# Gabriel-Ducrocq/GibbsSampler

Hardware: NVIDIA B200
Metric: gibbs_iters_per_s (higher is better)
Workload: dtype f64

## Files before the change

### gibbssampler_b200/_lib.py

```python
import ctypes as C
import os

_HERE = os.path.dirname(os.path.abspath(__file__))
LIB_PATH = os.environ.get("GIBBS_B200_LIB") or os.path.join(_HERE, "csrc", "_build", "libgibbs_b200.so")

GS_ALM_COMPLEX = 0
GS_ALM_REAL = 1

_lib = None

_vp = C.c_void_p
_i = C.c_int
_d = C.c_double
_i64 = C.c_int64

SIGNATURES = {
    "gs_last_error_string": (C.c_char_p, []),
    "gs_version": (_i, []),
    "gs_plan_create": (_i, [C.POINTER(_vp), _i, _i, _i]),
    "gs_plan_destroy": (_i, [_vp]),
    "gs_plan_reserve_chains": (_i, [_vp, _i]),
    "gs_plan_nside": (_i, [_vp]),
    "gs_plan_lmax": (_i, [_vp]),
    "gs_plan_npix": (_i64, [_vp]),
    "gs_plan_nalm": (_i64, [_vp]),
    "gs_plan_nreal": (_i64, [_vp]),
    "gs_alm2map_spin0": (_i, [_vp, _vp, _i, _vp, _vp, _vp]),
    "gs_alm2map_spin2": (_i, [_vp, _vp, _vp, _i, _vp, _vp, _vp, _vp]),
    "gs_map2alm_spin0": (_i, [_vp, _vp, _vp, _i, _i, _vp, _vp, _i, _vp]),
    "gs_map2alm_spin2": (_i, [_vp, _vp, _vp, _vp, _i, _i, _vp, _vp, _vp, _i, _vp]),
    "gs_alm2map_batch": (_i, [_vp, _i, _i, _vp, _vp, _i64, _i, _vp, _vp, _vp, _i64, _vp]),
    "gs_map2alm_batch": (_i, [_vp, _i, _i, _vp, _vp, _i64, _vp, _i, _vp, _vp, _vp, _i64, _i, _vp]),
    "gs_real_to_complex": (_i, [_vp, _vp, _i, _vp]),
    "gs_complex_to_real": (_i, [_vp, _vp, _i, _vp]),
    "gs_expand_per_l": (_i, [_vp, _i, _i, _vp, _vp]),
    "gs_unfold_bins": (_i, [_vp, _vp, _i, _vp, _i, _vp]),
    "gs_almxfl": (_i, [_vp, _i, _i, _vp, _vp, _vp]),
    "gs_alm2cl": (_i, [_vp, _i, _i, _vp, _vp]),
    "gs_alm2map_spin2_fl2": (_i, [_vp, _vp, _vp, _i, _vp, _vp, _vp, _vp, _vp]),
    "gs_cr_rhs_pol": (_i, [_vp] * 14 + [_i, _vp, _vp, _vp]),
    "gs_cr_pcg_pol": (_i, [_vp, _vp, _vp, _vp, _vp, _d, _vp, _vp, _vp, _vp, _i, _d, _i, _i,
                           C.POINTER(_i), C.POINTER(_d), _vp]),
    "gs_cr_pcg_pol_batch": (_i, [_vp, _i, _vp, _vp, _vp, _vp, _d, _vp, _vp, _vp, _vp, _i64, _d, _i, _i,
                                 C.POINTER(_i), C.POINTER(_d), _vp]),
    "gs_set_pcg_graph": (_i, [_i]),
    "gs_cr_apply_q_pol": (_i, [_vp] * 10),
    "gs_cr_rhs_tt": (_i, [_vp] * 9 + [_i, _vp, _vp]),
    "gs_cr_pcg_tt": (_i, [_vp, _vp, _vp, _vp, _d, _vp, _vp, _i, _d, _i, _i, C.POINTER(_i), C.POINTER(_d), _vp]),
    "gs_cr_apply_q_tt": (_i, [_vp] * 7),
    "gs_cr_rhs_teb": (_i, [_vp] * 22 + [_i, _vp, _vp, _vp, _vp]),
    "gs_cr_pcg_teb": (_i, [_vp] * 8 + [_d, _d] + [_vp] * 6 + [_i, _d, _i, _i, C.POINTER(_i), C.POINTER(_d), _vp]),
    "gs_cr_apply_q_teb": (_i, [_vp] * 15),
    "gs_gibbs_run_centered_fullsky": (_i, [_i, _i64, _d, _vp, _vp, _vp, _vp, _i, _vp, _i, _vp, _vp, _i, C.c_uint64, _vp, _vp, _vp, _vp,
                                           _i, _vp]),
    "gs_cr_direct": (_i, [_vp, _vp, _vp, _vp, _d, _i, _i, _vp, _vp]),
    "gs_cr_direct_pix": (_i, [_vp, _vp, _vp, _vp, _d, _i, _i, _i, _vp, _vp]),
    "gs_cls_invgamma": (_i, [_vp, _vp, _i, _vp, C.c_uint64, C.c_uint64, _vp, _vp, _vp, _vp]),
    "gs_truncnorm_propose": (_i, [_vp, _vp, _i, _vp, _vp, _vp]),
    "gs_truncnorm_logpdf": (_i, [_vp, _vp, _vp, _i, _vp, _vp]),
    "gs_loglik_pix": (_i, [_vp, _vp, _vp, _vp, _vp, _i64, _vp, _vp, _vp]),
    "gs_loglik_alm": (_i, [_vp, _vp, _vp, _vp, _vp, _vp, _i, _d, _vp, _vp, _vp]),
    "gs_randn": (_i, [_vp, _i64, C.c_uint64, C.c_uint64, _vp]),
    "gs_randu": (_i, [_vp, _i64, C.c_uint64, C.c_uint64, _vp]),
    "gs_sum": (_i, [_vp, _i64, _vp, _vp, _vp]),
    "gs_mwg_filters": (_i, [_vp, _vp, _vp, _vp, _vp, _i, _vp, _i, _i, _i, _i, _vp, _i, _i, _vp, _vp, _vp]),
    "gs_mwg_accept": (_i, [_vp, _vp, _vp, _i, _i, _vp, _vp, _vp, _vp, _vp]),
    "gs_mwg_sweep_blocks": (_i, [_vp] * 9 + [_vp, _i, _vp, _i, _vp, _i, _vp, _i, _i, _vp, _i, _vp, _vp, _vp, _vp, _vp, _vp, _i64, _vp]),
    "gs_mul": (_i, [_vp, _vp, _vp, _i64, _vp]),
    "gs_aux_v_update": (_i, [_vp, _vp, _vp, _vp, _d, _d, _vp, _vp, _i64, _vp]),
    "gs_aux_s_update": (_i, [_vp, _vp, _vp, _vp, _d, _d, _i, _vp, _vp]),
    "gs_pncp_factor": (_i, [_vp, _i, _i, _i, _vp, _vp]),
    "gs_mala_sigma": (_i, [_vp, _vp, _d, _i, _vp, _vp]),
    "gs_mala_grad": (_i, [_vp, _vp, _vp, _vp, _vp, _i64, _vp]),
    "gs_mala_propose": (_i, [_vp, _vp, _vp, _vp, _d, _vp, _i64, _vp]),
    "gs_mala_logq": (_i, [_vp, _vp, _vp, _vp, _d, _i64, _vp, _vp, _vp]),
    "gs_dot3": (_i, [_vp, _vp, _vp, _i64, _vp, _vp, _vp]),
    "gs_ula_nomask": (_i, [_vp, _vp, _vp, _vp, _vp, _d, _d, _i, _vp, _vp, _vp, _vp]),
    "gs_remove_monopole_dipole": (_i, [_vp, _i, _vp]),
    "gs_expand_var_cl_3x3": (_i, [_vp, _i, _vp, _vp]),
    "gs_inv_chol_3x3": (_i, [_vp, _vp, _i, _vp, _vp, _vp]),
    "gs_matvec_3x3": (_i, [_vp, _vp, _vp, _i, _vp, _vp]),
    "gs_alm2cl_cross": (_i, [_vp, _vp, _i, _vp, _vp]),
    "gs_cls_invwishart": (_i, [_vp, _vp, _vp, _i, _vp, C.c_uint64, C.c_uint64, _vp, _vp, _vp, _vp]),
    "gs_cls_invwishart_binned": (_i, [_vp, _vp, _vp, _i, _vp, _i, _vp, C.c_uint64, C.c_uint64, _vp, _vp, _vp, _vp]),
    "gs_nccl_unique_id": (_i, [C.c_char_p]),
    "gs_plan_create_sharded": (_i, [C.POINTER(_vp), _i, _i, _i, _i, _i, C.c_char_p]),
    "gs_local_group_create": (_i, [C.POINTER(_vp), _i]),
    "gs_local_group_destroy": (_i, [_vp]),
    "gs_plan_create_sharded_local": (_i, [C.POINTER(_vp), _i, _i, _i, _i, _i, _vp]),
    "gs_plan_world": (_i, [_vp]),
    "gs_plan_rank": (_i, [_vp]),
    "gs_plan_nreal_local": (_i64, [_vp]),
    "gs_plan_npix_local": (_i64, [_vp]),
    "gs_shard_partition_m": (_i, [_i, _i, _i, _vp]),
    "gs_shard_partition_rings": (_i, [_i, _i, _i, _vp]),
    "gs_shard_real_index": (_i64, [_i, _i, _i, _vp]),
    "gs_shard_pixel_index": (_i64, [_i, _i, _i, _vp]),
    "gs_shard_expand_per_l": (_i, [_vp, _vp, _i, _vp, _vp]),
# ... 42 lines not shown
```

### gibbssampler_b200/csrc/gs_internal.h

```cpp
#pragma once
#include <cuda_runtime.h>
#include <stdint.h>
#include <string>
#include <vector>

#include "../../include/gibbs_b200.h"

void gs_set_error(const char* fmt, ...);
#define GS_CHECK_CUDA(expr)                                                                  \
    do {                                                                                     \
        cudaError_t _e = (expr);                                                             \
        if (_e != cudaSuccess) {                                                             \
            gs_set_error("%s:%d: %s -> %s", __FILE__, __LINE__, #expr, cudaGetErrorString(_e)); \
            return GS_E_CUDA;                                                                \
        }                                                                                    \
    } while (0)
#define GS_CHECK_LAUNCH() GS_CHECK_CUDA(cudaGetLastError())
#define GS_REQUIRE(cond, msg)                                \
    do {                                                     \
        if (!(cond)) {                                       \
            gs_set_error("%s: %s", __func__, msg);           \
            return GS_E_BADARG;                              \
        }                                                    \
    } while (0)
// ... 31 lines not shown
    const int64_t* rbase;
    const int* m_owner;
    const int* m_loc;
    const int* ring_owner;
    const int* ring_loc;
    const int64_t* ring_start_loc;
    const int* l_of_loc;
};

struct SplitJob {
    int ringA, compA, ringB, compB;
    int bs2;
    int pad;
    int64_t off;
};

struct PlanDev {
    int nside, lmax, nring, npair;
    int64_t npix, nalm;
    const double* cth;
    const double* sth;
    const double* c2;
    const double* s2;
    const int* mlim0;
    const int* mlim2;
    const int* pmin0;
    const int* pmin2;
    const ScaledSeed* seed0;
    const ScaledSeed* seed2;
    const ScaledSeed* sinpow;
    const double* rec0;
    const double* alpha0;
    const double2* rec2;
    const double* alpha2;
    const int* ring_nphi;
    const int64_t* ring_start;
    const int* ring_phq;
    const int* ring_phden;
    const int* ring_bs;
    const BluesteinDesc* bs;
    const double2* bs_tab;
    const double2* tw;
    int tw_n;
    int max_M;
    ShardDev sh;
};

struct RingFlags {
    unsigned char* act_ring;
    int* act_pairs;
    int* act_count;
    int* act_slot0;
    double* ring_wconst;
    int2* groups0_dyn;
    int2* groups2_dyn;
};

struct gs_plan {
    int device;
    PlanDev d;
    int world, rank;
    int64_t nreal_loc, npix_loc;
    void* comm;
    void* lgroup;
    double2* Fx;
    double* red_loc;
    std::vector<int> h_mlist, h_rings;
    std::vector<void*> owned;
    RingJob* jobs2;
    int njobs2;
    RingJob* jobs0;
    int njobs0;
    int2* groups2;
    int ngroups2;
    int2* groups0;
    int ngroups0;
    int2* groups2_dyn;
    int2* groups0_dyn;
    SplitJob* sjobs2;
    int nsjobs2;
    SplitJob* sjobs0;
    int nsjobs0;
    double2* ring_scratch;
    size_t split_smem;
    double2* mwg_F;
    double* mwg_maps;
    int mwg_group;
    double* mwg_small;
    double* mwg_data;
    int* mwg_meta;
    std::vector<int> mwg_meta_host;
    unsigned char* act_ring;
    int* act_pairs;
    int* act_count;
    double* act_red;
    int* act_slot0;
    double* ring_wconst;
    bool use_act;
    double2* Fm;
    double* partial;
    int anal_chunks;
    int chain_cap;
    size_t ring_smem;
    double* mapQ_tmp;
    double* mapU_tmp;
    double* almE_tmp;
    double* almB_tmp;
    double* almE_tmp2;
    double* almB_tmp2;
    void* pcg_ws;
    void* pcg_ws_batch;
    int* pcg_alldone;
    void* pcg_ws_teb;
    RingFlags flags_T;
    void* comm_stream;
    std::vector<void*> comm_events;
    void* work_stream;
    void* work_event;
};

extern int g_gs_ring_const;
extern int g_gs_ring_skip;
extern int g_gs_ring_fused;
extern long long g_gs_launches;
static inline int64_t gs_nalm(int lmax) { return (int64_t)(lmax + 1) * (lmax + 2) / 2; }

int gs_leg_synth(gs_plan* p, int spin, const double* almE, const double* almB, int layout, const double* fl,
                 cudaStream_t st, const int* skip = nullptr, const double* flB = nullptr, int nc = 1, int64_t alm_stride = 0);
int gs_leg_anal(gs_plan* p, int spin, double* almE, double* almB, int layout, const double* fl, double scale,
                int accumulate, cudaStream_t st, const int* skip = nullptr, int nc = 1, int64_t alm_stride = 0);
int64_t gs_fm_stride(const gs_plan* p);
int64_t gs_part_stride(const gs_plan* p, int nc);
int gs_active_rings_build(gs_plan* p, const double* pixw, cudaStream_t st);
int gs_leg_build_sinpow(gs_plan* p);
int gs_leg_prepare(gs_plan* p);
int gs_ring_setup(gs_plan* p);
int gs_ring_synth(gs_plan* p, int spin, double* mapQ, double* mapU, cudaStream_t st, const int* skip = nullptr, int nc = 1,
                  int64_t map_stride = 0, const double* wconst = nullptr);
int gs_ring_anal(gs_plan* p, int spin, const double* mapQ, const double* mapU, const double* pixw, cudaStream_t st,
                 const int* skip = nullptr, int nc = 1, int64_t map_stride = 0);
int gs_ring_apply(gs_plan* p, int spin, const double* pixw, cudaStream_t st, const int* skip = nullptr, int nc = 1);
int gs_ring_synth_batch(gs_plan* p, const double2* F, int64_t f_stride, const int* mmax, double* mapQ, double* mapU,
                        int64_t map_stride, int nb, cudaStream_t st, const unsigned char* ract = nullptr, const double* wconst = nullptr);
int gs_ring_order_build(gs_plan* p, cudaStream_t st);
int gs_ring_mwg_data(gs_plan* p, const double* mapQ, const double* mapU, double* outQ, double* outU, const double* wconst, cudaStream_t st);
int gs_leg_synth_blocks(gs_plan* p, const double* almE, const double* almB, const double* dflE, const double* dflB,
                        const int* lbE, int e0, int e1, const int* lbB, int b0, int b1, int lend, double2* Fblk, cudaStream_t st);
int gs_launch_expand_per_l(const double* x, int lmax, int mode, double* out, cudaStream_t st);
int gs_plan_expand_per_l(gs_plan* p, const double* x, int mode, double* out, cudaStream_t st);
void gs_pcg_ws_free(gs_plan* p);
int gs_shard_build(gs_plan* p, int rank, int world, const char* nccl_id);
void gs_shard_free(gs_plan* p);
int gs_shard_exchange(gs_plan* p, const double2* send, double2* recv, cudaStream_t st);
int gs_shard_exchange_block(gs_plan* p, const double2* send, double2* recv, int blk, cudaStream_t st);
int gs_shard_pipeline(gs_plan* p, cudaStream_t* comm, cudaEvent_t** events);
int gs_shard_allreduce(gs_plan* p, double* buf, int n, cudaStream_t st);
```

### gibbssampler_b200/csrc/legendre.cu

```cuda
#include <algorithm>
#include <type_traits>

#include "gs_internal.h"

#ifndef LEG_NT
#define LEG_NT 128
#endif
#define LEG_NW (LEG_NT / 32)
#define LEG_TL LEG_NT
#ifndef LEG_SU
#define LEG_SU 1
#endif
#define LEG_TLS (LEG_SU * LEG_NT)
#ifndef LEG_R
#define LEG_R 2
#endif
#ifndef LEG_R2
#define LEG_R2 2
#endif
#ifndef LEG_RA
#define LEG_RA 4
#endif
#ifndef LEG_UA
#define LEG_UA 2
// ... 189 lines not shown
#pragma unroll
    for (int c = 1; c < NC; ++c) {
        double2 dummy;
        fetch_alm<SPIN, false>(P, m, l, base, roff, almE + c * alm_stride, SPIN ? almB + c * alm_stride : almB, layout, fl, flB, e[c], b[c], dummy);
    }
}

template <bool SH>
__device__ __forceinline__ int64_t fm_index(const PlanDev& P, int comp, int ring, int m, int mk)
{
    if (SH) {
        const int blk = mk / P.sh.MLb, w = mk - blk * P.sh.MLb;
        return ((((int64_t)blk * P.sh.world + P.sh.ring_owner[ring]) * 2 + comp) * P.sh.RL + P.sh.ring_loc[ring]) * P.sh.MLb + w;
    }
    return ((int64_t)comp * P.nring + ring) * (P.lmax + 1) + m;
}
template <bool SH>
__device__ __forceinline__ int64_t real_off(const PlanDev& P, int m, int mk, int64_t base)
{
    if (SH) return P.sh.rbase[mk] - (m ? 2 : 1) * (int64_t)m;
    return m ? 2 * base - (P.lmax + 1) : 0;
}

template <int SPIN>
struct SynthAcc {
    double sqr, sqi, aqr, aqi;
    double sur, sui, aur, aui;
};

template <int SPIN, bool FIRST>
__device__ __forceinline__ void synth_acc(SynthAcc<SPIN>& A, double pc, double mc, double2 e, double2 b)
{
    if (SPIN == 0) {
        if (FIRST) { A.sqr = fma(e.x, pc, A.sqr); A.sqi = fma(e.y, pc, A.sqi); }
        else       { A.aqr = fma(e.x, pc, A.aqr); A.aqi = fma(e.y, pc, A.aqi); }
    } else {
        A.sqr = fma(pc, e.x, A.sqr); A.sqi = fma(mc, e.y, A.sqi);
        A.sur = fma(pc, b.x, A.sur); A.sui = fma(mc, b.y, A.sui);
        if (FIRST) {
            A.aqr = fma(mc, e.x, A.aqr); A.aqi = fma(pc, e.y, A.aqi);
            A.aur = fma(mc, b.x, A.aur); A.aui = fma(pc, b.y, A.aui);
        } else {
            A.aqr = fma(-mc, e.x, A.aqr); A.aqi = fma(-pc, e.y, A.aqi);
            A.aur = fma(-mc, b.x, A.aur); A.aui = fma(-pc, b.y, A.aui);
        }
    }
}

template <int SPIN, int R, bool SH, int NC>
__global__ void LEG_SYNTH_BOUNDS
leg_synth_kernel(PlanDev P, const double* __restrict__ almE, const double* __restrict__ almB, int layout,
                 const double* __restrict__ fl, const double* __restrict__ flB, double2* __restrict__ Fm,
                 const int* __restrict__ skip, const int* __restrict__ plist, const int* __restrict__ pcount,
                 const int* __restrict__ slot0, int64_t alm_stride, int64_t fm_stride, int mk0)
{
    if (skip && *skip) return;
    const int L = P.lmax, mk = blockIdx.y + mk0, m = SH ? P.sh.mlist[mk] : mk, tid = threadIdx.x;
    const int s0 = slot0[m], nact = (plist ? *pcount : P.npair) - s0;
    if ((int)blockIdx.x * (LEG_NT * R) >= nact) return;
    __shared__ double2 sEb[2][NC][LEG_TLS], sBb[2][SPIN ? NC : 1][SPIN ? LEG_TLS : 1], sRb[2][LEG_TLS];
    const int l0 = m > SPIN ? m : SPIN;
    const int64_t base = (int64_t)m * (2 * L + 1 - m) / 2;
    const int64_t roff = real_off<SH>(P, m, mk, base);
    const int chunk = blockIdx.x * (LEG_NT * R);

    RingState<SPIN> st[R];
    SynthAcc<SPIN> acc[R][NC];
    int pj[R];
    bool any_act = false;
    unsigned myact = 0;
#pragma unroll
    for (int j = 0; j < R; ++j) {
        const int k = chunk + ((tid >> 5) * R + j) * 32 + (tid & 31);
        const int p = k < nact ? (plist ? plist[s0 + k] : s0 + k) : -1;
        pj[j] = p;
        st[j].x = 0.0; st[j].pc = st[j].pp = st[j].mc = st[j].mp = 0.0; st[j].sc = 0;
#pragma unroll
        for (int c = 0; c < NC; ++c) {
            acc[j][c].sqr = acc[j][c].sqi = acc[j][c].aqr = acc[j][c].aqi = 0.0;
            acc[j][c].sur = acc[j][c].sui = acc[j][c].aur = acc[j][c].aui = 0.0;
        }
        if (p >= 0 && m <= (SPIN ? P.mlim2[p] : P.mlim0[p])) {
            st[j].x = P.cth[p];
            seed_ring<SPIN>(P, p, m, st[j].pc, st[j].mc, st[j].sc);
            any_act = true;
            myact |= 1u << j;
        }
    }
    const bool warp_act = __any_sync(FULL, any_act);
    unsigned gact = 0;
#pragma unroll
    for (int j = 0; j < R; ++j) if (__any_sync(FULL, (myact >> j) & 1u)) gact |= 1u << j;
    bool all_live = false;

#pragma unroll
    for (int u = 0; u < LEG_SU; ++u) {
        double2 e[NC], b[NC], r;
        fetch_alm_nc<SPIN, NC>(P, m, l0 + u * LEG_NT + tid, base, roff, almE, almB, alm_stride, layout, fl, flB, e, b, r);
#pragma unroll
        for (int c = 0; c < NC; ++c) { sEb[0][c][u * LEG_NT + tid] = e[c]; if (SPIN) sBb[0][c][u * LEG_NT + tid] = b[c]; }
        sRb[0][u * LEG_NT + tid] = r;
    }
    __syncthreads();
    int cur = 0;
    for (int lt = l0; lt <= L; lt += LEG_TLS, cur ^= 1) {
        const bool has_next = lt + LEG_TLS <= L;
        double2 ne[LEG_SU][NC], nb[LEG_SU][NC], nr[LEG_SU];
// ... 62 lines not shown
                        }
                        rec_step<SPIN>(st[j], r0.x, r0.y);
                        if (j >= J0) {
#pragma unroll
                            for (int c = 0; c < NC; ++c) synth_acc<SPIN, false>(acc[j][c], st[j].pc, st[j].mc, e1[c], b1[c]);
                        }
                        rec_step<SPIN>(st[j], r1.x, r1.y);
                    }
                }
            };
            if (R >= 4 && jlo == 3) run(std::integral_constant<int, (R >= 4 ? 3 : R)>());
            else if (R >= 3 && jlo == 2) run(std::integral_constant<int, (R >= 3 ? 2 : R)>());
            else if (R >= 2 && jlo == 1) run(std::integral_constant<int, (R >= 2 ? 1 : R)>());
            else run(std::integral_constant<int, R>());
        }
#pragma unroll 2
        for (; ip < npr; ++ip) {
            const int i = 2 * ip;
            const double2 r0 = sR[i], r1 = sR[i + 1];
            double2 e0[NC], b0[NC], e1[NC], b1[NC];
#pragma unroll
            for (int c = 0; c < NC; ++c) {
                e0[c] = sE[c][i]; e1[c] = sE[c][i + 1];
                b0[c] = SPIN ? sB[c][i] : e0[c]; b1[c] = SPIN ? sB[c][i + 1] : e1[c];
            }
#pragma unroll
            for (int j = 0; j < R; ++j) {
#pragma unroll
                for (int c = 0; c < NC; ++c) synth_acc<SPIN, true>(acc[j][c], st[j].pc, st[j].mc, e0[c], b0[c]);
                rec_step<SPIN>(st[j], r0.x, r0.y);
#pragma unroll
                for (int c = 0; c < NC; ++c) synth_acc<SPIN, false>(acc[j][c], st[j].pc, st[j].mc, e1[c], b1[c]);
                rec_step<SPIN>(st[j], r1.x, r1.y);
            }
        }
        if (has_next) {
#pragma unroll
            for (int u = 0; u < LEG_SU; ++u) {
#pragma unroll
                for (int c = 0; c < NC; ++c) { sEb[cur ^ 1][c][u * LEG_NT + tid] = ne[u][c]; if (SPIN) sBb[cur ^ 1][c][u * LEG_NT + tid] = nb[u][c]; }
                sRb[cur ^ 1][u * LEG_NT + tid] = nr[u];
            }
        }
        __syncthreads();
    }

    const double sg = ((l0 + m) & 1) ? -1.0 : 1.0;
#pragma unroll
    for (int j = 0; j < R; ++j) {
        const int p = pj[j];
        if (p < 0) continue;
        const int rn = p, rs = P.nring - 1 - p;
        const int64_t in = fm_index<SH>(P, 0, rn, m, mk), is = fm_index<SH>(P, 0, rs, m, mk);
#pragma unroll
        for (int c = 0; c < NC; ++c) {
            const SynthAcc<SPIN>& a = acc[j][c];
            double2* F = Fm + c * fm_stride;
            if (SPIN == 0) {
                F[in] = make_double2(a.sqr + a.aqr, a.sqi + a.aqi);
                if (rs != rn) F[is] = make_double2(sg * (a.sqr - a.aqr), sg * (a.sqi - a.aqi));
            } else {
                const int64_t cs = SH ? (int64_t)P.sh.RL * P.sh.MLb : (int64_t)P.nring * (L + 1);
                F[in] = make_double2(a.sqr + a.sqi, a.sur + a.sui);
                F[in + cs] = make_double2(a.sur - a.sui, a.sqi - a.sqr);
                if (rs != rn) {
                    F[is] = make_double2(sg * (a.aqr + a.aqi), sg * (a.aur + a.aui));
                    F[is + cs] = make_double2(sg * (a.aur - a.aui), sg * (a.aqi - a.aqr));
                }
            }
        }
    }
}

template <int R, bool DO_E, bool DO_B>
__global__ void __launch_bounds__(LEG_NT)
leg_synth_blocks_kernel(PlanDev P, const double* __restrict__ almE, const double* __restrict__ almB, const double* __restrict__ dflE,
                        const double* __restrict__ dflB, const int* __restrict__ lbE, int e0, int e1, const int* __restrict__ lbB,
                        int b0, int b1, int lend, double2* __restrict__ Fblk)
{
    __shared__ double2 sE[LEG_TL], sB[LEG_TL], sSE[LEG_TL], sSB[LEG_TL], sR[LEG_TL];
    extern __shared__ unsigned char sflag[];
    const int L = P.lmax, m = blockIdx.y, tid = threadIdx.x;
    const int l0 = m > 2 ? m : 2;
    if (l0 >= lend) return;
    const int s0 = P.pmin2[m], nact = P.npair - s0;
    const int chunk = blockIdx.x * (LEG_NT * R);
    if (chunk >= nact) return;
    unsigned char* sfE = sflag;
    unsigned char* sfB = sflag + (L + 2);
    for (int i = tid; i < 2 * (L + 2); i += LEG_NT) sflag[i] = 0;
    __syncthreads();
    if (DO_E) for (int i = e0 + tid; i < e1; i += LEG_NT) { const int end = lbE[i + 1]; if (end >= 1 && end <= L + 1) sfE[end - 1] = 1; }
    if (DO_B) for (int i = b0 + tid; i < b1; i += LEG_NT) { const int end = lbB[i + 1]; if (end >= 1 && end <= L + 1) sfB[end - 1] = 1; }
    const int64_t base = (int64_t)m * (2 * L + 1 - m) / 2;
    const int64_t roff = real_off<false>(P, m, m, base);
    const int64_t nm = L + 1, cs = (int64_t)P.nring * nm, slot = 2 * cs;

    RingState<2> st[R];
    double aE[R][DO_E ? 8 : 1], aB[R][DO_B ? 8 : 1];
    int pj[R];
    bool any_act = false, all_plain = true;
#pragma unroll
    for (int j = 0; j < R; ++j) {
        const int k = chunk + ((tid >> 5) * R + j) * 32 + (tid & 31);
        const int p = k < nact ? s0 + k : -1;
        pj[j] = p;
        st[j].x = 0.0; st[j].pc = st[j].pp = st[j].mc = st[j].mp = 0.0; st[j].sc = 0;
#pragma unroll
        for (int q = 0; q < (DO_E ? 8 : 1); ++q) aE[j][q] = 0.0;
#pragma unroll
        for (int q = 0; q < (DO_B ? 8 : 1); ++q) aB[j][q] = 0.0;
        if (p >= 0 && m <= P.mlim2[p]) {
            st[j].x = P.cth[p];
            seed_ring<2>(P, p, m, st[j].pc, st[j].mc, st[j].sc);
            any_act = true;
            all_plain = all_plain && st[j].sc == 0;
        }
    }
    const bool warp_act = __any_sync(FULL, any_act);
    bool fast = __all_sync(FULL, all_plain);
// ... 435 lines not shown
        } else {
#pragma unroll kUnrollA
            for (; ip < npr; ++ip) {
                double v[NC][NVAL];
                const double2 r0 = sR[2 * ip], r1 = sR[2 * ip + 1];
#pragma unroll
                for (int j = 0; j < R; ++j) {
#pragma unroll
                    for (int c = 0; c < NC; ++c) {
                        if (j == 0) anal_acc<SPIN, true, true>(v[c], G[j][c], st[j].pc, st[j].mc);
                        else anal_acc<SPIN, true, false>(v[c], G[j][c], st[j].pc, st[j].mc);
                    }
                    rec_step<SPIN>(st[j], r0.x, r0.y);
#pragma unroll
                    for (int c = 0; c < NC; ++c) {
                        if (j == 0) anal_acc<SPIN, false, true>(v[c] + NV, G[j][c], st[j].pc, st[j].mc);
                        else anal_acc<SPIN, false, false>(v[c] + NV, G[j][c], st[j].pc, st[j].mc);
                    }
                    rec_step<SPIN>(st[j], r1.x, r1.y);
                }
#pragma unroll
                for (int c = 0; c < NC; ++c) {
                    const double s = warp_fold<SPIN>(v[c], lane);
                    if (writer) sPart(w, c)[ip * NVAL + vidx] = __hiloint2double(__double2hiint(s) ^ flipmask, __double2loint(s));
                }
            }
        }
        __syncthreads();
#pragma unroll
        for (int c = 0; c < NC; ++c) {
            double* out = partial + c * part_stride + (pbase + lt) * NV;
            for (int i = tid; i < ni * NV; i += LEG_NT) {
                double s = 0.0;
#pragma unroll
                for (int ww = 0; ww < LEG_NW; ++ww) s += sPart(ww, c)[i];
                out[i] = s;
            }
        }
    }
}

template <int SPIN, bool SH>
__global__ void leg_finish_kernel(PlanDev P, const double* __restrict__ partial, int nchunk, double* __restrict__ almE,
                                  double* __restrict__ almB, int layout, const double* __restrict__ fl, double scale,
                                  int accumulate, const int* __restrict__ skip, const int* __restrict__ pcount,
                                  const int* __restrict__ slot0, int chunk_pairs, int64_t part_stride, int64_t alm_stride)
{
    if (skip && *skip) return;
    constexpr int NV = SPIN ? 4 : 2;
    const int L = P.lmax, mk = blockIdx.y, m = SH ? P.sh.mlist[mk] : mk;
    partial += blockIdx.z * part_stride;
    almE += blockIdx.z * alm_stride;
    if (SPIN) almB += blockIdx.z * alm_stride;
    {
        const int nact = (pcount ? *pcount : P.npair) - slot0[m];
        nchunk = nact > 0 ? (nact + chunk_pairs - 1) / chunk_pairs : 0;
    }
    const int l = m + blockIdx.x * blockDim.x + threadIdx.x;
    if (l > L) return;
    const int64_t base = (int64_t)m * (2 * L + 1 - m) / 2, id = base + l;
    const int64_t pid = SH ? P.sh.cbase[mk] + (l - m) : id, pn = SH ? P.sh.nalm_loc : P.nalm;
    const int64_t roff = real_off<SH>(P, m, mk, base);
    double v[NV];
#pragma unroll
    for (int c = 0; c < NV; ++c) v[c] = 0.0;
    if (l >= SPIN) {
        for (int k = 0; k < nchunk; ++k) {
            const double* q = partial + ((int64_t)k * pn + pid) * NV;
#pragma unroll
            for (int c = 0; c < NV; ++c) v[c] += q[c];
        }
        if (SPIN) {
            const double y1 = v[0], y2 = v[1], y3 = v[2], y4 = v[3];
            v[0] = y1 + y2; v[1] = y3 + y4; v[2] = y3 - y4; v[3] = y2 - y1;
        }
        double post = scale * (SPIN ? -0.5 * P.alpha2[id] : P.alpha0[id]);
        if (fl) post *= fl[l];
        if (layout == GS_ALM_REAL && m > 0) post *= 1.41421356237309504880;
#pragma unroll
        for (int c = 0; c < NV; ++c) v[c] *= post;
    }
    if (layout == GS_ALM_COMPLEX) {
        double2* E = reinterpret_cast<double2*>(almE);
        double2 e = make_double2(v[0], v[1]);
        if (accumulate) { double2 o = E[id]; e.x += o.x; e.y += o.y; }
        E[id] = e;
        if (SPIN) {
            double2* B = reinterpret_cast<double2*>(almB);
            double2 b = make_double2(v[2], v[3]);
            if (accumulate) { double2 o = B[id]; b.x += o.x; b.y += o.y; }
            B[id] = b;
        }
    } else if (m == 0) {
        almE[roff + l] = accumulate ? almE[roff + l] + v[0] : v[0];
        if (SPIN) almB[roff + l] = accumulate ? almB[roff + l] + v[2] : v[2];
    } else {
        const int64_t off = roff + 2 * l;
        almE[off] = accumulate ? almE[off] + v[0] : v[0];
        almE[off + 1] = accumulate ? almE[off + 1] + v[1] : v[1];
        if (SPIN) {
            almB[off] = accumulate ? almB[off] + v[2] : v[2];
            almB[off + 1] = accumulate ? almB[off + 1] + v[3] : v[3];
        }
    }
}

template <bool SH>
__global__ void __launch_bounds__(256) ring_active_kernel(PlanDev P, const double* __restrict__ pixw, unsigned char* __restrict__ act,
                                                          double* __restrict__ actd, double* __restrict__ wconst)
{
    const int ring = blockIdx.x, n = P.ring_nphi[ring];
    if (SH && P.sh.ring_owner[ring] != P.sh.rank) { if (threadIdx.x == 0) actd[ring] = 0.0; return; }
    const double* w = pixw + (SH ? P.sh.ring_start_loc[ring] : P.ring_start[ring]);
    const double w0 = w[0];
    int any = 0, differ = 0;
    for (int j = threadIdx.x; j < n; j += blockDim.x) { const double v = w[j]; any |= (v != 0.0); differ |= !(v == w0); }
    any = __syncthreads_or(any);
    if (!SH && wconst) differ = __syncthreads_or(differ);
    if (threadIdx.x == 0) {
        if (SH) actd[ring] = any ? 1.0 : 0.0; else act[ring] = any ? 1 : 0;
        if (!SH && wconst) wconst[ring] = differ ? __longlong_as_double(0x7ff8000000000000LL) : w0;
    }
}

__global__ void ring_flags_kernel(const double* __restrict__ actd, unsigned char* __restrict__ act, int n)
{
    const int i = blockIdx.x * blockDim.x + threadIdx.x;
    if (i < n) act[i] = actd[i] > 0.0 ? 1 : 0;
}

__global__ void __launch_bounds__(1024) pair_compact_kernel(PlanDev P, unsigned char* act, int* __restrict__ list,
                                                            int* __restrict__ count)
{
    __shared__ int wsum[32];
// ... 17 lines not shown
    }
    if (tid == 0) *count = base;
}

__global__ void __launch_bounds__(256) list_slot0_kernel(PlanDev P, const int* __restrict__ list, const int* __restrict__ count,
                                                         int* __restrict__ slot0)
{
    const int L = P.lmax, wid = (blockIdx.x * blockDim.x + threadIdx.x) >> 5, lane = threadIdx.x & 31;
    if (wid >= 2 * (L + 1)) return;
    const int spin2 = wid > L, m = spin2 ? wid - (L + 1) : wid, n = *count;
    const int* mlim = spin2 ? P.mlim2 : P.mlim0;
    int first = n;
    for (int k0 = 0; k0 < n && first == n; k0 += 32) {
        const int k = k0 + lane;
        const unsigned b = __ballot_sync(FULL, k < n && mlim[list[k]] >= m);
        if (b) first = k0 + __ffs(b) - 1;
    }
    if (lane == 0) slot0[wid] = first;
}

int gs_active_rings_build(gs_plan* p, const double* pixw, cudaStream_t st)
{
    if (p->world > 1) {
        ring_active_kernel<true><<<p->d.nring, 256, 0, st>>>(p->d, pixw, p->act_ring, p->act_red, nullptr);
        GS_CHECK_LAUNCH();
        int rc = gs_shard_allreduce(p, p->act_red, p->d.nring, st);
        if (rc) return rc;
        ring_flags_kernel<<<(p->d.nring + 255) / 256, 256, 0, st>>>(p->act_red, p->act_ring, p->d.nring);
    } else {
        ring_active_kernel<false><<<p->d.nring, 256, 0, st>>>(p->d, pixw, p->act_ring, nullptr, p->ring_wconst);
    }
    pair_compact_kernel<<<1, 1024, 0, st>>>(p->d, p->act_ring, p->act_pairs, p->act_count);
    list_slot0_kernel<<<(2 * (p->d.lmax + 1) * 32 + 255) / 256, 256, 0, st>>>(p->d, p->act_pairs, p->act_count, p->act_slot0);
    GS_CHECK_LAUNCH();
    g_gs_launches += 3;
    return gs_ring_order_build(p, st);
}

int64_t gs_fm_stride(const gs_plan* p) { return (int64_t)2 * p->d.nring * (p->d.lmax + 1); }
static int anal_chunks_of(const gs_plan* p, int nc) { const int per = LEG_NT * (nc > 1 ? LEG_RA2 : LEG_RA); return (p->d.npair + per - 1) / per; }
int64_t gs_part_stride(const gs_plan* p, int nc) { return (int64_t)anal_chunks_of(p, nc) * p->d.nalm * 4; }

static int check_batch(const gs_plan* p, int nc, int layout, const char* who)
{
    if (nc == 1) return GS_OK;
    if (nc != 2) { gs_set_error("%s: chain batches run 2 right-hand sides per launch (got %d)", who, nc); return GS_E_BADARG; }
    if (p->world > 1) { gs_set_error("%s: chain batches need an unsharded plan", who); return GS_E_BADARG; }
    if (p->chain_cap < nc) { gs_set_error("%s: call gs_plan_reserve_chains(plan, %d) first", who, nc); return GS_E_BADARG; }
    (void)layout;
    return GS_OK;
}

int gs_leg_synth(gs_plan* p, int spin, const double* almE, const double* almB, int layout, const double* fl,
                 cudaStream_t st, const int* skip, const double* flB, int nc, int64_t alm_stride)
{
    const bool sh = p->world > 1;
    if (sh && layout != GS_ALM_REAL) { gs_set_error("sharded plans take the (local) real alm layout only"); return GS_E_BADARG; }
    int rc = check_batch(p, nc, layout, "gs_leg_synth");
    if (rc) return rc;
    const int rr = nc == 2 ? LEG_R2 : LEG_R;
    dim3 grid((p->d.npair + LEG_NT * rr - 1) / (LEG_NT * rr), sh ? p->d.sh.nm_loc : p->d.lmax + 1);
    const int* plist = p->use_act ? p->act_pairs : nullptr;
    const int* pcount = plist ? p->act_count : nullptr;
    const int* slot0 = plist ? p->act_slot0 + (spin ? p->d.lmax + 1 : 0) : (spin ? p->d.pmin2 : p->d.pmin0);
    const int64_t fs = gs_fm_stride(p);
    if (nc == 2) {
        if (spin == 0) leg_synth_kernel<0, LEG_R2, false, 2><<<grid, LEG_NT, 0, st>>>(p->d, almE, almB, layout, fl, flB, p->Fm, skip, plist, pcount, slot0, alm_stride, fs, 0);
        else leg_synth_kernel<2, LEG_R2, false, 2><<<grid, LEG_NT, 0, st>>>(p->d, almE, almB, layout, fl, flB, p->Fm, skip, plist, pcount, slot0, alm_stride, fs, 0);
    } else if (!sh) {
        if (spin == 0) leg_synth_kernel<0, LEG_R, false, 1><<<grid, LEG_NT, 0, st>>>(p->d, almE, almB, layout, fl, flB, p->Fm, skip, plist, pcount, slot0, 0, 0, 0);
        else leg_synth_kernel<2, LEG_R, false, 1><<<grid, LEG_NT, 0, st>>>(p->d, almE, almB, layout, fl, flB, p->Fm, skip, plist, pcount, slot0, 0, 0, 0);
    } else {
        const ShardDev& S = p->d.sh;
        cudaStream_t comm = st;
        cudaEvent_t* ev = nullptr;
        const bool pipelined = !p->lgroup && S.NB > 1;
        if (pipelined && (rc = gs_shard_pipeline(p, &comm, &ev))) return rc;
        for (int b = 0; b < S.NB; ++b) {
            const int mk0 = b * S.MLb, cnt = std::min(S.MLb, S.nm_loc - mk0);
            if (cnt > 0) {
                dim3 g(grid.x, cnt);
                if (spin == 0) leg_synth_kernel<0, LEG_R, true, 1><<<g, LEG_NT, 0, st>>>(p->d, almE, almB, layout, fl, flB, p->Fm, skip, plist, pcount, slot0, 0, 0, mk0);
                else leg_synth_kernel<2, LEG_R, true, 1><<<g, LEG_NT, 0, st>>>(p->d, almE, almB, layout, fl, flB, p->Fm, skip, plist, pcount, slot0, 0, 0, mk0);
                GS_CHECK_LAUNCH();
                g_gs_launches += 1;
            }
            if (pipelined) {
                GS_CHECK_CUDA(cudaEventRecord(ev[b], st));
                GS_CHECK_CUDA(cudaStreamWaitEvent(comm, ev[b], 0));
            }
            if ((rc = gs_shard_exchange_block(p, p->Fm, p->Fx, b, comm))) return rc;
        }
        if (pipelined) {
            GS_CHECK_CUDA(cudaEventRecord(ev[S.NB], comm));
            GS_CHECK_CUDA(cudaStreamWaitEvent(st, ev[S.NB], 0));
        }
        return GS_OK;
    }
    GS_CHECK_LAUNCH();
    g_gs_launches += 1;
    return GS_OK;
}

template <int SPIN, int R, bool SH, int NC>
static int launch_anal(gs_plan* p, dim3 grid, cudaStream_t st, const int* skip, const int* plist, const int* pcount, const int* slot0,
                       int64_t fs, int64_t ps, int mk0 = 0)
{
    constexpr size_t sm = leg_anal_smem<SPIN, NC>();
    leg_anal_kernel<SPIN, R, SH, NC><<<grid, LEG_NT, sm, st>>>(p->d, p->Fm, p->partial, skip, plist, pcount, slot0, fs, ps, mk0);
    GS_CHECK_LAUNCH();
    return GS_OK;
}

int gs_leg_prepare(gs_plan* p)
{
    (void)p;
#define GS_ANAL_ATTR(SPIN, R, SH, NC) \
    GS_CHECK_CUDA(cudaFuncSetAttribute(leg_anal_kernel<SPIN, R, SH, NC>, cudaFuncAttributeMaxDynamicSharedMemorySize, (int)leg_anal_smem<SPIN, NC>()))
    GS_ANAL_ATTR(0, LEG_RA, false, 1); GS_ANAL_ATTR(2, LEG_RA, false, 1);
    GS_ANAL_ATTR(0, LEG_RA, true, 1);  GS_ANAL_ATTR(2, LEG_RA, true, 1);
    GS_ANAL_ATTR(0, LEG_RA2, false, 2); GS_ANAL_ATTR(2, LEG_RA2, false, 2);
#undef GS_ANAL_ATTR
    return GS_OK;
}

int gs_leg_anal(gs_plan* p, int spin, double* almE, double* almB, int layout, const double* fl, double scale,
                int accumulate, cudaStream_t st, const int* skip, int nc, int64_t alm_stride)
{
    const bool sh = p->world > 1;
    if (sh && layout != GS_ALM_REAL) { gs_set_error("sharded plans take the (local) real alm layout only"); return GS_E_BADARG; }
    int rc = check_batch(p, nc, layout, "gs_leg_anal");
    if (rc) return rc;
    const int nchunk = anal_chunks_of(p, nc);
    if (nchunk * nc > p->anal_chunks) { gs_set_error("gs_leg_anal: workspace too small"); return GS_E_BADARG; }
    const int nmy = sh ? p->d.sh.nm_loc : p->d.lmax + 1;
    dim3 grid(nchunk, nmy);
    dim3 fgrid((p->d.lmax + 256) / 256, nmy, nc);
    const int* plist = p->use_act ? p->act_pairs : nullptr;
    const int* pcount = plist ? p->act_count : nullptr;
    const int* slot0 = plist ? p->act_slot0 + (spin ? p->d.lmax + 1 : 0) : (spin ? p->d.pmin2 : p->d.pmin0);
    const int64_t fs = gs_fm_stride(p), ps = gs_part_stride(p, nc);
    const int cp = LEG_NT * (nc > 1 ? LEG_RA2 : LEG_RA);

    if (nc == 2) {
        if (spin == 0) {
            if ((rc = launch_anal<0, LEG_RA2, false, 2>(p, grid, st, skip, plist, pcount, slot0, fs, ps))) return rc;
            leg_finish_kernel<0, false><<<fgrid, 256, 0, st>>>(p->d, p->partial, nchunk, almE, almB, layout, fl, scale, accumulate, skip, pcount, slot0, cp, ps, alm_stride);
        } else {
            if ((rc = launch_anal<2, LEG_RA2, false, 2>(p, grid, st, skip, plist, pcount, slot0, fs, ps))) return rc;
            leg_finish_kernel<2, false><<<fgrid, 256, 0, st>>>(p->d, p->partial, nchunk, almE, almB, layout, fl, scale, accumulate, skip, pcount, slot0, cp, ps, alm_stride);
        }
    } else if (!sh) {
        if (spin == 0) {
            if ((rc = launch_anal<0, LEG_RA, false, 1>(p, grid, st, skip, plist, pcount, slot0, 0, 0))) return rc;
            leg_finish_kernel<0, false><<<fgrid, 256, 0, st>>>(p->d, p->partial, nchunk, almE, almB, layout, fl, scale, accumulate, skip, pcount, slot0, cp, 0, 0);
        } else {
            if ((rc = launch_anal<2, LEG_RA, false, 1>(p, grid, st, skip, plist, pcount, slot0, 0, 0))) return rc;
            leg_finish_kernel<2, false><<<fgrid, 256, 0, st>>>(p->d, p->partial, nchunk, almE, almB, layout, fl, scale, accumulate, skip, pcount, slot0, cp, 0, 0);
        }
    } else {
        const ShardDev& S = p->d.sh;
        cudaStream_t comm = st;
        cudaEvent_t* ev = nullptr;
        const bool pipelined = !p->lgroup && S.NB > 1;
        if (pipelined) {
            if ((rc = gs_shard_pipeline(p, &comm, &ev))) return rc;
            GS_CHECK_CUDA(cudaEventRecord(ev[S.NB], st));
            GS_CHECK_CUDA(cudaStreamWaitEvent(comm, ev[S.NB], 0));
        }
        for (int b = 0; b < S.NB; ++b) {
            if ((rc = gs_shard_exchange_block(p, p->Fx, p->Fm, b, comm))) return rc;
            if (pipelined) {
                GS_CHECK_CUDA(cudaEventRecord(ev[b], comm));
                GS_CHECK_CUDA(cudaStreamWaitEvent(st, ev[b], 0));
            }
            const int mk0 = b * S.MLb, cnt = std::min(S.MLb, S.nm_loc - mk0);
            if (cnt <= 0) continue;
            dim3 g(grid.x, cnt);
            if (spin == 0) rc = launch_anal<0, LEG_RA, true, 1>(p, g, st, skip, plist, pcount, slot0, 0, 0, mk0);
            else rc = launch_anal<2, LEG_RA, true, 1>(p, g, st, skip, plist, pcount, slot0, 0, 0, mk0);
            if (rc) return rc;
        }
        if (spin == 0) leg_finish_kernel<0, true><<<fgrid, 256, 0, st>>>(p->d, p->partial, nchunk, almE, almB, layout, fl, scale, accumulate, skip, pcount, slot0, cp, 0, 0);
        else leg_finish_kernel<2, true><<<fgrid, 256, 0, st>>>(p->d, p->partial, nchunk, almE, almB, layout, fl, scale, accumulate, skip, pcount, slot0, cp, 0, 0);
    }
    GS_CHECK_LAUNCH();
    g_gs_launches += 2;
    return GS_OK;
}

int gs_leg_synth_blocks(gs_plan* p, const double* almE, const double* almB, const double* dflE, const double* dflB,
                        const int* lbE, int e0, int e1, const int* lbB, int b0, int b1, int lend, double2* Fblk, cudaStream_t st)
{
    if (p->world > 1) { gs_set_error("block-batched synthesis needs an unsharded plan"); return GS_E_BADARG; }
    constexpr int RB = 2;
    dim3 grid((p->d.npair + LEG_NT * RB - 1) / (LEG_NT * RB), std::min(lend, p->d.lmax + 1));
    const size_t sm = 2 * (size_t)(p->d.lmax + 2);
    const bool doE = e1 > e0, doB = b1 > b0;
    if (!doE && !doB) return GS_OK;
    if (doE && doB) leg_synth_blocks_kernel<RB, true, true><<<grid, LEG_NT, sm, st>>>(p->d, almE, almB, dflE, dflB, lbE, e0, e1, lbB, b0, b1, lend, Fblk);
    else if (doE) leg_synth_blocks_kernel<RB, true, false><<<grid, LEG_NT, sm, st>>>(p->d, almE, almB, dflE, dflB, lbE, e0, e1, lbB, b0, b1, lend, Fblk);
    else leg_synth_blocks_kernel<RB, false, true><<<grid, LEG_NT, sm, st>>>(p->d, almE, almB, dflE, dflB, lbE, e0, e1, lbB, b0, b1, lend, Fblk);
    GS_CHECK_LAUNCH();
    g_gs_launches += 1;
    return GS_OK;
}
```

### gibbssampler_b200/csrc/plan.cu

```cuda
#include <math.h>
#include <stdarg.h>
#include <stdio.h>
#include <string.h>

#include <algorithm>

#include "gs_internal.h"

static thread_local char g_err[512] = "";

void gs_set_error(const char* fmt, ...)
{
    va_list ap;
    va_start(ap, fmt);
    vsnprintf(g_err, sizeof(g_err), fmt, ap);
    va_end(ap);
}

extern "C" const char* gs_last_error_string(void) { return g_err; }
extern "C" int gs_version(void) { return 100; }

static const long double PI_L = 3.14159265358979323846264338327950288L;

template <typename T>
// ... 152 lines not shown
                long double ll = l, L1 = l + 1.0L, mm = m;
                long double den = sqrtl((L1 * L1 - mm * mm) * (L1 * L1 - mp * mp));
                long double f = L1 * (2.0L * ll + 1.0L) / den;
                long double A = sqrtl((2.0L * ll + 3.0L) / (2.0L * ll + 1.0L)) * f;
                long double B = (l == 0) ? 0.0L : mm * mp / (ll * L1);
                long double a_next;
                if (l == l0) a_next = 1.0L;
                else {
                    long double Cc = sqrtl((2.0L * ll + 3.0L) / (2.0L * ll - 1.0L)) * f *
                                     sqrtl((ll * ll - mm * mm) * (ll * ll - mp * mp)) / (ll * (2.0L * ll + 1.0L));
                    a_next = Cc * a_prev;
                }
                long double a = A * a_cur / a_next;
                if (spin == 0) rec0[base + l] = (double)a;
                else rec2[base + l] = make_double2((double)a, (double)(a * B));
                a_prev = a_cur;
                a_cur = a_next;
            }
        }
    }
    if ((rc = upload(p, rec0, &p->d.rec0))) return rc;
    if ((rc = upload(p, alpha0, &p->d.alpha0))) return rc;
    if ((rc = upload(p, rec2, &p->d.rec2))) return rc;
    if ((rc = upload(p, alpha2, &p->d.alpha2))) return rc;
    return GS_OK;
}

static int plan_create_impl(gs_plan** out, int nside, int lmax, int device, int rank, int world, const char* nccl_id,
                            void* lgroup = nullptr)
{
    if (!out) { gs_set_error("gs_plan_create: null output"); return GS_E_BADARG; }
    *out = nullptr;
    GS_REQUIRE(nside >= 1 && nside <= 8192, "nside out of range [1, 8192]");
    GS_REQUIRE(lmax >= 2 && lmax <= 4 * nside, "lmax must satisfy 2 <= lmax <= 4 nside");
    GS_REQUIRE(world >= 1 && rank >= 0 && rank < world, "need 0 <= rank < world");
    GS_REQUIRE(world <= 2 * nside && world <= (lmax + 2) / 2, "more ranks than ring pairs or m pairs");
    if (device >= 0) GS_CHECK_CUDA(cudaSetDevice(device));
    int dev = 0;
    GS_CHECK_CUDA(cudaGetDevice(&dev));
    gs_plan* p = new gs_plan();
    memset(&p->d, 0, sizeof(p->d));
    p->device = dev;
    p->d.nside = nside;
    p->d.lmax = lmax;
    p->jobs0 = p->jobs2 = nullptr;
    p->groups0 = p->groups2 = nullptr;
    p->groups0_dyn = p->groups2_dyn = nullptr;
    p->ngroups0 = p->ngroups2 = 0;
    p->sjobs0 = p->sjobs2 = nullptr;
    p->nsjobs0 = p->nsjobs2 = 0;
    p->ring_scratch = nullptr;
    p->act_ring = nullptr;
    p->ring_wconst = nullptr;
    p->act_pairs = nullptr;
    p->act_count = nullptr;
    p->act_slot0 = nullptr;
    p->act_red = nullptr;
    p->use_act = false;
    p->mwg_F = nullptr;
    p->mwg_maps = nullptr;
    p->mwg_group = 0;
    p->mwg_small = nullptr;
    p->mwg_data = nullptr;
    p->mwg_meta = nullptr;
    p->world = world;
    p->rank = rank;
    p->comm = nullptr;
    p->lgroup = lgroup;
    p->pcg_ws = nullptr;
    p->pcg_ws_batch = nullptr;
    p->pcg_alldone = nullptr;
    p->pcg_ws_teb = nullptr;
    memset(&p->flags_T, 0, sizeof(p->flags_T));
    p->work_stream = nullptr;
    p->work_event = nullptr;
    p->comm_stream = nullptr;
    p->chain_cap = 1;
    p->Fx = nullptr;
    p->red_loc = nullptr;
    p->d.sh.world = 1;
    int rc = build_tables(p);
    if (rc == GS_OK) rc = gs_leg_build_sinpow(p);
    if (rc == GS_OK) rc = gs_leg_prepare(p);
    const int64_t nm = lmax + 1;
    p->nreal_loc = nm * nm;
    p->npix_loc = p->d.npix;
    if (rc == GS_OK && world > 1) rc = gs_shard_build(p, rank, world, nccl_id);
    if (rc == GS_OK) rc = gs_ring_setup(p);
    if (rc == GS_OK) {
        const size_t nfm = world > 1 ? (size_t)world * 2 * p->d.sh.RL * p->d.sh.ML : (size_t)2 * p->d.nring * nm;
        rc = dev_alloc(p, nfm, &p->Fm);
        if (rc == GS_OK && world > 1) rc = dev_alloc(p, nfm, &p->Fx);
        if (rc == GS_OK) cudaMemset(p->Fm, 0, nfm * sizeof(double2));
        if (rc == GS_OK && world > 1) cudaMemset(p->Fx, 0, nfm * sizeof(double2));
        p->anal_chunks = (p->d.npair + 127) / 128;
        const size_t nalm_part = world > 1 ? (size_t)p->d.sh.nalm_loc : (size_t)p->d.nalm;
        if (rc == GS_OK) rc = dev_alloc(p, (size_t)p->anal_chunks * nalm_part * 4, &p->partial);
        if (rc == GS_OK) rc = dev_alloc(p, (size_t)p->d.nring, &p->act_ring);
        if (rc == GS_OK) rc = dev_alloc(p, (size_t)p->d.npair, &p->act_pairs);
        if (rc == GS_OK) rc = dev_alloc(p, (size_t)1, &p->act_count);
        if (rc == GS_OK) rc = dev_alloc(p, (size_t)2 * (lmax + 1), &p->act_slot0);
        if (rc == GS_OK) rc = dev_alloc(p, (size_t)p->d.nring, &p->act_red);
        if (rc == GS_OK && world <= 1) rc = dev_alloc(p, (size_t)p->d.nring, &p->ring_wconst);
        if (rc == GS_OK) rc = dev_alloc(p, (size_t)p->npix_loc, &p->mapQ_tmp);
        if (rc == GS_OK) rc = dev_alloc(p, (size_t)p->npix_loc, &p->mapU_tmp);
        const size_t nre = (size_t)p->nreal_loc;
        if (rc == GS_OK) rc = dev_alloc(p, nre, &p->almE_tmp);
        if (rc == GS_OK) rc = dev_alloc(p, nre, &p->almB_tmp);
        if (rc == GS_OK) rc = dev_alloc(p, nre, &p->almE_tmp2);
        if (rc == GS_OK) rc = dev_alloc(p, nre, &p->almB_tmp2);
    }
    if (rc == GS_OK) {
        cudaError_t e = cudaDeviceSynchronize();
        if (e != cudaSuccess) { gs_set_error("plan setup: %s", cudaGetErrorString(e)); rc = GS_E_CUDA; }
    }
    if (rc != GS_OK) { gs_plan_destroy(p); return rc; }
    *out = p;
    return GS_OK;
}

extern "C" int gs_plan_create(gs_plan** out, int nside, int lmax, int device)
{
    return plan_create_impl(out, nside, lmax, device, 0, 1, nullptr);
}

extern "C" int gs_plan_create_sharded(gs_plan** out, int nside, int lmax, int device, int rank, int world,
                                      const char* nccl_id128_host)
{
    return plan_create_impl(out, nside, lmax, device, rank, world, nccl_id128_host);
}

extern "C" int gs_plan_create_sharded_local(gs_plan** out, int nside, int lmax, int device, int rank, int world,
                                            void* local_group)
{
    if (!local_group) { gs_set_error("null local group"); return GS_E_BADARG; }
    return plan_create_impl(out, nside, lmax, device, rank, world, nullptr, local_group);
}

extern "C" int gs_plan_reserve_chains(gs_plan* p, int n_chain)
{
    if (!p) { gs_set_error("null plan"); return GS_E_BADARG; }
    GS_REQUIRE(n_chain >= 1 && n_chain <= 2, "n_chain must be 1 or 2");
    GS_REQUIRE(p->world == 1, "chain batches need an unsharded plan");
    if (n_chain <= p->chain_cap) return GS_OK;
    GS_CHECK_CUDA(cudaSetDevice(p->device));
    const int64_t nm = p->d.lmax + 1;
    const size_t nfm = (size_t)n_chain * 2 * p->d.nring * nm;
    double2* F = nullptr;
    int rc = dev_alloc(p, nfm, &F);
    if (rc) return rc;
    GS_CHECK_CUDA(cudaMemset(F, 0, nfm * sizeof(double2)));
    const int chunks = std::max(p->anal_chunks, n_chain * ((p->d.npair + 255) / 256));
    double* part = nullptr;
    if (chunks > p->anal_chunks) {
        rc = dev_alloc(p, (size_t)chunks * p->d.nalm * 4, &part);
        if (rc) return rc;
// ... 34 lines not shown
```

### gibbssampler_b200/csrc/ringfft.cu

```cuda
#include <math.h>
#include <stdlib.h>

#include <algorithm>
#include <map>

#include "gs_internal.h"

#define RF_NT 256

__device__ __forceinline__ double2 cmul(double2 a, double2 b) { return make_double2(a.x * b.x - a.y * b.y, a.x * b.y + a.y * b.x); }
__device__ __forceinline__ double2 cmulc(double2 a, double2 b) { return make_double2(a.x * b.x + a.y * b.y, a.y * b.x - a.x * b.y); }
__device__ __forceinline__ double2 cadd(double2 a, double2 b) { return make_double2(a.x + b.x, a.y + b.y); }
__device__ __forceinline__ double2 csub(double2 a, double2 b) { return make_double2(a.x - b.x, a.y - b.y); }

#define PADI(i) ((i) + ((i) >> 4) + ((i) >> 8))
#define PADLEN(M) ((M) + ((M) >> 4) + ((M) >> 8) + 2)

__device__ __forceinline__ double2 tw_get(const double2* twq, int idx, int quarter)
{
    if (idx < quarter) return twq[idx];
    const double2 w = twq[idx - quarter];
    return make_double2(w.y, -w.x);
}

// ... 167 lines not shown
    if (r == 3) { N <<= 3; pass8<true>(buf, M, N, twq, twn, tid, nt); return; }
    if (r & 2) { N <<= 2; pass4<true>(buf, M, N, twq, twn, tid, nt); }
    if (r & 1) { N <<= 1; pass2<true>(buf, M, N, twq, twn, tid, nt); }
}

__device__ __forceinline__ void load_twq(const PlanDev& P, double2* twq)
{
    const int nq = (P.tw_n >> 2) + 1;
    for (int k = threadIdx.x; k < nq; k += RF_NT) twq[k] = __ldg(&P.tw[k]);
}

__device__ __forceinline__ double2 chirp_val(int t, int n)
{
    const int r = (int)(((long long)t * t) % (2 * n));
    double s, c;
    sincospi((double)r / (double)n, &s, &c);
    return make_double2(c, s);
}

__device__ void ring_idft(const PlanDev& P, double2* buf, const double2* twq, int n, int bsi, int tid = threadIdx.x, int nt = RF_NT)
{
    __syncthreads();
    if (bsi < 0) { fft_dit_inv(buf, n, twq, P.tw_n, tid, nt); return; }
    const BluesteinDesc d = P.bs[bsi];
    fft_dif<true>(buf, d.M, twq, P.tw_n, P.bs_tab + d.bhat_off, tid, nt);
    fft_dit_inv(buf, d.M, twq, P.tw_n, tid, nt);
}

__global__ void __launch_bounds__(RF_NT) bluestein_setup_kernel(PlanDev P, double2* tab, int nbs)
{
    extern __shared__ double2 smem_all[];
    double2* twq = smem_all;
    double2* buf = smem_all + (P.tw_n >> 2) + 1;
    load_twq(P, twq);
    const BluesteinDesc d = P.bs[blockIdx.x];
    double2* chirp = tab + d.chirp_off;
    double2* bhat = tab + d.bhat_off;
    for (int k = threadIdx.x; k < d.M; k += blockDim.x) buf[PADI(k)] = make_double2(0.0, 0.0);
    __syncthreads();
    for (int t = threadIdx.x; t < d.n; t += blockDim.x) {
        const double2 c = chirp_val(t, d.n);
        chirp[t] = c;
        const double2 cc = make_double2(c.x, -c.y);
        buf[PADI(t)] = cc;
        if (t > 0) buf[PADI(d.M - t)] = cc;
    }
    __syncthreads();
    fft_dif<false>(buf, d.M, twq, P.tw_n, nullptr);
    const double inv = 1.0 / (double)d.M;
    for (int k = threadIdx.x; k < d.M; k += blockDim.x) { const double2 v = buf[PADI(k)]; bhat[k] = make_double2(v.x * inv, v.y * inv); }
    (void)nbs;
}

__device__ __forceinline__ double2 ring_phase(const PlanDev& P, int ring, int m)
{
    const int q = P.ring_phq[ring], den = P.ring_phden[ring];
    const unsigned r = ((unsigned)m * (unsigned)q) % (2u * (unsigned)den);
    double s, c;
    sincospi((double)r / (double)den, &s, &c);
    return make_double2(c, s);
}

template <bool SH>
__device__ __forceinline__ int64_t fm_ring_index(const PlanDev& P, int comp, int ring, int m)
{
    if (SH) return P.sh.m_base[m] + ((int64_t)comp * P.sh.RL + P.sh.ring_loc[ring]) * P.sh.MLb;
    return ((int64_t)comp * P.nring + ring) * (P.lmax + 1) + m;
}
template <bool SH>
__device__ __forceinline__ int64_t ring_first_pixel(const PlanDev& P, int ring)
{
    return SH ? P.sh.ring_start_loc[ring] : P.ring_start[ring];
}

__device__ __forceinline__ int ring_mtop(const PlanDev& P, int ring, int spin2)
{
    const int p = ring < P.npair ? ring : P.nring - 1 - ring;
    return spin2 ? P.mlim2[p] : P.mlim0[p];
}

__device__ __forceinline__ bool group_idle(const unsigned char* __restrict__ ract, const RingJob* __restrict__ jobs, const int2* __restrict__ groups)
{
    if (!ract) return false;
    const int2 g = groups[blockIdx.x];
    bool any = false;
    for (int s = 0; s < g.y; ++s) {
        const RingJob jb = jobs[g.x + s];
        any = any || ract[jb.ringA] || (jb.ringB >= 0 && ract[jb.ringB]);
    }
    return !any;
}
__device__ __forceinline__ bool group_const(const double* __restrict__ wconst, const RingJob* __restrict__ jobs, const int2* __restrict__ groups)
{
    if (!wconst) return false;
    const int2 g = groups[blockIdx.x];
    bool all = true;
    for (int s = 0; s < g.y; ++s) {
        const RingJob jb = jobs[g.x + s];
        const double a = wconst[jb.ringA], b = jb.ringB >= 0 ? wconst[jb.ringB] : 0.0;
        all = all && a == a && b == b;
    }
    return all;
}
__global__ void __launch_bounds__(1024) ring_order_kernel(const RingJob* __restrict__ jobs, const int2* __restrict__ groups, int ngroups,
                                                          const unsigned char* __restrict__ ract, const double* __restrict__ wconst,
                                                          int2* __restrict__ groups_out)
{
    __shared__ int wcount[32][3];
    __shared__ int base[3], total[3];
    const int tid = threadIdx.x, lane = tid & 31, w = tid >> 5;
    auto cls_of = [&](int gi) {
        if (gi >= ngroups) return 3;
        const int2 g = groups[gi];
        bool any = false, allc = true;
        for (int s = 0; s < g.y; ++s) {
            const RingJob jb = jobs[g.x + s];
            any = any || ract[jb.ringA] || (jb.ringB >= 0 && ract[jb.ringB]);
            const double a = wconst[jb.ringA], b = jb.ringB >= 0 ? wconst[jb.ringB] : 0.0;
            allc = allc && a == a && b == b;
        }
        return !any ? 2 : allc ? 1 : 0;
    };
    for (int pass = 0; pass < 2; ++pass) {
        if (tid < 3) { if (pass == 0) total[tid] = 0; else base[tid] = tid == 0 ? 0 : tid == 1 ? total[0] : total[0] + total[1]; }
        __syncthreads();
        for (int g0 = 0; g0 < ngroups; g0 += 1024) {
            const int gi = g0 + tid, c = cls_of(gi);
            unsigned bal[3];
#pragma unroll
            for (int k = 0; k < 3; ++k) { bal[k] = __ballot_sync(0xffffffffu, c == k); if (lane == 0) wcount[w][k] = __popc(bal[k]); }
            __syncthreads();
            if (pass == 1 && c < 3) {
                int off = base[c];
                for (int i = 0; i < w; ++i) off += wcount[i][c];
                groups_out[off + __popc(bal[c] & ((1u << lane) - 1u))] = groups[gi];
            }
            __syncthreads();
            if (tid < 3) {
                int t = 0;
                for (int i = 0; i < 32; ++i) t += wcount[i][tid];
                if (pass == 0) total[tid] += t; else base[tid] += t;
            }
            __syncthreads();
        }
    }
}

__device__ __forceinline__ bool split_idle(const unsigned char* __restrict__ ract, const SplitJob& jb)
{
    return ract && !(ract[jb.ringA] || (jb.ringB >= 0 && ract[jb.ringB]));
}

struct RingSub {
    RingJob job;
    int n, bsi, M, tid, nt;
    double2* buf;
    double2* scratch;
    const double2* chirp;
};

// ... 270 lines not shown
    const int lg = 31 - __clz(n);
    for (int j = S.tid; j < S.M; j += S.nt) {
        const int pos = PADI(S.bsi < 0 ? (int)(__brev((unsigned)j) >> (32 - lg)) : j);
        if (j >= n) { S.buf[pos] = make_double2(0.0, 0.0); continue; }
        double a = ia[j], b = ib ? ib[j] : 0.0;
        if (pixw) { a *= pixw[sa + j]; if (ib) b *= pixw[sb + j]; }
        double2 z = make_double2(a, -b);
        if (S.bsi >= 0) z = cmul(z, __ldg(&S.chirp[j]));
        S.buf[pos] = z;
    }
    ring_idft(P, S.buf, twq, n, S.bsi, S.tid, S.nt);
    ring_unpack_F<SH>(P, S, UNPACK_CONJ, Fm, ring_mtop(P, job.ringA, spin2), S.bsi >= 0 ? S.chirp : nullptr);
}

__global__ void __launch_bounds__(RF_NT, 2)
ring_mwg_data_kernel(PlanDev P, const RingJob* __restrict__ jobs, const int2* __restrict__ groups, const double* __restrict__ mapQ,
                     const double* __restrict__ mapU, double* __restrict__ outQ, double* __restrict__ outU, const double* __restrict__ wconst)
{
    extern __shared__ double2 smem[];
    double2* twq = smem;
    const bool spectral = group_const(wconst, jobs, groups);
    if (spectral) load_twq(P, twq);
    const RingSub S = ring_sub(P, jobs, groups, twq + (P.tw_n >> 2) + 1);
    const int n = S.n;
    const int64_t s0 = P.ring_start[S.job.ringA];
    const double* ia = mapQ + s0;
    const double* ib = mapU + s0;
    if (!spectral) {
        for (int j = S.tid; j < n; j += S.nt) { outQ[s0 + j] = ia[j]; outU[s0 + j] = ib[j]; }
        return;
    }
    const int lg = 31 - __clz(n);
    for (int j = S.tid; j < S.M; j += S.nt) {
        const int pos = PADI(S.bsi < 0 ? (int)(__brev((unsigned)j) >> (32 - lg)) : j);
        if (j >= n) { S.buf[pos] = make_double2(0.0, 0.0); continue; }
        double2 z = make_double2(ia[j], -ib[j]);
        if (S.bsi >= 0) z = cmul(z, __ldg(&S.chirp[j]));
        S.buf[pos] = z;
    }
    ring_idft(P, S.buf, twq, n, S.bsi, S.tid, S.nt);
    const double s = rsqrt((double)n);
    for (int k = S.tid; k < n; k += S.nt) {
        double2 c = S.buf[PADI(k)];
        if (S.bsi >= 0) c = cmul(c, __ldg(&S.chirp[k]));
        outQ[s0 + k] = s * c.x;
        outU[s0 + k] = -s * c.y;
    }
}

template <bool SH>
__global__ void __launch_bounds__(RF_NT, 2)
ring_apply_kernel(PlanDev P, const RingJob* __restrict__ jobs, const int2* __restrict__ groups, double2* __restrict__ Fm,
                  const double* __restrict__ pixw, const int* __restrict__ skip, const unsigned char* __restrict__ ract, int spin2,
                  int64_t f_stride, const double* __restrict__ wconst)
{
    if (skip && *skip) return;
    if (group_idle(ract, jobs, groups)) return;
    extern __shared__ double2 smem[];
    Fm += blockIdx.y * f_stride;
    double2* twq = smem;
    if (group_const(wconst, jobs, groups)) {
        const RingSub S = ring_sub(P, jobs, groups, twq + (P.tw_n >> 2) + 1);
        const int mtop = ring_mtop(P, S.job.ringA, spin2);
        const double wA = wconst[S.job.ringA], wB = wconst[S.job.ringB >= 0 ? S.job.ringB : S.job.ringA];
        bool direct = true;
        {
            const int2 g = groups[blockIdx.x];
            for (int s = 0; s < g.y; ++s) {
                const int ra = jobs[g.x + s].ringA;
                direct = direct && 2 * ring_mtop(P, ra, spin2) <= P.ring_nphi[ra];
            }
        }
        if (direct) {
            const RingJob& job = S.job;
            const double sa = (double)S.n * wA, sb = (double)S.n * wB;
            for (int m = S.tid; m <= mtop; m += S.nt) {
                const int64_t ia = fm_ring_index<SH>(P, job.compA, job.ringA, m);
                const int64_t ib = job.ringB >= 0 ? fm_ring_index<SH>(P, job.compB, job.ringB, m) : ia;
                double2 a = Fm[ia], b = job.ringB >= 0 ? Fm[ib] : make_double2(0.0, 0.0);
                if (m == 0) { a.y = 0.0; b.y = 0.0; }
                else if (2 * m == S.n) {
                    const double2 e2 = ring_phase(P, job.ringA, 2 * m);
                    const double2 ta = cmul(a, e2), tb = cmul(b, e2);
                    a = make_double2(a.x + ta.x, a.y - ta.y);
                    b = make_double2(b.x + tb.x, b.y - tb.y);
                }
                Fm[ia] = make_double2(sa * a.x, sa * a.y);
                if (job.ringB >= 0) Fm[ib] = make_double2(sb * b.x, sb * b.y);
            }
            return;
        }
        ring_build_Z<SH>(P, S, Fm, mtop, S.scratch, false, true);
        __syncthreads();
        const double half_n = 0.5 * (double)S.n;
        ring_unpack_F<SH>(P, S, UNPACK_PLAIN, Fm, mtop, nullptr, half_n * wA, half_n * wB);
        return;
    }
    load_twq(P, twq);
    const RingSub S = ring_sub(P, jobs, groups, twq + (P.tw_n >> 2) + 1);
    const int n = S.n;
    const double* wa = pixw + ring_first_pixel<SH>(P, S.job.ringA);
    const double* wb = S.job.ringB >= 0 ? pixw + ring_first_pixel<SH>(P, S.job.ringB) : wa;
    const int mtop = ring_mtop(P, S.job.ringA, spin2);
    ring_build_Z<SH>(P, S, Fm, mtop, S.scratch);
    __syncthreads();
    ring_idft(P, S.buf, twq, n, S.bsi, S.tid, S.nt);
    if (S.bsi < 0) {
        auto weigh = [wa, wb](int j, double2 z) { return make_double2(z.x * wa[j], z.y * wb[j]); };
        fft_dif<false>(S.buf, n, twq, P.tw_n, nullptr, S.tid, S.nt, weigh);
        ring_unpack_F<SH>(P, S, UNPACK_BREV, Fm, mtop);
    } else {
        const double2* chirp = S.chirp;
        for (int j = S.tid; j < S.M; j += S.nt) {
            if (j >= n) { S.buf[PADI(j)] = make_double2(0.0, 0.0); continue; }
            const double2 c = __ldg(&chirp[j]);
            const double2 z = cmul(S.buf[PADI(j)], c);
            S.buf[PADI(j)] = cmul(make_double2(z.x * wa[j], -z.y * wb[j]), c);
        }
        ring_idft(P, S.buf, twq, n, S.bsi, S.tid, S.nt);
        ring_unpack_F<SH>(P, S, UNPACK_CONJ, Fm, mtop, chirp);
    }
    __syncthreads();
}

template <bool SH>
__device__ __forceinline__ double2 fold_spectrum(const PlanDev& P, const double2* __restrict__ Fm, int comp, int ring, int k, int n, int L)
{
    const int kk = (n - k) % n;
    double2 g = make_double2(0.0, 0.0), h = g;
    for (int m = k; m <= L; m += n) {
        const double w = m ? 1.0 : 0.5;
        const double2 ph = ring_phase(P, ring, m);
        g = cadd(g, cmul(Fm[fm_ring_index<SH>(P, comp, ring, m)], make_double2(ph.x * w, ph.y * w)));
    }
    for (int m = kk; m <= L; m += n) {
        const double w = m ? 1.0 : 0.5;
        const double2 ph = ring_phase(P, ring, m);
        h = cadd(h, cmul(Fm[fm_ring_index<SH>(P, comp, ring, m)], make_double2(ph.x * w, ph.y * w)));
    }
    return make_double2(g.x + h.x, g.y - h.y);
}

__device__ __forceinline__ double2 mul_ipow(double2 v, int p)
{
// ... 354 lines not shown
        return rc;
    }
    const RingJob* jobs = spin == 0 ? p->jobs0 : p->jobs2;
    const int2* grp = spin == 0 ? p->groups0 : p->groups2;
    const SplitJob* sj = spin == 0 ? p->sjobs0 : p->sjobs2;
    const unsigned char* ract = p->use_act ? p->act_ring : nullptr;
    const double* mu = spin == 0 ? mapQ : mapU;
    const bool sh = p->world > 1;
    double2* F = sh ? p->Fx : p->Fm;
    if (ns > 0) {
        if (sh) {
            ring_anal_split_kernel<true><<<4 * ns, RF_NT, p->split_smem, st>>>(p->d, sj, mapQ, mu, pixw, p->ring_scratch, skip, ract);
            ring_anal_finish_kernel<true><<<ns, RF_NT, 0, st>>>(p->d, sj, p->ring_scratch, F, skip, ract);
        } else {
            ring_anal_split_kernel<false><<<4 * ns, RF_NT, p->split_smem, st>>>(p->d, sj, mapQ, mu, pixw, p->ring_scratch, skip, ract);
            ring_anal_finish_kernel<false><<<ns, RF_NT, 0, st>>>(p->d, sj, p->ring_scratch, F, skip, ract);
        }
        GS_CHECK_LAUNCH();
        g_gs_launches += 2;
    }
    if (nj > 0) {
        if (sh) ring_anal_kernel<true><<<nj, RF_NT, p->ring_smem, st>>>(p->d, jobs, grp, mapQ, mu, pixw, F, skip, spin ? 1 : 0, ract, 0, 0);
        else ring_anal_kernel<false><<<dim3(nj, nc), RF_NT, p->ring_smem, st>>>(p->d, jobs, grp, mapQ, mu, pixw, F, skip, spin ? 1 : 0, ract, nc > 1 ? gs_fm_stride(p) : 0, nc > 1 ? map_stride : 0);
        GS_CHECK_LAUNCH();
    }
    g_gs_launches += 1;
    return GS_OK;
}

int gs_ring_apply(gs_plan* p, int spin, const double* pixw, cudaStream_t st, const int* skip, int nc)
{
    const int nj = spin == 0 ? p->ngroups0 : p->ngroups2, ns = spin == 0 ? p->nsjobs0 : p->nsjobs2;
    if (nc > 1 && (p->world > 1 || !pixw)) { gs_set_error("chain batches need an unsharded plan and pixel weights"); return GS_E_BADARG; }
    if (nc > 1 && ns > 0) {
        double2* F0 = p->Fm;
        int rc = GS_OK;
        for (int c = 0; c < nc && rc == GS_OK; ++c) {
            p->Fm = F0 + c * gs_fm_stride(p);
            rc = gs_ring_apply(p, spin, pixw, st, skip, 1);
        }
        p->Fm = F0;
        return rc;
    }
    if (ns > 0 || !pixw) {
        int rc = gs_ring_synth(p, spin, p->mapQ_tmp, p->mapU_tmp, st, skip);
        if (rc) return rc;
        return gs_ring_anal(p, spin, p->mapQ_tmp, p->mapU_tmp, pixw, st, skip);
    }
    if (nj <= 0) return GS_OK;
    const RingJob* jobs = spin == 0 ? p->jobs0 : p->jobs2;
    const int2* grp = spin == 0 ? p->groups0 : p->groups2;
    const double* wconst = (p->use_act && g_gs_ring_const) ? p->ring_wconst : nullptr;
    if (wconst) grp = spin == 0 ? p->groups0_dyn : p->groups2_dyn;
    if (p->world > 1) ring_apply_kernel<true><<<nj, RF_NT, p->ring_smem, st>>>(p->d, jobs, grp, p->Fx, pixw, skip, p->use_act ? p->act_ring : nullptr, spin ? 1 : 0, 0, nullptr);
    else ring_apply_kernel<false><<<dim3(nj, nc), RF_NT, p->ring_smem, st>>>(p->d, jobs, grp, p->Fm, pixw, skip, p->use_act ? p->act_ring : nullptr, spin ? 1 : 0, nc > 1 ? gs_fm_stride(p) : 0, wconst);
    GS_CHECK_LAUNCH();
    g_gs_launches += 1;
    return GS_OK;
}

int gs_ring_order_build(gs_plan* p, cudaStream_t st)
{
    if (p->world > 1 || !p->ring_wconst) return GS_OK;
    if (p->ngroups2 > 0) ring_order_kernel<<<1, 1024, 0, st>>>(p->jobs2, p->groups2, p->ngroups2, p->act_ring, p->ring_wconst, p->groups2_dyn);
    if (p->ngroups0 > 0) ring_order_kernel<<<1, 1024, 0, st>>>(p->jobs0, p->groups0, p->ngroups0, p->act_ring, p->ring_wconst, p->groups0_dyn);
    GS_CHECK_LAUNCH();
    g_gs_launches += 2;
    return GS_OK;
}

int gs_ring_mwg_data(gs_plan* p, const double* mapQ, const double* mapU, double* outQ, double* outU, const double* wconst, cudaStream_t st)
{
    if (p->world > 1 || p->nsjobs2 > 0) { gs_set_error("spectral ring storage needs an unsharded plan without split rings"); return GS_E_BADARG; }
    if (p->ngroups2 <= 0) return GS_OK;
    ring_mwg_data_kernel<<<p->ngroups2, RF_NT, p->ring_smem, st>>>(p->d, p->jobs2, p->groups2, mapQ, mapU, outQ, outU, wconst);
    GS_CHECK_LAUNCH();
    g_gs_launches += 1;
    return GS_OK;
}

int gs_ring_synth_batch(gs_plan* p, const double2* F, int64_t f_stride, const int* mmax, double* mapQ, double* mapU,
                        int64_t map_stride, int nb, cudaStream_t st, const unsigned char* ract, const double* wconst)
{
    if (p->world > 1 || p->nsjobs2 > 0) { gs_set_error("batched ring synthesis needs an unsharded plan without split rings"); return GS_E_BADARG; }
    if (nb <= 0 || p->ngroups2 <= 0) return GS_OK;
    ring_synth_kernel<false><<<dim3(p->ngroups2, nb), RF_NT, p->ring_smem, st>>>(p->d, p->jobs2, wconst ? p->groups2_dyn : p->groups2, F, mapQ, mapU,
                                                                                 nullptr, f_stride, map_stride, mmax, 1, ract, wconst);
    GS_CHECK_LAUNCH();
    g_gs_launches += 1;
    return GS_OK;
}
```

### gibbssampler_b200/csrc/rng.cuh

```cuda
#pragma once
#include <math.h>
#include <stdint.h>

struct Philox {
    uint32_t k0, k1;
    __device__ Philox(uint64_t seed) : k0((uint32_t)seed), k1((uint32_t)(seed >> 32)) {}
    __device__ uint4 operator()(uint64_t ctr, uint64_t stream) const
    {
        uint32_t c0 = (uint32_t)ctr, c1 = (uint32_t)(ctr >> 32), c2 = (uint32_t)stream, c3 = (uint32_t)(stream >> 32);
        uint32_t a = k0, b = k1;
#pragma unroll
        for (int r = 0; r < 10; ++r) {
            const uint32_t hi0 = __umulhi(0xD2511F53u, c0), lo0 = 0xD2511F53u * c0;
            const uint32_t hi1 = __umulhi(0xCD9E8D57u, c2), lo1 = 0xCD9E8D57u * c2;
            const uint32_t n0 = hi1 ^ c1 ^ a, n2 = hi0 ^ c3 ^ b;
            c0 = n0; c1 = lo1; c2 = n2; c3 = lo0;
            a += 0x9E3779B9u; b += 0xBB67AE85u;
        }
        return make_uint4(c0, c1, c2, c3);
    }
};

__device__ __forceinline__ double u01(uint32_t hi, uint32_t lo)
{
    const uint64_t x = (((uint64_t)hi << 32) | lo) >> 11;
    return ((double)x + 0.5) * 0x1p-53;
}

__device__ __forceinline__ void box_muller(uint4 r, double& n0, double& n1)
{
    const double u1 = u01(r.x, r.y), u2 = u01(r.z, r.w);
    const double rad = sqrt(-2.0 * log(u1));
    double s, c;
    sincospi(2.0 * u2, &s, &c);
    n0 = rad * c;
    n1 = rad * s;
}

__device__ inline double gamma_mt(double a, const Philox& ph, uint64_t stream)
{
    uint64_t ctr = 0;
    double boost = 1.0;
    if (a < 1.0) {
        const uint4 r = ph(ctr++, stream);
        boost = pow(u01(r.x, r.y), 1.0 / a);
        a += 1.0;
    }
    const double d = a - 1.0 / 3.0, c = 1.0 / sqrt(9.0 * d);
    for (int it = 0; it < 1000; ++it) {
        double x, x2;
        box_muller(ph(ctr++, stream), x, x2);
        const uint4 r = ph(ctr++, stream);
        const double u = u01(r.x, r.y);
        double v = 1.0 + c * x;
        if (v <= 0.0) { x = x2; v = 1.0 + c * x; if (v <= 0.0) continue; }
        v = v * v * v;
        if (log(u) < 0.5 * x * x + d * (1.0 - v + log(v))) return boost * d * v;
    }
    return boost * d;
}

__device__ __forceinline__ int l_of_real(int64_t i, int L)
{
    if (i <= L) return (int)i;
    const int64_t id = (i + L + 1) >> 1;
    const double b = 2.0 * L + 3.0;
    int mm = (int)floor((b - sqrt(b * b - 8.0 * (double)id)) * 0.5);
    if (mm < 0) mm = 0;
    if (mm > L) mm = L;
    while (mm > 0 && (int64_t)mm * (2 * L + 1 - mm) / 2 + mm > id) --mm;
    while (mm < L && (int64_t)(mm + 1) * (2 * L + 1 - (mm + 1)) / 2 + (mm + 1) <= id) ++mm;
    return (int)(id - (int64_t)mm * (2 * L + 1 - mm) / 2);
}
```

### gibbssampler_b200/csrc/solver.cu

```cuda
#include <math.h>
#include <string.h>

#include <algorithm>

#include "gs_internal.h"
#include "rng.cuh"

#define SV_NT 256
#define SV_GRID (148 * 4)

struct PcgState {
    double delta, pq, rr, rz, d0, alpha, beta, eps2;
    int iter, itermax, done;
    unsigned counter;
};

struct gs_pcg_ws {
    double *r[2], *p[2], *q[2];
    const unsigned short* lof;
    double* ic_l[2];
    double* pre_l[2];
    double* partials;
    double* red;
    PcgState* state;
    PcgState* host_state;
};

template <int NR>
__device__ bool grid_reduce(double (&v)[NR], double* partials, unsigned* counter, double (&tot)[NR])
{
    __shared__ double sm[NR][SV_NT / 32];
    __shared__ bool last;
    const int lane = threadIdx.x & 31, w = threadIdx.x >> 5;
#pragma unroll
    for (int k = 0; k < NR; ++k) {
        double s = v[k];
        for (int o = 16; o; o >>= 1) s += __shfl_xor_sync(0xffffffffu, s, o);
        if (lane == 0) sm[k][w] = s;
    }
    __syncthreads();
    if (threadIdx.x == 0) {
#pragma unroll
        for (int k = 0; k < NR; ++k) {
            double s = 0.0;
            for (int i = 0; i < SV_NT / 32; ++i) s += sm[k][i];
            partials[blockIdx.x * NR + k] = s;
        }
        __threadfence();
        const unsigned t = atomicInc(counter, gridDim.x - 1);
        last = (t == gridDim.x - 1);
    }
    __syncthreads();
    if (!last) return false;
    __threadfence();
#pragma unroll
    for (int k = 0; k < NR; ++k) {
        double s = 0.0;
        for (int i = threadIdx.x; i < (int)gridDim.x; i += blockDim.x) s += partials[i * NR + k];
        for (int o = 16; o; o >>= 1) s += __shfl_xor_sync(0xffffffffu, s, o);
        __syncthreads();
        if (lane == 0) sm[k][w] = s;
        __syncthreads();
        double t = 0.0;
        for (int i = 0; i < SV_NT / 32; ++i) t += sm[k][i];
        tot[k] = t;
    }
    return true;
}

__global__ void precond_kernel(const double* __restrict__ dl, const double* __restrict__ bl, double ninv, int L,
                               double* __restrict__ invc_l, double* __restrict__ pre_l)
{
    const int l = blockIdx.x * blockDim.x + threadIdx.x;
    if (l > L) return;
    double c = dl[l];
    if (l) c = c * 2.0 * 3.14159265358979323846 / ((double)l * (double)(l + 1));
    const double ic = c != 0.0 ? 1.0 / c : 0.0;
    const double d = ic + bl[l] * bl[l] * ninv;
    invc_l[l] = ic;
    pre_l[l] = d != 0.0 ? 1.0 / d : 0.0;
}

__device__ __forceinline__ void pick(int64_t i, int64_t n, int& c, int64_t& j)
{
    c = i >= n;
    j = c ? i - n : i;
}

__device__ __forceinline__ void fin_init(PcgState* s, double rr, double rz)
{
    s->rr = rr; s->d0 = rr; s->delta = rz; s->iter = 0;
    s->done = (rr <= 0.0 || s->itermax <= 0) ? 1 : 0;
}
__device__ __forceinline__ void fin_apq(PcgState* s, double pq)
{
    s->pq = pq;
    s->alpha = pq != 0.0 ? s->delta / pq : 0.0;
}
__device__ __forceinline__ void fin_update(PcgState* s, double rr, double rz)
{
    s->rr = rr; s->rz = rz;
    s->beta = s->delta != 0.0 ? rz / s->delta : 0.0;
    s->delta = rz;
    s->iter += 1;
    if (rr <= s->eps2 * s->d0 || s->iter >= s->itermax) s->done = 1;
}
__global__ void pcg_scalar_kernel(gs_pcg_ws W, int stage)
{
    PcgState* s = W.state;
    if (stage == 0) fin_init(s, W.red[0], W.red[1]);
    else if (s->done) return;
    else if (stage == 1) fin_apq(s, W.red[0]);
    else fin_update(s, W.red[0], W.red[1]);
}

__global__ void __launch_bounds__(SV_NT)
pcg_init_kernel(gs_pcg_ws W, const double* bE, const double* bB, int have_q, int64_t n, int nc)
{
    double v[2] = {0.0, 0.0};
    for (int64_t i = blockIdx.x * (int64_t)blockDim.x + threadIdx.x; i < nc * n; i += (int64_t)gridDim.x * blockDim.x) {
        int c; int64_t j;
        pick(i, n, c, j);
        double r = (c ? bB : bE)[j];
        if (have_q) r -= (c ? W.q[1] : W.q[0])[j];
        const double z = (c ? W.pre_l[1] : W.pre_l[0])[W.lof[j]] * r;
        (c ? W.r[1] : W.r[0])[j] = r;
        (c ? W.p[1] : W.p[0])[j] = z;
        v[0] += r * r;
        v[1] += r * z;
    }
    double tot[2];
    if (grid_reduce<2>(v, W.partials, &W.state->counter, tot) && threadIdx.x == 0) {
        if (W.red) { W.red[0] = tot[0]; W.red[1] = tot[1]; }
        else fin_init(W.state, tot[0], tot[1]);
    }
}

#define SV_U 4

__global__ void __launch_bounds__(SV_NT) pcg_apq_kernel(gs_pcg_ws W, int64_t n, int nc)
{
    if (W.state->done) return;
    double v[1] = {0.0};
    const int64_t stride = (int64_t)gridDim.x * blockDim.x, total = nc * n;
    for (int64_t i0 = blockIdx.x * (int64_t)blockDim.x + threadIdx.x; i0 < total; i0 += SV_U * stride) {
        double p[SV_U], q[SV_U], ic[SV_U];
#pragma unroll
        for (int k = 0; k < SV_U; ++k) {
            const int64_t i = i0 + k * stride;
            int c; int64_t j;
            pick(i, n, c, j);
            const bool ok = i < total;
            p[k] = ok ? (c ? W.p[1] : W.p[0])[j] : 0.0; q[k] = ok ? (c ? W.q[1] : W.q[0])[j] : 0.0;
            ic[k] = ok ? __ldg((c ? W.ic_l[1] : W.ic_l[0]) + W.lof[j]) : 0.0;
        }
#pragma unroll
        for (int k = 0; k < SV_U; ++k) {
            const int64_t i = i0 + k * stride;
            if (i >= total) break;
            int c; int64_t j;
            pick(i, n, c, j);
            const double qq = fma(ic[k], p[k], q[k]);
            (c ? W.q[1] : W.q[0])[j] = qq;
            v[0] += p[k] * qq;
        }
    }
    double tot[1];
    if (grid_reduce<1>(v, W.partials, &W.state->counter, tot) && threadIdx.x == 0) {
        if (W.red) W.red[0] = tot[0];
        else fin_apq(W.state, tot[0]);
    }
}

__global__ void __launch_bounds__(SV_NT) pcg_update_kernel(gs_pcg_ws W, double* xE, double* xB, int64_t n, int nc)
{
    if (W.state->done) return;
    const double alpha = W.state->alpha;
    double v[2] = {0.0, 0.0};
    const int64_t stride = (int64_t)gridDim.x * blockDim.x, total = nc * n;
    for (int64_t i0 = blockIdx.x * (int64_t)blockDim.x + threadIdx.x; i0 < total; i0 += SV_U * stride) {
        double x[SV_U], p[SV_U], q[SV_U], r[SV_U], pre[SV_U];
#pragma unroll
        for (int k = 0; k < SV_U; ++k) {
            const int64_t i = i0 + k * stride;
            int c; int64_t j;
            pick(i, n, c, j);
            const bool ok = i < total;
            x[k] = ok ? (c ? xB : xE)[j] : 0.0; p[k] = ok ? (c ? W.p[1] : W.p[0])[j] : 0.0; q[k] = ok ? (c ? W.q[1] : W.q[0])[j] : 0.0;
            r[k] = ok ? (c ? W.r[1] : W.r[0])[j] : 0.0; pre[k] = ok ? __ldg((c ? W.pre_l[1] : W.pre_l[0]) + W.lof[j]) : 0.0;
        }
#pragma unroll
        for (int k = 0; k < SV_U; ++k) {
            const int64_t i = i0 + k * stride;
            if (i >= total) break;
            int c; int64_t j;
            pick(i, n, c, j);
            (c ? xB : xE)[j] = fma(alpha, p[k], x[k]);
            const double rr = fma(-alpha, q[k], r[k]);
            (c ? W.r[1] : W.r[0])[j] = rr;
            v[0] += rr * rr;
            v[1] += rr * rr * pre[k];
        }
    }
    double tot[2];
    if (grid_reduce<2>(v, W.partials, &W.state->counter, tot) && threadIdx.x == 0) {
        if (W.red) { W.red[0] = tot[0]; W.red[1] = tot[1]; }
        else fin_update(W.state, tot[0], tot[1]);
    }
}

__global__ void __launch_bounds__(SV_NT) pcg_dir_kernel(gs_pcg_ws W, int64_t n, int nc)
{
    if (W.state->done) return;
    const double beta = W.state->beta;
    const int64_t stride = (int64_t)gridDim.x * blockDim.x, total = nc * n;
    for (int64_t i0 = blockIdx.x * (int64_t)blockDim.x + threadIdx.x; i0 < total; i0 += SV_U * stride) {
        double p[SV_U], r[SV_U], pre[SV_U];
#pragma unroll
        for (int k = 0; k < SV_U; ++k) {
            const int64_t i = i0 + k * stride;
            int c; int64_t j;
            pick(i, n, c, j);
            const bool ok = i < total;
            p[k] = ok ? (c ? W.p[1] : W.p[0])[j] : 0.0; r[k] = ok ? (c ? W.r[1] : W.r[0])[j] : 0.0;
            pre[k] = ok ? __ldg((c ? W.pre_l[1] : W.pre_l[0]) + W.lof[j]) : 0.0;
        }
#pragma unroll
        for (int k = 0; k < SV_U; ++k) {
            const int64_t i = i0 + k * stride;
            if (i >= total) break;
            int c; int64_t j;
            pick(i, n, c, j);
            (c ? W.p[1] : W.p[0])[j] = fma(beta, p[k], pre[k] * r[k]);
        }
    }
}

__global__ void zero2_kernel(double* a, double* b, int64_t n)
{
    for (int64_t i = blockIdx.x * (int64_t)blockDim.x + threadIdx.x; i < n; i += (int64_t)gridDim.x * blockDim.x) {
        a[i] = 0.0;
        b[i] = 0.0;
    }
}

__global__ void add_cinv_kernel(const double* q, const double* __restrict__ ic_l, const unsigned short* __restrict__ lof,
                                const double* __restrict__ x, double* y, int64_t n)
{
    for (int64_t i = blockIdx.x * (int64_t)blockDim.x + threadIdx.x; i < n; i += (int64_t)gridDim.x * blockDim.x)
        y[i] = fma(ic_l[lof[i]], x[i], q[i]);
}

__global__ void scale_map_kernel(const double* __restrict__ a, const double* __restrict__ w, double* __restrict__ out, int64_t n)
{
    for (int64_t i = blockIdx.x * (int64_t)blockDim.x + threadIdx.x; i < n; i += (int64_t)gridDim.x * blockDim.x) out[i] = a[i] * w[i];
}

__global__ void rhs_combine_kernel(double* rhs, const double* sic, const double* xi, const double* bdata, double resc, int64_t n)
{
    for (int64_t i = blockIdx.x * (int64_t)blockDim.x + threadIdx.x; i < n; i += (int64_t)gridDim.x * blockDim.x)
        rhs[i] = fma(resc, rhs[i], fma(sic[i], xi[i], bdata[i]));
}

__global__ void lof_build_kernel(unsigned short* __restrict__ lof, const int* __restrict__ l_of_loc, int L, int64_t n)
{
    for (int64_t i = blockIdx.x * (int64_t)blockDim.x + threadIdx.x; i < n; i += (int64_t)gridDim.x * blockDim.x)
        lof[i] = (unsigned short)(l_of_loc ? l_of_loc[i] : l_of_real(i, L));
}
static bool build_lof(gs_plan* p, const unsigned short** out)
{
    void* d = nullptr;
    const int64_t n = p->nreal_loc;
    if (cudaMalloc(&d, (size_t)n * sizeof(unsigned short)) != cudaSuccess) return false;
    p->owned.push_back(d);
    lof_build_kernel<<<SV_GRID, SV_NT>>>((unsigned short*)d, p->world > 1 ? p->d.sh.l_of_loc : nullptr, p->d.lmax, n);
    if (cudaDeviceSynchronize() != cudaSuccess) return false;
    *out = (const unsigned short*)d;
    return true;
}

static bool alloc_owned(gs_plan* p, double** q, size_t cnt)
{
    void* d = nullptr;
    if (cudaMalloc(&d, cnt * sizeof(double)) != cudaSuccess) return false;
    p->owned.push_back(d);
    *q = (double*)d;
    return true;
}

static bool alloc_state(gs_plan* p, PcgState** state, PcgState** host_state)
{
    void* d = nullptr;
    if (cudaMalloc(&d, sizeof(PcgState)) != cudaSuccess) return false;
    p->owned.push_back(d);
    *state = (PcgState*)d;
    return cudaMallocHost((void**)host_state, 2 * sizeof(PcgState)) == cudaSuccess;
}

static gs_pcg_ws* get_ws(gs_plan* p)
{
    if (p->pcg_ws) return (gs_pcg_ws*)p->pcg_ws;
    gs_pcg_ws* w = new gs_pcg_ws();
    const size_t n = (size_t)p->nreal_loc;
    w->red = p->world > 1 ? p->red_loc : nullptr;
    bool ok = true;
    const size_t L1 = (size_t)p->d.lmax + 1;
    for (int c = 0; c < 2 && ok; ++c)
        ok = alloc_owned(p, &w->r[c], n) && alloc_owned(p, &w->p[c], n) && alloc_owned(p, &w->q[c], n) && alloc_owned(p, &w->ic_l[c], L1) &&
             alloc_owned(p, &w->pre_l[c], L1);
    ok = ok && alloc_owned(p, &w->partials, SV_GRID * 2) && build_lof(p, &w->lof);
    ok = ok && alloc_state(p, &w->state, &w->host_state);
    if (!ok) { gs_set_error("PCG workspace allocation failed: %s", cudaGetErrorString(cudaGetLastError())); delete w; return nullptr; }
    p->pcg_ws = w;
    return w;
}

static gs_pcg_ws* get_ws_batch(gs_plan* p)
{
    if (p->pcg_ws_batch) return (gs_pcg_ws*)p->pcg_ws_batch;
    gs_pcg_ws* w = new gs_pcg_ws[2]();
    const size_t n = (size_t)p->nreal_loc, L1 = (size_t)p->d.lmax + 1;
    double *P = nullptr, *Q = nullptr;
    bool ok = alloc_owned(p, &P, 4 * n) && alloc_owned(p, &Q, 4 * n);
    for (int k = 0; k < 2 && ok; ++k) {
        w[k].red = nullptr;
        for (int c = 0; c < 2 && ok; ++c) {
            w[k].p[c] = P + (2 * k + c) * n;
            w[k].q[c] = Q + (2 * k + c) * n;
            ok = alloc_owned(p, &w[k].r[c], n) && alloc_owned(p, &w[k].ic_l[c], L1) && alloc_owned(p, &w[k].pre_l[c], L1);
        }
        ok = ok && alloc_owned(p, &w[k].partials, SV_GRID * 2);
        if (ok) { if (k == 0) ok = build_lof(p, &w[0].lof); else w[1].lof = w[0].lof; }
        ok = ok && alloc_state(p, &w[k].state, &w[k].host_state);
    }
    void* d = nullptr;
    ok = ok && cudaMalloc(&d, sizeof(int)) == cudaSuccess;
    if (ok) { p->owned.push_back(d); p->pcg_alldone = (int*)d; }
    if (!ok) { gs_set_error("batched PCG workspace allocation failed: %s", cudaGetErrorString(cudaGetLastError())); delete[] w; return nullptr; }
    p->pcg_ws_batch = w;
    return w;
}

static void teb_ws_free(gs_plan* p);
void gs_pcg_ws_free(gs_plan* p)
{
    teb_ws_free(p);
    gs_pcg_ws* w = (gs_pcg_ws*)p->pcg_ws;
    if (w) {
        if (w->host_state) cudaFreeHost(w->host_state);
        delete w;
        p->pcg_ws = nullptr;
    }
    gs_pcg_ws* b = (gs_pcg_ws*)p->pcg_ws_batch;
    if (b) {
        for (int k = 0; k < 2; ++k) if (b[k].host_state) cudaFreeHost(b[k].host_state);
        delete[] b;
        p->pcg_ws_batch = nullptr;
    }
}

int g_gs_pcg_graph = 1;
extern "C" int gs_set_pcg_graph(int on) { const int old = g_gs_pcg_graph; g_gs_pcg_graph = on ? 1 : 0; return old; }
int g_gs_ring_fused = 1;
extern "C" int gs_set_ring_fused(int fused) { const int old = g_gs_ring_fused; g_gs_ring_fused = fused ? 1 : 0; return old; }

int g_gs_ring_skip = 1;
int g_gs_ring_const = 1;
extern "C" int gs_set_ring_const(int on) { const int old = g_gs_ring_const; g_gs_ring_const = on ? 1 : 0; return old; }
extern "C" int gs_set_ring_skip(int on) { const int old = g_gs_ring_skip; g_gs_ring_skip = on ? 1 : 0; return old; }

struct ActiveRings {
    gs_plan* p;
    bool on;
    ActiveRings(gs_plan* p_) : p(p_), on(false) {}
    int begin(const double* pixw, cudaStream_t st)
    {
        if (!g_gs_ring_skip || !pixw) return GS_OK;
        int rc = gs_active_rings_build(p, pixw, st);
        if (rc == GS_OK) { p->use_act = true; on = true; }
        return rc;
    }
    ~ActiveRings() { if (on) p->use_act = false; }
};

static int apply_noise_op(gs_plan* p, const double* vE, const double* vB, const double* bl, const double* inv_noise,
                          double* qE, double* qB, cudaStream_t st, const int* skip, int spin = 2, int nc = 1, int64_t stride = 0)
{
    int rc;
    if ((rc = gs_leg_synth(p, spin, vE, vB, GS_ALM_REAL, bl, st, skip, nullptr, nc, stride))) return rc;
    if (g_gs_ring_fused || nc > 1) {
        if ((rc = gs_ring_apply(p, spin, inv_noise, st, skip, nc))) return rc;
    } else {
        if ((rc = gs_ring_synth(p, spin, p->mapQ_tmp, p->mapU_tmp, st, skip))) return rc;
        if ((rc = gs_ring_anal(p, spin, p->mapQ_tmp, p->mapU_tmp, inv_noise, st, skip))) return rc;
    }
    return gs_leg_anal(p, spin, qE, qB, GS_ALM_REAL, bl, 1.0, 0, st, skip, nc, stride);
}

template <class Iteration>
static int pcg_poll_loop(gs_plan* p, cudaStream_t st, PcgState* state, PcgState* host_state, bool dist, double eps, int itermax,
                         int check_every, Iteration& iteration, int* n_iter_out, double* resid_out)
{
    int rc = GS_OK;
    int launched = 0;
    bool finished = false;
    cudaGraphExec_t gexec = nullptr;
    long long launches_per_graph = 0;
    if (g_gs_pcg_graph && !dist && itermax >= check_every) {
        if (!p->work_stream) {
            cudaStream_t ws = nullptr;
            GS_CHECK_CUDA(cudaStreamCreateWithFlags(&ws, cudaStreamNonBlocking));
            p->work_stream = ws;
            cudaEvent_t ev = nullptr;
            GS_CHECK_CUDA(cudaEventCreateWithFlags(&ev, cudaEventDisableTiming));
            p->work_event = ev;
        }
        cudaStream_t ws = (cudaStream_t)p->work_stream;
        GS_CHECK_CUDA(cudaEventRecord((cudaEvent_t)p->work_event, st));
        GS_CHECK_CUDA(cudaStreamWaitEvent(ws, (cudaEvent_t)p->work_event, 0));
        st = ws;
        cudaGraph_t graph = nullptr;
        const long long l0 = g_gs_launches;
        GS_CHECK_CUDA(cudaStreamBeginCapture(st, cudaStreamCaptureModeThreadLocal));
        rc = GS_OK;
        for (int k = 0; k < check_every && rc == GS_OK; ++k) rc = iteration(st);
        cudaError_t ce = cudaStreamEndCapture(st, &graph);
        launches_per_graph = g_gs_launches - l0;
        g_gs_launches = l0;
        if (rc != GS_OK) { if (graph) cudaGraphDestroy(graph); return rc; }
        if (ce != cudaSuccess) { gs_set_error("PCG graph capture: %s", cudaGetErrorString(ce)); return GS_E_CUDA; }
        ce = cudaGraphInstantiate(&gexec, graph, 0);
        cudaGraphDestroy(graph);
        if (ce != cudaSuccess) { gs_set_error("PCG graph instantiate: %s", cudaGetErrorString(ce)); return GS_E_CUDA; }
    }
    if (gexec) {
        PcgState* hs = host_state;
        cudaEvent_t ev[2] = {nullptr, nullptr};
        cudaError_t ce = cudaEventCreateWithFlags(&ev[0], cudaEventDisableTiming);
        if (ce == cudaSuccess) ce = cudaEventCreateWithFlags(&ev[1], cudaEventDisableTiming);
        int cur = 0, inflight = 0;
        while (ce == cudaSuccess && !finished) {
            while (ce == cudaSuccess && inflight < 2 && launched + check_every <= itermax) {
                const int sl = (cur + inflight) & 1;
                ce = cudaGraphLaunch(gexec, st);
                if (ce == cudaSuccess) ce = cudaMemcpyAsync(hs + sl, state, sizeof(PcgState), cudaMemcpyDeviceToHost, st);
                if (ce == cudaSuccess) ce = cudaEventRecord(ev[sl], st);
                launched += check_every;
                g_gs_launches += launches_per_graph;
                ++inflight;
// ... 31 lines not shown
    if (resid_out) *resid_out = s.d0 > 0.0 ? sqrt(s.rr / s.d0) : 0.0;
    if (s.d0 > 0.0 && s.rr > s.eps2 * s.d0) {
        gs_set_error("PCG stopped at iter_max = %d with |r|/|r0| = %.3e > eps = %.1e", itermax, sqrt(s.rr / s.d0), eps);
        return GS_E_NOTCONVERGED;
    }
    return GS_OK;
}

static int cr_pcg_impl(gs_plan* p, int spin, const double* dl_EE, const double* dl_BB, const double* bl,
                       const double* inv_noise, double ninv_sum_over_4pi, const double* rhs_E,
                       const double* rhs_B, double* x_E, double* x_B, int warm_start, double eps, int itermax,
                       int check_every, int* n_iter_out, double* resid_out, void* stream)
{
    const int nc = spin ? 2 : 1;
    GS_REQUIRE(eps > 0.0 && itermax >= 0, "eps must be > 0 and itermax >= 0");
    GS_CHECK_CUDA(cudaSetDevice(p->device));
    cudaStream_t st = (cudaStream_t)stream;
    gs_pcg_ws* w = get_ws(p);
    if (!w) return GS_E_NOMEM;
    const int L = p->d.lmax;
    const int64_t n = p->nreal_loc;
    if (check_every < 1) check_every = 8;

    const int lb = (L + 256) / 256;
    precond_kernel<<<lb, 256, 0, st>>>(dl_EE, bl, ninv_sum_over_4pi, L, w->ic_l[0], w->pre_l[0]);
    if (nc == 2) precond_kernel<<<lb, 256, 0, st>>>(dl_BB, bl, ninv_sum_over_4pi, L, w->ic_l[1], w->pre_l[1]);
    GS_CHECK_LAUNCH();
    int rc;
    const bool dist = p->world > 1;
    ActiveRings act(p);
    if ((rc = act.begin(inv_noise, st))) return rc;

    PcgState h;
    memset(&h, 0, sizeof(h));
    h.eps2 = eps * eps;
    h.itermax = itermax;
    *w->host_state = h;
    GS_CHECK_CUDA(cudaMemcpyAsync(w->state, w->host_state, sizeof(PcgState), cudaMemcpyHostToDevice, st));
    if (warm_start) {
        if ((rc = apply_noise_op(p, x_E, x_B, bl, inv_noise, w->q[0], w->q[1], st, nullptr, spin))) return rc;
        add_cinv_kernel<<<SV_GRID, SV_NT, 0, st>>>(w->q[0], w->ic_l[0], w->lof, x_E, w->q[0], n);
        if (nc == 2) add_cinv_kernel<<<SV_GRID, SV_NT, 0, st>>>(w->q[1], w->ic_l[1], w->lof, x_B, w->q[1], n);
    } else {
        zero2_kernel<<<SV_GRID, SV_NT, 0, st>>>(x_E, nc == 2 ? x_B : x_E, n);
    }
    pcg_init_kernel<<<SV_GRID, SV_NT, 0, st>>>(*w, rhs_E, rhs_B, warm_start ? 1 : 0, n, nc);
    GS_CHECK_LAUNCH();
    if (dist) {
        if ((rc = gs_shard_allreduce(p, w->red, 2, st))) return rc;
        pcg_scalar_kernel<<<1, 1, 0, st>>>(*w, 0);
    }

    const int* done = &w->state->done;
    auto iteration = [&](cudaStream_t s) -> int {
        int r;
        if ((r = apply_noise_op(p, w->p[0], w->p[1], bl, inv_noise, w->q[0], w->q[1], s, done, spin))) return r;
        pcg_apq_kernel<<<SV_GRID, SV_NT, 0, s>>>(*w, n, nc);
        if (dist) {
            if ((r = gs_shard_allreduce(p, w->red, 1, s))) return r;
            pcg_scalar_kernel<<<1, 1, 0, s>>>(*w, 1);
        }
        pcg_update_kernel<<<SV_GRID, SV_NT, 0, s>>>(*w, x_E, x_B, n, nc);
        if (dist) {
            if ((r = gs_shard_allreduce(p, w->red, 2, s))) return r;
            pcg_scalar_kernel<<<1, 1, 0, s>>>(*w, 2);
        }
        pcg_dir_kernel<<<SV_GRID, SV_NT, 0, s>>>(*w, n, nc);
        GS_CHECK_LAUNCH();
        g_gs_launches += 3;
        return GS_OK;
    };
    return pcg_poll_loop(p, st, w->state, w->host_state, dist, eps, itermax, check_every, iteration, n_iter_out, resid_out);
}

extern "C" int gs_cr_pcg_pol(gs_plan* p, const double* dl_EE, const double* dl_BB, const double* bl,
                             const double* inv_noise, double ninv_sum_over_4pi, const double* rhs_E,
                             const double* rhs_B, double* x_E, double* x_B, int warm_start, double eps, int itermax,
                             int check_every, int* n_iter_out, double* resid_out, void* stream)
{
    if (!p) { gs_set_error("null plan"); return GS_E_BADARG; }
    GS_REQUIRE(dl_EE && dl_BB && bl && inv_noise && rhs_E && rhs_B && x_E && x_B, "null pointer argument");
    return cr_pcg_impl(p, 2, dl_EE, dl_BB, bl, inv_noise, ninv_sum_over_4pi, rhs_E, rhs_B, x_E, x_B, warm_start, eps, itermax,
                       check_every, n_iter_out, resid_out, stream);
}

__global__ void pcg_alldone_kernel(const PcgState* a, const PcgState* b, int* out) { *out = (a->done && b->done) ? 1 : 0; }

extern "C" int gs_cr_pcg_pol_batch(gs_plan* p, int n_chain, const double* dl_EE, const double* dl_BB, const double* bl,
                                   const double* inv_noise, double ninv_sum_over_4pi, const double* rhs_E,
                                   const double* rhs_B, double* x_E, double* x_B, int64_t stride, double eps, int itermax,
                                   int check_every, int* n_iter_out, double* resid_out, void* stream)
{
    if (!p) { gs_set_error("null plan"); return GS_E_BADARG; }
    GS_REQUIRE(dl_EE && dl_BB && bl && inv_noise && rhs_E && rhs_B && x_E && x_B, "null pointer argument");
    GS_REQUIRE(n_chain == 1 || n_chain == 2, "n_chain must be 1 or 2");
    const int L = p->d.lmax;
    if (n_chain == 1)
        return cr_pcg_impl(p, 2, dl_EE, dl_BB, bl, inv_noise, ninv_sum_over_4pi, rhs_E, rhs_B, x_E, x_B, 0, eps, itermax, check_every,
                           n_iter_out, resid_out, stream);
    GS_REQUIRE(p->world == 1, "chain batches need an unsharded plan");
    GS_REQUIRE(eps > 0.0 && itermax >= 0, "eps must be > 0 and itermax >= 0");
    GS_CHECK_CUDA(cudaSetDevice(p->device));
    int rc;
    if ((rc = gs_plan_reserve_chains(p, 2))) return rc;
    cudaStream_t st = (cudaStream_t)stream;
    gs_pcg_ws* W = get_ws_batch(p);
    if (!W) return GS_E_NOMEM;
    const int64_t n = p->nreal_loc;
    if (check_every < 1) check_every = 8;
    const int lb = (L + 256) / 256;
    ActiveRings act(p);
    if ((rc = act.begin(inv_noise, st))) return rc;
    for (int k = 0; k < 2; ++k) {
        gs_pcg_ws* w = &W[k];
        precond_kernel<<<lb, 256, 0, st>>>(dl_EE + k * (L + 1), bl, ninv_sum_over_4pi, L, w->ic_l[0], w->pre_l[0]);
        precond_kernel<<<lb, 256, 0, st>>>(dl_BB + k * (L + 1), bl, ninv_sum_over_4pi, L, w->ic_l[1], w->pre_l[1]);
        GS_CHECK_LAUNCH();
        PcgState h;
        memset(&h, 0, sizeof(h));
        h.eps2 = eps * eps;
        h.itermax = itermax;
        *w->host_state = h;
        GS_CHECK_CUDA(cudaMemcpyAsync(w->state, w->host_state, sizeof(PcgState), cudaMemcpyHostToDevice, st));
        zero2_kernel<<<SV_GRID, SV_NT, 0, st>>>(x_E + k * stride, x_B + k * stride, n);
        pcg_init_kernel<<<SV_GRID, SV_NT, 0, st>>>(*w, rhs_E + k * stride, rhs_B + k * stride, 0, n, 2);
        GS_CHECK_LAUNCH();
    }
    pcg_alldone_kernel<<<1, 1, 0, st>>>(W[0].state, W[1].state, p->pcg_alldone);
    const int64_t bstride = 2 * n;
    bool done[2] = {false, false};
    int launched = 0;
    while (!(done[0] && done[1]) && launched < itermax) {
        for (int it = 0; it < check_every && launched < itermax; ++it, ++launched) {
            if (!done[0] && !done[1]) {
                if ((rc = apply_noise_op(p, W[0].p[0], W[0].p[1], bl, inv_noise, W[0].q[0], W[0].q[1], st, p->pcg_alldone, 2, 2, bstride))) return rc;
            } else {
                gs_pcg_ws* w = &W[done[0] ? 1 : 0];
                if ((rc = apply_noise_op(p, w->p[0], w->p[1], bl, inv_noise, w->q[0], w->q[1], st, &w->state->done, 2))) return rc;
            }
            for (int k = 0; k < 2; ++k) {
                if (done[k]) continue;
                pcg_apq_kernel<<<SV_GRID, SV_NT, 0, st>>>(W[k], n, 2);
                pcg_update_kernel<<<SV_GRID, SV_NT, 0, st>>>(W[k], x_E + k * stride, x_B + k * stride, n, 2);
                pcg_dir_kernel<<<SV_GRID, SV_NT, 0, st>>>(W[k], n, 2);
                g_gs_launches += 3;
            }
            if (!done[0] && !done[1]) { pcg_alldone_kernel<<<1, 1, 0, st>>>(W[0].state, W[1].state, p->pcg_alldone); g_gs_launches += 1; }
            GS_CHECK_LAUNCH();
        }
        for (int k = 0; k < 2; ++k) GS_CHECK_CUDA(cudaMemcpyAsync(W[k].host_state, W[k].state, sizeof(PcgState), cudaMemcpyDeviceToHost, st));
        GS_CHECK_CUDA(cudaStreamSynchronize(st));
        for (int k = 0; k < 2; ++k) done[k] = W[k].host_state->done != 0;
    }
    int ret = GS_OK;
    for (int k = 0; k < 2; ++k) {
        const PcgState& sdone = *W[k].host_state;
        if (n_iter_out) n_iter_out[k] = sdone.iter;
        if (resid_out) resid_out[k] = sdone.d0 > 0.0 ? sqrt(sdone.rr / sdone.d0) : 0.0;
        if (sdone.d0 > 0.0 && sdone.rr > sdone.eps2 * sdone.d0) {
            gs_set_error("PCG (chain %d of the batch) stopped at iter_max = %d with |r|/|r0| = %.3e > eps = %.1e", k, itermax, sqrt(sdone.rr / sdone.d0), eps);
            ret = GS_E_NOTCONVERGED;
        }
    }
    return ret;
}

extern "C" int gs_cr_pcg_tt(gs_plan* p, const double* dl_TT, const double* bl, const double* inv_noise,
                            double ninv_sum_over_4pi, const double* rhs, double* x, int warm_start, double eps, int itermax,
                            int check_every, int* n_iter_out, double* resid_out, void* stream)
{
    if (!p) { gs_set_error("null plan"); return GS_E_BADARG; }
    GS_REQUIRE(dl_TT && bl && inv_noise && rhs && x, "null pointer argument");
    return cr_pcg_impl(p, 0, dl_TT, nullptr, bl, inv_noise, ninv_sum_over_4pi, rhs, nullptr, x, nullptr, warm_start, eps, itermax,
                       check_every, n_iter_out, resid_out, stream);
}

extern "C" int gs_cr_apply_q_tt(gs_plan* p, const double* dl_TT, const double* bl, const double* inv_noise, const double* x,
                                double* y, void* stream)
{
    if (!p) { gs_set_error("null plan"); return GS_E_BADARG; }
    GS_REQUIRE(dl_TT && bl && inv_noise && x && y, "null pointer argument");
    GS_CHECK_CUDA(cudaSetDevice(p->device));
    cudaStream_t st = (cudaStream_t)stream;
    gs_pcg_ws* w = get_ws(p);
    if (!w) return GS_E_NOMEM;
    int rc;
    ActiveRings act(p);
    if ((rc = act.begin(inv_noise, st))) return rc;
    const int L = p->d.lmax;
    precond_kernel<<<(L + 256) / 256, 256, 0, st>>>(dl_TT, bl, 0.0, L, w->ic_l[0], w->pre_l[0]);
    if ((rc = apply_noise_op(p, x, nullptr, bl, inv_noise, w->q[0], nullptr, st, nullptr, 0))) return rc;
    add_cinv_kernel<<<SV_GRID, SV_NT, 0, st>>>(w->q[0], w->ic_l[0], w->lof, x, y, p->nreal_loc);
    GS_CHECK_LAUNCH();
    return GS_OK;
// ... 294 lines not shown
        double fTT, fTE, fEE;
        if (b == 0.0) {
            fTT = a != 0.0 ? sqrt(1.0 / a) : 0.0;
            fTE = 0.0;
            fEE = d != 0.0 ? sqrt(1.0 / d) : 0.0;
        } else {
            const double l11 = sqrt(a), l21 = b / l11, l22 = sqrt(d - l21 * l21);
            fTT = 1.0 / l11;
            fTE = -l21 / (l11 * l22);
            fEE = 1.0 / l22;
        }
        const double fBB = e != 0.0 ? sqrt(1.0 / e) : 0.0;
        const double xt = xiT[j], xe = xiE[j], xb = xiB[j];
        rT[j] = fma(resc, rT[j], fma(fTT, xt, fma(fTE, xe, bdT[j])));
        rE[j] = fma(resc, rE[j], fma(fEE, xe, bdE[j]));
        rB[j] = fma(resc, rB[j], fma(fBB, xb, bdB[j]));
    }
}

static TebWs* get_ws_teb(gs_plan* p)
{
    if (p->pcg_ws_teb) return (TebWs*)p->pcg_ws_teb;
    gs_pcg_ws* base = get_ws(p);
    if (!base) return nullptr;
    TebWs* w = new TebWs();
    const size_t n = (size_t)p->nreal_loc;
    bool ok = true;
    for (int c = 0; c < 3 && ok; ++c) ok = alloc_owned(p, &w->r[c], n) && alloc_owned(p, &w->p[c], n) && alloc_owned(p, &w->q[c], n);
    ok = ok && alloc_owned(p, &w->tab, (size_t)TEB_TAB * (p->d.lmax + 1)) && alloc_owned(p, &w->partials, SV_GRID * 2);
    w->lof = base->lof;
    ok = ok && alloc_state(p, &w->state, &w->host_state);
    if (!ok) { gs_set_error("joint T/E/B workspace allocation failed: %s", cudaGetErrorString(cudaGetLastError())); delete w; return nullptr; }
    p->pcg_ws_teb = w;
    return w;
}

static void teb_ws_free(gs_plan* p)
{
    TebWs* w = (TebWs*)p->pcg_ws_teb;
    if (!w) return;
    if (w->host_state) cudaFreeHost(w->host_state);
    delete w;
    p->pcg_ws_teb = nullptr;
}

static void swap_flags(gs_plan* p)
{
    RingFlags& f = p->flags_T;
    std::swap(p->act_ring, f.act_ring);
    std::swap(p->act_pairs, f.act_pairs);
    std::swap(p->act_count, f.act_count);
    std::swap(p->act_slot0, f.act_slot0);
    std::swap(p->ring_wconst, f.ring_wconst);
    std::swap(p->groups0_dyn, f.groups0_dyn);
    std::swap(p->groups2_dyn, f.groups2_dyn);
}

static int alloc_flags_T(gs_plan* p)
{
    RingFlags& f = p->flags_T;
    if (f.act_ring) return GS_OK;
    const int L1 = p->d.lmax + 1;
    auto alloc = [&](void** q, size_t bytes) { void* d = nullptr; if (cudaMalloc(&d, std::max<size_t>(16, bytes)) != cudaSuccess) return false; p->owned.push_back(d); *q = d; return true; };
    bool ok = alloc((void**)&f.act_ring, (size_t)p->d.nring) && alloc((void**)&f.act_pairs, (size_t)p->d.npair * sizeof(int)) &&
              alloc((void**)&f.act_count, sizeof(int)) && alloc((void**)&f.act_slot0, (size_t)2 * L1 * sizeof(int)) &&
              alloc((void**)&f.ring_wconst, (size_t)p->d.nring * sizeof(double)) &&
              alloc((void**)&f.groups0_dyn, (size_t)p->ngroups0 * sizeof(int2)) && alloc((void**)&f.groups2_dyn, (size_t)p->ngroups2 * sizeof(int2));
    if (!ok) { memset(&f, 0, sizeof(f)); gs_set_error("ring flag allocation failed: %s", cudaGetErrorString(cudaGetLastError())); return GS_E_NOMEM; }
    return GS_OK;
}

struct TebRings {
    gs_plan* p;
    ActiveRings act;
    bool two;
    TebRings(gs_plan* p_) : p(p_), act(p_), two(false) {}
    int begin(const double* invT, const double* invP, cudaStream_t st)
    {
        int rc = act.begin(invP, st);
        if (rc || !act.on || invT == invP) return rc;
        if ((rc = alloc_flags_T(p))) return rc;
        swap_flags(p);
        rc = gs_active_rings_build(p, invT, st);
        swap_flags(p);
        two = rc == GS_OK;
        return rc;
    }
};

static int teb_noise_op(gs_plan* p, TebRings& tr, const double* vT, const double* vE, const double* vB, const double* bl,
                        const double* invT, const double* invP, double* qT, double* qE, double* qB, cudaStream_t st, const int* skip)
{
    if (tr.two) swap_flags(p);
    int rc = apply_noise_op(p, vT, nullptr, bl, invT, qT, nullptr, st, skip, 0);
    if (tr.two) swap_flags(p);
    if (rc) return rc;
    return apply_noise_op(p, vE, vB, bl, invP, qE, qB, st, skip, 2);
}

static int teb_unsharded(gs_plan* p, const char* who)
{
    if (p->world > 1) {
        gs_set_error("%s: the joint T/E/B solve needs an unsharded plan (this plan is sharded over %d ranks)", who, p->world);
        return GS_E_BADARG;
    }
    return GS_OK;
}

extern "C" int gs_cr_pcg_teb(gs_plan* p, const double* dl_TT, const double* dl_TE, const double* dl_EE, const double* dl_BB,
                             const double* bl, const double* inv_noise_T, const double* inv_noise_P, double ninvT_sum_over_4pi,
                             double ninvP_sum_over_4pi, const double* rhs_T, const double* rhs_E, const double* rhs_B, double* x_T,
                             double* x_E, double* x_B, int warm_start, double eps, int itermax, int check_every, int* n_iter_out,
                             double* resid_out, void* stream)
{
    if (!p) { gs_set_error("null plan"); return GS_E_BADARG; }
    GS_REQUIRE(dl_TT && dl_TE && dl_EE && dl_BB && bl && inv_noise_T && inv_noise_P && rhs_T && rhs_E && rhs_B && x_T && x_E && x_B,
               "null pointer argument");
    GS_REQUIRE(eps > 0.0 && itermax >= 0, "eps must be > 0 and itermax >= 0");
    int rc;
// ... 130 lines not shown
        for (int k = 0; k < 5 && rc == GS_OK; ++k) {
            for (int rep = -1; rep < nrep && rc == GS_OK; ++rep) {
                if (k >= 2 && (cudaMemsetAsync(p->partial, 0, flush_bytes, st) != cudaSuccess ||
                               cudaMemsetAsync(scratch, 0, sizeof(PcgState), st) != cudaSuccess)) { rc = GS_E_CUDA; break; }
                cudaEventRecord(e0, st);
                if (k == 0) {
                    if (tr.two) swap_flags(p);
                    rc = apply_noise_op(p, w->p[0], nullptr, bl, inv_noise_T, w->q[0], nullptr, st, nullptr, 0);
                    if (tr.two) swap_flags(p);
                } else if (k == 1) {
                    rc = apply_noise_op(p, w->p[1], w->p[2], bl, inv_noise_P, w->q[1], w->q[2], st, nullptr, 2);
                } else if (k == 2) {
                    teb_apq_kernel<<<SV_GRID, SV_NT, 0, st>>>(v, n);
                } else if (k == 3) {
                    teb_update_kernel<<<SV_GRID, SV_NT, 0, st>>>(v, x[0], x[1], x[2], n);
                } else {
                    teb_dir_kernel<<<SV_GRID, SV_NT, 0, st>>>(v, n);
                }
                cudaEventRecord(e1, st);
                if (cudaEventSynchronize(e1) != cudaSuccess) { rc = GS_E_CUDA; break; }
                float ms = 0;
                cudaEventElapsedTime(&ms, e0, e1);
                if (rep >= 0) acc[k] += ms;
            }
        }
    }
    if (rc == GS_E_CUDA) gs_set_error("gs_profile_matvec_teb: %s", cudaGetErrorString(cudaGetLastError()));
    for (int k = 0; k < 5; ++k) ms_out[k] = (float)(acc[k] / nrep);
    if (e0) cudaEventDestroy(e0);
    if (e1) cudaEventDestroy(e1);
    cudaFree(scratch);
    return rc;
}

long long g_gs_launches = 0;
extern "C" long long gs_launch_count(void) { return g_gs_launches; }

extern "C" int gs_profile_matvec(gs_plan* p, const double* x_E, const double* x_B, const double* bl,
                                 const double* inv_noise, double* y_E, double* y_B, int nrep, float* ms_out,
                                 void* stream)
{
    if (!p) { gs_set_error("null plan"); return GS_E_BADARG; }
    GS_REQUIRE(x_E && x_B && bl && inv_noise && y_E && y_B && ms_out && nrep >= 1, "bad arguments");
    GS_CHECK_CUDA(cudaSetDevice(p->device));
    cudaStream_t st = (cudaStream_t)stream;
    cudaEvent_t ev[5];
    for (int i = 0; i < 5; ++i) GS_CHECK_CUDA(cudaEventCreate(&ev[i]));
    double acc[4] = {0, 0, 0, 0};
    int rc = GS_OK;
    ActiveRings act(p);
    if ((rc = act.begin(inv_noise, st))) { for (int i = 0; i < 5; ++i) cudaEventDestroy(ev[i]); return rc; }
    for (int r = 0; r < nrep && rc == GS_OK; ++r) {
        cudaEventRecord(ev[0], st);
        rc = gs_leg_synth(p, 2, x_E, x_B, GS_ALM_REAL, bl, st);
        cudaEventRecord(ev[1], st);
        if (!rc) rc = g_gs_ring_fused ? gs_ring_apply(p, 2, inv_noise, st) : gs_ring_synth(p, 2, p->mapQ_tmp, p->mapU_tmp, st);
        cudaEventRecord(ev[2], st);
        if (!rc && !g_gs_ring_fused) rc = gs_ring_anal(p, 2, p->mapQ_tmp, p->mapU_tmp, inv_noise, st);
        cudaEventRecord(ev[3], st);
        if (!rc) rc = gs_leg_anal(p, 2, y_E, y_B, GS_ALM_REAL, bl, 1.0, 0, st);
        cudaEventRecord(ev[4], st);
        if (cudaEventSynchronize(ev[4]) != cudaSuccess) { gs_set_error("gs_profile_matvec: %s", cudaGetErrorString(cudaGetLastError())); rc = GS_E_CUDA; break; }
        for (int i = 0; i < 4; ++i) { float ms = 0; cudaEventElapsedTime(&ms, ev[i], ev[i + 1]); acc[i] += ms; }
    }
    for (int i = 0; i < 4; ++i) ms_out[i] = (float)(acc[i] / nrep);
    if (g_gs_ring_fused) ms_out[2] = 0.0f;
    for (int i = 0; i < 5; ++i) cudaEventDestroy(ev[i]);
    return rc;
}

extern "C" int gs_profile_matvec_batch(gs_plan* p, int n_chain, const double* x_E, const double* x_B, int64_t stride,
                                       const double* bl, const double* inv_noise, double* y_E, double* y_B, int nrep,
                                       float* ms_out, void* stream)
{
    if (!p) { gs_set_error("null plan"); return GS_E_BADARG; }
    GS_REQUIRE(x_E && x_B && bl && inv_noise && y_E && y_B && ms_out && nrep >= 1 && (n_chain == 1 || n_chain == 2), "bad arguments");
    GS_CHECK_CUDA(cudaSetDevice(p->device));
    int rc;
    if (n_chain > 1 && (rc = gs_plan_reserve_chains(p, n_chain))) return rc;
    cudaStream_t st = (cudaStream_t)stream;
    cudaEvent_t ev[4];
    for (int i = 0; i < 4; ++i) GS_CHECK_CUDA(cudaEventCreate(&ev[i]));
    double acc[3] = {0, 0, 0};
    rc = GS_OK;
    {
        ActiveRings act(p);
        rc = act.begin(inv_noise, st);
        for (int r = 0; r < nrep && rc == GS_OK; ++r) {
            cudaEventRecord(ev[0], st);
            rc = gs_leg_synth(p, 2, x_E, x_B, GS_ALM_REAL, bl, st, nullptr, nullptr, n_chain, stride);
            cudaEventRecord(ev[1], st);
            if (!rc) rc = gs_ring_apply(p, 2, inv_noise, st, nullptr, n_chain);
            cudaEventRecord(ev[2], st);
            if (!rc) rc = gs_leg_anal(p, 2, y_E, y_B, GS_ALM_REAL, bl, 1.0, 0, st, nullptr, n_chain, stride);
            cudaEventRecord(ev[3], st);
            if (cudaEventSynchronize(ev[3]) != cudaSuccess) { gs_set_error("gs_profile_matvec_batch: %s", cudaGetErrorString(cudaGetLastError())); rc = GS_E_CUDA; break; }
            for (int i = 0; i < 3; ++i) { float ms = 0; cudaEventElapsedTime(&ms, ev[i], ev[i + 1]); acc[i] += ms; }
        }
    }
    for (int i = 0; i < 3; ++i) ms_out[i] = (float)(acc[i] / nrep);
    for (int i = 0; i < 4; ++i) cudaEventDestroy(ev[i]);
    return rc;
}

extern "C" int gs_profile_pcg_vectors(gs_plan* p, int spin, int nrep, float* ms_out, void* stream)
{
    if (!p) { gs_set_error("null plan"); return GS_E_BADARG; }
    GS_REQUIRE(ms_out && nrep >= 1 && (spin == 0 || spin == 2), "bad arguments");
    GS_CHECK_CUDA(cudaSetDevice(p->device));
    cudaStream_t st = (cudaStream_t)stream;
    gs_pcg_ws* w = get_ws(p);
    if (!w) return GS_E_NOMEM;
    const int nc = spin ? 2 : 1;
    const int64_t n = p->nreal_loc;
    for (int c = 0; c < 2; ++c) {
        double* arrs[3] = {w->r[c], w->p[c], w->q[c]};
        for (double* a : arrs) GS_CHECK_CUDA(cudaMemsetAsync(a, 0, (size_t)n * sizeof(double), st));
        double* tabs[2] = {w->ic_l[c], w->pre_l[c]};
        for (double* a : tabs) GS_CHECK_CUDA(cudaMemsetAsync(a, 0, (size_t)(p->d.lmax + 1) * sizeof(double), st));
    }
    GS_CHECK_CUDA(cudaMemsetAsync(p->almE_tmp, 0, (size_t)n * sizeof(double), st));
    GS_CHECK_CUDA(cudaMemsetAsync(p->almB_tmp, 0, (size_t)n * sizeof(double), st));
    GS_CHECK_CUDA(cudaMemsetAsync(w->state, 0, sizeof(PcgState), st));
    double* red = nullptr;
    GS_CHECK_CUDA(cudaMalloc(&red, 2 * sizeof(double)));
    gs_pcg_ws v = *w;
    v.red = red;
    cudaEvent_t e0 = nullptr, e1 = nullptr;
    int rc = GS_OK;
    if (cudaEventCreate(&e0) != cudaSuccess || cudaEventCreate(&e1) != cudaSuccess) rc = GS_E_CUDA;
    const size_t flush_bytes = (size_t)p->anal_chunks * (size_t)(p->world > 1 ? p->d.sh.nalm_loc : p->d.nalm) * 4 * sizeof(double);
    for (int k = 0; k < 3 && rc == GS_OK; ++k) {
        double acc = 0.0;
        for (int rep = -2; rep < nrep; ++rep) {
            if (cudaMemsetAsync(p->partial, 0, flush_bytes, st) != cudaSuccess) { rc = GS_E_CUDA; break; }
            cudaEventRecord(e0, st);
            if (k == 0) pcg_apq_kernel<<<SV_GRID, SV_NT, 0, st>>>(v, n, nc);
            else if (k == 1) pcg_update_kernel<<<SV_GRID, SV_NT, 0, st>>>(v, p->almE_tmp, p->almB_tmp, n, nc);
            else pcg_dir_kernel<<<SV_GRID, SV_NT, 0, st>>>(v, n, nc);
            cudaEventRecord(e1, st);
            if (cudaEventSynchronize(e1) != cudaSuccess) { rc = GS_E_CUDA; break; }
            float ms = 0;
            cudaEventElapsedTime(&ms, e0, e1);
// ... 80 lines not shown
```

### include/gibbs_b200.h

```cpp
#ifndef GIBBS_B200_H
#define GIBBS_B200_H

#include <stddef.h>
#include <stdint.h>

#ifdef __cplusplus
extern "C" {
#endif

#define GS_OK 0
#define GS_E_BADARG (-1)
#define GS_E_CUDA (-2)
#define GS_E_NOTCONVERGED (-3)
#define GS_E_NCCL (-4)
#define GS_E_NOMEM (-5)

#define GS_ALM_COMPLEX 0
#define GS_ALM_REAL 1

typedef struct gs_plan gs_plan;

const char* gs_last_error_string(void);
int gs_version(void);

// ... 5 lines not shown
int64_t gs_plan_npix(const gs_plan* plan);
int64_t gs_plan_nalm(const gs_plan* plan);
int64_t gs_plan_nreal(const gs_plan* plan);

int gs_alm2map_spin0(gs_plan* plan, const double* alm, int layout, const double* fl, double* map,
                     void* stream);

int gs_alm2map_spin2(gs_plan* plan, const double* almE, const double* almB, int layout,
                     const double* fl, double* mapQ, double* mapU, void* stream);

int gs_map2alm_spin0(gs_plan* plan, const double* map, const double* pixw, int iter, int adjoint,
                     const double* fl, double* alm, int layout, void* stream);

int gs_map2alm_spin2(gs_plan* plan, const double* mapQ, const double* mapU, const double* pixw,
                     int iter, int adjoint, const double* fl, double* almE, double* almB,
                     int layout, void* stream);

int gs_alm2map_batch(gs_plan* plan, int spin, int n_chain, const double* almE, const double* almB,
                     int64_t alm_stride, int layout, const double* fl, double* mapQ, double* mapU,
                     int64_t map_stride, void* stream);
int gs_map2alm_batch(gs_plan* plan, int spin, int n_chain, const double* mapQ, const double* mapU,
                     int64_t map_stride, const double* pixw, int adjoint, const double* fl, double* almE,
                     double* almB, int64_t alm_stride, int layout, void* stream);

int gs_real_to_complex(const double* real_alm, double* complex_alm, int lmax, void* stream);
int gs_complex_to_real(const double* complex_alm, double* real_alm, int lmax, void* stream);
int gs_expand_per_l(const double* x, int lmax, int mode, double* out, void* stream);
int gs_unfold_bins(const double* binned, const int* bins, int nbins, double* out, int nout,
                   void* stream);
int gs_almxfl(const double* alm, int layout, int lmax, const double* fl, double* out, void* stream);
int gs_alm2cl(const double* alm, int layout, int lmax, double* cl, void* stream);

int gs_alm2map_spin2_fl2(gs_plan* plan, const double* almE, const double* almB, int layout,
                         const double* flE, const double* flB, double* mapQ, double* mapU,
                         void* stream);

int gs_cr_rhs_pol(gs_plan* plan, const double* dl_EE, const double* dl_BB, const double* bl,
                  const double* inv_noise, const double* sqrt_inv_noise, const double* bdata_E,
                  const double* bdata_B, const double* d_Q, const double* d_U, const double* xi_Q,
                  const double* xi_U, const double* xi_E, const double* xi_B, int fluct_iter,
                  double* rhs_E, double* rhs_B, void* stream);

int gs_cr_pcg_pol(gs_plan* plan, const double* dl_EE, const double* dl_BB, const double* bl,
                  const double* inv_noise, double ninv_sum_over_4pi, const double* rhs_E,
                  const double* rhs_B, double* x_E, double* x_B, int warm_start, double eps,
                  int itermax, int check_every, int* n_iter_out, double* resid_out, void* stream);

int gs_cr_pcg_pol_batch(gs_plan* plan, int n_chain, const double* dl_EE, const double* dl_BB, const double* bl,
                        const double* inv_noise, double ninv_sum_over_4pi, const double* rhs_E,
                        const double* rhs_B, double* x_E, double* x_B, int64_t stride, double eps, int itermax,
                        int check_every, int* n_iter_out, double* resid_out, void* stream);

int gs_set_pcg_graph(int on);

int gs_cr_apply_q_pol(gs_plan* plan, const double* dl_EE, const double* dl_BB, const double* bl,
                      const double* inv_noise, const double* x_E, const double* x_B, double* y_E,
                      double* y_B, void* stream);

int gs_cr_rhs_tt(gs_plan* plan, const double* dl_TT, const double* bl, const double* inv_noise,
                 const double* sqrt_inv_noise, const double* bdata, const double* d, const double* xi_alm,
                 const double* xi_pix, int fluct_iter, double* rhs, void* stream);
int gs_cr_pcg_tt(gs_plan* plan, const double* dl_TT, const double* bl, const double* inv_noise,
                 double ninv_sum_over_4pi, const double* rhs, double* x, int warm_start, double eps, int itermax,
                 int check_every, int* n_iter_out, double* resid_out, void* stream);
int gs_cr_apply_q_tt(gs_plan* plan, const double* dl_TT, const double* bl, const double* inv_noise,
                     const double* x, double* y, void* stream);

int gs_cr_rhs_teb(gs_plan* plan, const double* dl_TT, const double* dl_TE, const double* dl_EE, const double* dl_BB,
                  const double* bl, const double* inv_noise_T, const double* sqrt_inv_noise_T, const double* inv_noise_P,
                  const double* sqrt_inv_noise_P, const double* bdata_T, const double* bdata_E, const double* bdata_B,
                  const double* d_I, const double* d_Q, const double* d_U, const double* xi_I, const double* xi_Q,
                  const double* xi_U, const double* xi_T, const double* xi_E, const double* xi_B, int fluct_iter,
                  double* rhs_T, double* rhs_E, double* rhs_B, void* stream);
int gs_cr_pcg_teb(gs_plan* plan, const double* dl_TT, const double* dl_TE, const double* dl_EE, const double* dl_BB,
                  const double* bl, const double* inv_noise_T, const double* inv_noise_P, double ninvT_sum_over_4pi,
                  double ninvP_sum_over_4pi, const double* rhs_T, const double* rhs_E, const double* rhs_B, double* x_T,
                  double* x_E, double* x_B, int warm_start, double eps, int itermax, int check_every, int* n_iter_out,
                  double* resid_out, void* stream);
int gs_cr_apply_q_teb(gs_plan* plan, const double* dl_TT, const double* dl_TE, const double* dl_EE, const double* dl_BB,
                      const double* bl, const double* inv_noise_T, const double* inv_noise_P, const double* x_T,
                      const double* x_E, const double* x_B, double* y_T, double* y_E, double* y_B, void* stream);

int gs_cr_direct(const double* dl, const double* bl, const double* d_alm, const double* xi,
                 double npix_over_noise_4pi, int lmax, int mode, double* out, void* stream);

int gs_cr_direct_pix(const double* dl, const double* bl, const double* bsum, const double* xi,
                     double npix_over_noise_4pi, int lmax, int l_cut, int zero_low, double* out, void* stream);

int gs_cls_invgamma(const double* cl_hat, const int* bins, int nbins, const double* gamma_inject,
                    uint64_t seed, uint64_t call, double* dl_binned, double* alpha_out,
                    double* beta_out, void* stream);

int gs_truncnorm_propose(const double* dl_old, const double* prop_var, int nbins, const double* u,
                         double* dl_new, void* stream);
int gs_truncnorm_logpdf(const double* x, const double* from, const double* prop_var, int nbins,
                        double* out, void* stream);
int gs_loglik_pix(const double* d_Q, const double* d_U, const double* m_Q, const double* m_U,
                  const double* inv_noise, int64_t npix, double* scratch, double* out, void* stream);
int gs_loglik_alm(const double* d_E, const double* d_B, const double* s_E, const double* s_B, const double* fl_E,
                  const double* fl_B, int lmax, double weight, double* scratch, double* out, void* stream);

int gs_mwg_filters(const double* cur_E, const double* cur_B, const double* prop_E, const double* prop_B,
                   const int* bins_E, int nbins_E, const int* bins_B, int nbins_B, int pol, int b_start,
                   int b_end, const double* bl, int lmax, int l_cut, double* flE, double* flB,
                   void* stream);
int gs_mwg_accept(double* cur, const double* prop, const double* logr, int b_start, int b_end,
// ... 95 lines not shown
```

Baseline: 2.786.

## Fuse Legendre finish into PCG tail and apply ring scaling directly in synthesis

Result: no change. 2.768, median of 6 (-0.7%).

```diff
diff --git a/gibbssampler_b200/_lib.py b/gibbssampler_b200/_lib.py
--- a/gibbssampler_b200/_lib.py
+++ b/gibbssampler_b200/_lib.py
@@ -44,6 +44,7 @@
     "gs_cr_pcg_pol_batch": (_i, [_vp, _i, _vp, _vp, _vp, _vp, _d, _vp, _vp, _vp, _vp, _i64, _d, _i, _i,
                                  C.POINTER(_i), C.POINTER(_d), _vp]),
     "gs_set_pcg_graph": (_i, [_i]),
+    "gs_set_pcg_tail": (_i, [_i]),
     "gs_cr_apply_q_pol": (_i, [_vp] * 10),
     "gs_cr_rhs_tt": (_i, [_vp] * 9 + [_i, _vp, _vp]),
     "gs_cr_pcg_tt": (_i, [_vp, _vp, _vp, _vp, _d, _vp, _vp, _i, _d, _i, _i, C.POINTER(_i), C.POINTER(_d), _vp]),
diff --git a/gibbssampler_b200/csrc/gs_internal.h b/gibbssampler_b200/csrc/gs_internal.h
--- a/gibbssampler_b200/csrc/gs_internal.h
+++ b/gibbssampler_b200/csrc/gs_internal.h
@@ -107,6 +107,7 @@
     int* act_count;
     int* act_slot0;
     double* ring_wconst;
+    double* ring_sdir;
     int2* groups0_dyn;
     int2* groups2_dyn;
 };
@@ -151,6 +152,7 @@
     double* act_red;
     int* act_slot0;
     double* ring_wconst;
+    double* ring_sdir;
     bool use_act;
     double2* Fm;
     double* partial;
@@ -180,10 +182,81 @@
 extern long long g_gs_launches;
 static inline int64_t gs_nalm(int lmax) { return (int64_t)(lmax + 1) * (lmax + 2) / 2; }
 
+#ifdef __CUDACC__
+__device__ __forceinline__ double2 ring_phase(const PlanDev& P, int ring, int m)
+{
+    const int q = P.ring_phq[ring], den = P.ring_phden[ring];
+    const unsigned r = ((unsigned)m * (unsigned)q) % (2u * (unsigned)den);
+    double s, c;
+    sincospi((double)r / (double)den, &s, &c);
+    return make_double2(c, s);
+}
+
+__device__ __forceinline__ double2 ring_direct(const PlanDev& P, int ring, int m, double s, double2 a)
+{
+    if (m == 0) a.y = 0.0;
+    else if (2 * m == P.ring_nphi[ring]) {
+        const double2 e2 = ring_phase(P, ring, 2 * m);
+        const double2 t = make_double2(a.x * e2.x - a.y * e2.y, a.x * e2.y + a.y * e2.x);
+        a = make_double2(a.x + t.x, a.y - t.y);
+    }
+    return make_double2(s * a.x, s * a.y);
+}
+
+__device__ __forceinline__ int leg_finish_chunks(const PlanDev& P, const int* pcount, const int* slot0, int m, int cp)
+{
+    const int nact = (pcount ? *pcount : P.npair) - slot0[m];
+    return nact > 0 ? (nact + cp - 1) / cp : 0;
+}
+template <int SPIN>
+__device__ __forceinline__ double leg_finish_post(const PlanDev& P, int64_t id, int l, int m, const double* fl, double scale, int layout)
+{
+    double post = scale * (SPIN ? -0.5 * P.alpha2[id] : P.alpha0[id]);
+    if (fl) post *= fl[l];
+    if (layout == GS_ALM_REAL && m > 0) post *= 1.41421356237309504880;
+    return post;
+}
+template <int SPIN>
+__device__ __forceinline__ double leg_finish_one(const double* __restrict__ partial, int nchunk, int64_t pn, int64_t pid, double post, int comp)
+{
+    constexpr int NV = SPIN ? 4 : 2;
+    if constexpr (SPIN == 0) {
+        double v = 0.0;
+        for (int k = 0; k < nchunk; ++k) v += partial[((int64_t)k * pn + pid) * NV + comp];
+        return v * post;
+    } else {
+        const int a = comp == 0 ? 0 : comp == 3 ? 1 : 2, b = comp == 0 ? 1 : comp == 3 ? 0 : 3;
+        double va = 0.0, vb = 0.0;
+        for (int k = 0; k < nchunk; ++k) {
+            const double* q = partial + ((int64_t)k * pn + pid) * NV;
+            va += q[a];
+            vb += q[b];
+        }
+        return (comp < 2 ? va + vb : va - vb) * post;
+    }
+}
+template <int SPIN>
+__device__ __forceinline__ void leg_finish_coef(const double* __restrict__ partial, int nchunk, int64_t pn, int64_t pid, double post,
+                                                double (&v)[SPIN ? 4 : 2])
+{
+#pragma unroll
+    for (int c = 0; c < (SPIN ? 4 : 2); ++c) v[c] = leg_finish_one<SPIN>(partial, nchunk, pn, pid, post, c);
+}
+#endif
+
 int gs_leg_synth(gs_plan* p, int spin, const double* almE, const double* almB, int layout, const double* fl,
-                 cudaStream_t st, const int* skip = nullptr, const double* flB = nullptr, int nc = 1, int64_t alm_stride = 0);
+                 cudaStream_t st, const int* skip = nullptr, const double* flB = nullptr, int nc = 1, int64_t alm_stride = 0,
+                 const double* rscale = nullptr);
 int gs_leg_anal(gs_plan* p, int spin, double* almE, double* almB, int layout, const double* fl, double scale,
-                int accumulate, cudaStream_t st, const int* skip = nullptr, int nc = 1, int64_t alm_stride = 0);
+                int accumulate, cudaStream_t st, const int* skip = nullptr, int nc = 1, int64_t alm_stride = 0, int finish = 1);
+struct LegFinishArgs {
+    const double* partial;
+    int64_t part_stride;
+    int cp;
+    const int* pcount;
+    const int* slot0;
+};
+LegFinishArgs gs_leg_finish_args(const gs_plan* p, int spin, int nc);
 int64_t gs_fm_stride(const gs_plan* p);
 int64_t gs_part_stride(const gs_plan* p, int nc);
 int gs_active_rings_build(gs_plan* p, const double* pixw, cudaStream_t st);
@@ -195,6 +268,7 @@
 int gs_ring_anal(gs_plan* p, int spin, const double* mapQ, const double* mapU, const double* pixw, cudaStream_t st,
                  const int* skip = nullptr, int nc = 1, int64_t map_stride = 0);
 int gs_ring_apply(gs_plan* p, int spin, const double* pixw, cudaStream_t st, const int* skip = nullptr, int nc = 1);
+const double* gs_ring_direct_scale(const gs_plan* p, int spin, const double* pixw);
 int gs_ring_synth_batch(gs_plan* p, const double2* F, int64_t f_stride, const int* mmax, double* mapQ, double* mapU,
                         int64_t map_stride, int nb, cudaStream_t st, const unsigned char* ract = nullptr, const double* wconst = nullptr);
 int gs_ring_order_build(gs_plan* p, cudaStream_t st);
diff --git a/gibbssampler_b200/csrc/legendre.cu b/gibbssampler_b200/csrc/legendre.cu
--- a/gibbssampler_b200/csrc/legendre.cu
+++ b/gibbssampler_b200/csrc/legendre.cu
@@ -265,7 +265,7 @@
 leg_synth_kernel(PlanDev P, const double* __restrict__ almE, const double* __restrict__ almB, int layout,
                  const double* __restrict__ fl, const double* __restrict__ flB, double2* __restrict__ Fm,
                  const int* __restrict__ skip, const int* __restrict__ plist, const int* __restrict__ pcount,
-                 const int* __restrict__ slot0, int64_t alm_stride, int64_t fm_stride, int mk0)
+                 const int* __restrict__ slot0, int64_t alm_stride, int64_t fm_stride, int mk0, const double* __restrict__ rscale)
 {
     if (skip && *skip) return;
     const int L = P.lmax, mk = blockIdx.y + mk0, m = SH ? P.sh.mlist[mk] : mk, tid = threadIdx.x;
@@ -434,20 +434,29 @@
         if (p < 0) continue;
         const int rn = p, rs = P.nring - 1 - p;
         const int64_t in = fm_index<SH>(P, 0, rn, m, mk), is = fm_index<SH>(P, 0, rs, m, mk);
+        double scn = __longlong_as_double(0x7ff8000000000000LL), scs = scn;
+        if (rscale && ((myact >> j) & 1u)) { scn = rscale[rn]; scs = rscale[rs]; }
+        const bool dn = scn == scn, ds = scs == scs;
 #pragma unroll
         for (int c = 0; c < NC; ++c) {
             const SynthAcc<SPIN>& a = acc[j][c];
             double2* F = Fm + c * fm_stride;
             if (SPIN == 0) {
-                F[in] = make_double2(a.sqr + a.aqr, a.sqi + a.aqi);
-                if (rs != rn) F[is] = make_double2(sg * (a.sqr - a.aqr), sg * (a.sqi - a.aqi));
+                const double2 vn = make_double2(a.sqr + a.aqr, a.sqi + a.aqi);
+                F[in] = dn ? ring_direct(P, rn, m, scn, vn) : vn;
+                if (rs != rn) {
+                    const double2 vs = make_double2(sg * (a.sqr - a.aqr), sg * (a.sqi - a.aqi));
+                    F[is] = ds ? ring_direct(P, rs, m, scs, vs) : vs;
+                }
             } else {
                 const int64_t cs = SH ? (int64_t)P.sh.RL * P.sh.MLb : (int64_t)P.nring * (L + 1);
-                F[in] = make_double2(a.sqr + a.sqi, a.sur + a.sui);
-                F[in + cs] = make_double2(a.sur - a.sui, a.sqi - a.sqr);
+                const double2 qn = make_double2(a.sqr + a.sqi, a.sur + a.sui), un = make_double2(a.sur - a.sui, a.sqi - a.sqr);
+                F[in] = dn ? ring_direct(P, rn, m, scn, qn) : qn;
+                F[in + cs] = dn ? ring_direct(P, rn, m, scn, un) : un;
                 if (rs != rn) {
-                    F[is] = make_double2(sg * (a.aqr + a.aqi), sg * (a.aur + a.aui));
-                    F[is + cs] = make_double2(sg * (a.aur - a.aui), sg * (a.aqi - a.aqr));
+                    const double2 qs = make_double2(sg * (a.aqr + a.aqi), sg * (a.aur + a.aui)), us = make_double2(sg * (a.aur - a.aui), sg * (a.aqi - a.aqr));
+                    F[is] = ds ? ring_direct(P, rs, m, scs, qs) : qs;
+                    F[is + cs] = ds ? ring_direct(P, rs, m, scs, us) : us;
                 }
             }
         }
@@ -989,10 +998,7 @@
     partial += blockIdx.z * part_stride;
     almE += blockIdx.z * alm_stride;
     if (SPIN) almB += blockIdx.z * alm_stride;
-    {
-        const int nact = (pcount ? *pcount : P.npair) - slot0[m];
-        nchunk = nact > 0 ? (nact + chunk_pairs - 1) / chunk_pairs : 0;
-    }
+    nchunk = leg_finish_chunks(P, pcount, slot0, m, chunk_pairs);
     const int l = m + blockIdx.x * blockDim.x + threadIdx.x;
     if (l > L) return;
     const int64_t base = (int64_t)m * (2 * L + 1 - m) / 2, id = base + l;
@@ -1001,22 +1007,7 @@
     double v[NV];
 #pragma unroll
     for (int c = 0; c < NV; ++c) v[c] = 0.0;
-    if (l >= SPIN) {
-        for (int k = 0; k < nchunk; ++k) {
-            const double* q = partial + ((int64_t)k * pn + pid) * NV;
-#pragma unroll
-            for (int c = 0; c < NV; ++c) v[c] += q[c];
-        }
-        if (SPIN) {
-            const double y1 = v[0], y2 = v[1], y3 = v[2], y4 = v[3];
-            v[0] = y1 + y2; v[1] = y3 + y4; v[2] = y3 - y4; v[3] = y2 - y1;
-        }
-        double post = scale * (SPIN ? -0.5 * P.alpha2[id] : P.alpha0[id]);
-        if (fl) post *= fl[l];
-        if (layout == GS_ALM_REAL && m > 0) post *= 1.41421356237309504880;
-#pragma unroll
-        for (int c = 0; c < NV; ++c) v[c] *= post;
-    }
+    if (l >= SPIN) leg_finish_coef<SPIN>(partial, nchunk, pn, pid, leg_finish_post<SPIN>(P, id, l, m, fl, scale, layout), v);
     if (layout == GS_ALM_COMPLEX) {
         double2* E = reinterpret_cast<double2*>(almE);
         double2 e = make_double2(v[0], v[1]);
@@ -1140,10 +1131,11 @@
 }
 
 int gs_leg_synth(gs_plan* p, int spin, const double* almE, const double* almB, int layout, const double* fl,
-                 cudaStream_t st, const int* skip, const double* flB, int nc, int64_t alm_stride)
+                 cudaStream_t st, const int* skip, const double* flB, int nc, int64_t alm_stride, const double* rscale)
 {
     const bool sh = p->world > 1;
     if (sh && layout != GS_ALM_REAL) { gs_set_error("sharded plans take the (local) real alm layout only"); return GS_E_BADARG; }
+    if (sh && rscale) { gs_set_error("gs_leg_synth: ring scales need an unsharded plan"); return GS_E_BADARG; }
     int rc = check_batch(p, nc, layout, "gs_leg_synth");
     if (rc) return rc;
     const int rr = nc == 2 ? LEG_R2 : LEG_R;
@@ -1153,11 +1145,11 @@
     const int* slot0 = plist ? p->act_slot0 + (spin ? p->d.lmax + 1 : 0) : (spin ? p->d.pmin2 : p->d.pmin0);
     const int64_t fs = gs_fm_stride(p);
     if (nc == 2) {
-        if (spin == 0) leg_synth_kernel<0, LEG_R2, false, 2><<<grid, LEG_NT, 0, st>>>(p->d, almE, almB, layout, fl, flB, p->Fm, skip, plist, pcount, slot0, alm_stride, fs, 0);
-        else leg_synth_kernel<2, LEG_R2, false, 2><<<grid, LEG_NT, 0, st>>>(p->d, almE, almB, layout, fl, flB, p->Fm, skip, plist, pcount, slot0, alm_stride, fs, 0);
+        if (spin == 0) leg_synth_kernel<0, LEG_R2, false, 2><<<grid, LEG_NT, 0, st>>>(p->d, almE, almB, layout, fl, flB, p->Fm, skip, plist, pcount, slot0, alm_stride, fs, 0, rscale);
+        else leg_synth_kernel<2, LEG_R2, false, 2><<<grid, LEG_NT, 0, st>>>(p->d, almE, almB, layout, fl, flB, p->Fm, skip, plist, pcount, slot0, alm_stride, fs, 0, rscale);
     } else if (!sh) {
-        if (spin == 0) leg_synth_kernel<0, LEG_R, false, 1><<<grid, LEG_NT, 0, st>>>(p->d, almE, almB, layout, fl, flB, p->Fm, skip, plist, pcount, slot0, 0, 0, 0);
-        else leg_synth_kernel<2, LEG_R, false, 1><<<grid, LEG_NT, 0, st>>>(p->d, almE, almB, layout, fl, flB, p->Fm, skip, plist, pcount, slot0, 0, 0, 0);
+        if (spin == 0) leg_synth_kernel<0, LEG_R, false, 1><<<grid, LEG_NT, 0, st>>>(p->d, almE, almB, layout, fl, flB, p->Fm, skip, plist, pcount, slot0, 0, 0, 0, rscale);
+        else leg_synth_kernel<2, LEG_R, false, 1><<<grid, LEG_NT, 0, st>>>(p->d, almE, almB, layout, fl, flB, p->Fm, skip, plist, pcount, slot0, 0, 0, 0, rscale);
     } else {
         const ShardDev& S = p->d.sh;
         cudaStream_t comm = st;
@@ -1168,8 +1160,8 @@
             const int mk0 = b * S.MLb, cnt = std::min(S.MLb, S.nm_loc - mk0);
             if (cnt > 0) {
                 dim3 g(grid.x, cnt);
-                if (spin == 0) leg_synth_kernel<0, LEG_R, true, 1><<<g, LEG_NT, 0, st>>>(p->d, almE, almB, layout, fl, flB, p->Fm, skip, plist, pcount, slot0, 0, 0, mk0);
-                else leg_synth_kernel<2, LEG_R, true, 1><<<g, LEG_NT, 0, st>>>(p->d, almE, almB, layout, fl, flB, p->Fm, skip, plist, pcount, slot0, 0, 0, mk0);
+                if (spin == 0) leg_synth_kernel<0, LEG_R, true, 1><<<g, LEG_NT, 0, st>>>(p->d, almE, almB, layout, fl, flB, p->Fm, skip, plist, pcount, slot0, 0, 0, mk0, nullptr);
+                else leg_synth_kernel<2, LEG_R, true, 1><<<g, LEG_NT, 0, st>>>(p->d, almE, almB, layout, fl, flB, p->Fm, skip, plist, pcount, slot0, 0, 0, mk0, nullptr);
                 GS_CHECK_LAUNCH();
                 g_gs_launches += 1;
             }
@@ -1212,11 +1204,23 @@
     return GS_OK;
 }
 
+LegFinishArgs gs_leg_finish_args(const gs_plan* p, int spin, int nc)
+{
+    LegFinishArgs a;
+    a.partial = p->partial;
+    a.part_stride = gs_part_stride(p, nc);
+    a.cp = LEG_NT * (nc > 1 ? LEG_RA2 : LEG_RA);
+    a.pcount = p->use_act ? p->act_count : nullptr;
+    a.slot0 = p->use_act ? p->act_slot0 + (spin ? p->d.lmax + 1 : 0) : (spin ? p->d.pmin2 : p->d.pmin0);
+    return a;
+}
+
 int gs_leg_anal(gs_plan* p, int spin, double* almE, double* almB, int layout, const double* fl, double scale,
-                int accumulate, cudaStream_t st, const int* skip, int nc, int64_t alm_stride)
+                int accumulate, cudaStream_t st, const int* skip, int nc, int64_t alm_stride, int finish)
 {
     const bool sh = p->world > 1;
     if (sh && layout != GS_ALM_REAL) { gs_set_error("sharded plans take the (local) real alm layout only"); return GS_E_BADARG; }
+    if (sh && !finish) { gs_set_error("gs_leg_anal: sharded plans finish the analysis themselves"); return GS_E_BADARG; }
     int rc = check_batch(p, nc, layout, "gs_leg_anal");
     if (rc) return rc;
     const int nchunk = anal_chunks_of(p, nc);
@@ -1233,18 +1237,18 @@
     if (nc == 2) {
         if (spin == 0) {
             if ((rc = launch_anal<0, LEG_RA2, false, 2>(p, grid, st, skip, plist, pcount, slot0, fs, ps))) return rc;
-            leg_finish_kernel<0, false><<<fgrid, 256, 0, st>>>(p->d, p->partial, nchunk, almE, almB, layout, fl, scale, accumulate, skip, pcount, slot0, cp, ps, alm_stride);
+            if (finish) leg_finish_kernel<0, false><<<fgrid, 256, 0, st>>>(p->d, p->partial, nchunk, almE, almB, layout, fl, scale, accumulate, skip, pcount, slot0, cp, ps, alm_stride);
         } else {
             if ((rc = launch_anal<2, LEG_RA2, false, 2>(p, grid, st, skip, plist, pcount, slot0, fs, ps))) return rc;
-            leg_finish_kernel<2, false><<<fgrid, 256, 0, st>>>(p->d, p->partial, nchunk, almE, almB, layout, fl, scale, accumulate, skip, pcount, slot0, cp, ps, alm_stride);
+            if (finish) leg_finish_kernel<2, false><<<fgrid, 256, 0, st>>>(p->d, p->partial, nchunk, almE, almB, layout, fl, scale, accumulate, skip, pcount, slot0, cp, ps, alm_stride);
         }
     } else if (!sh) {
         if (spin == 0) {
             if ((rc = launch_anal<0, LEG_RA, false, 1>(p, grid, st, skip, plist, pcount, slot0, 0, 0))) return rc;
-            leg_finish_kernel<0, false><<<fgrid, 256, 0, st>>>(p->d, p->partial, nchunk, almE, almB, layout, fl, scale, accumulate, skip, pcount, slot0, cp, 0, 0);
+            if (finish) leg_finish_kernel<0, false><<<fgrid, 256, 0, st>>>(p->d, p->partial, nchunk, almE, almB, layout, fl, scale, accumulate, skip, pcount, slot0, cp, 0, 0);
         } else {
             if ((rc = launch_anal<2, LEG_RA, false, 1>(p, grid, st, skip, plist, pcount, slot0, 0, 0))) return rc;
-            leg_finish_kernel<2, false><<<fgrid, 256, 0, st>>>(p->d, p->partial, nchunk, almE, almB, layout, fl, scale, accumulate, skip, pcount, slot0, cp, 0, 0);
+            if (finish) leg_finish_kernel<2, false><<<fgrid, 256, 0, st>>>(p->d, p->partial, nchunk, almE, almB, layout, fl, scale, accumulate, skip, pcount, slot0, cp, 0, 0);
         }
     } else {
         const ShardDev& S = p->d.sh;
@@ -1273,7 +1277,7 @@
         else leg_finish_kernel<2, true><<<fgrid, 256, 0, st>>>(p->d, p->partial, nchunk, almE, almB, layout, fl, scale, accumulate, skip, pcount, slot0, cp, 0, 0);
     }
     GS_CHECK_LAUNCH();
-    g_gs_launches += 2;
+    g_gs_launches += finish ? 2 : 1;
     return GS_OK;
 }
 
diff --git a/gibbssampler_b200/csrc/plan.cu b/gibbssampler_b200/csrc/plan.cu
--- a/gibbssampler_b200/csrc/plan.cu
+++ b/gibbssampler_b200/csrc/plan.cu
@@ -228,6 +228,7 @@
     p->ring_scratch = nullptr;
     p->act_ring = nullptr;
     p->ring_wconst = nullptr;
+    p->ring_sdir = nullptr;
     p->act_pairs = nullptr;
     p->act_count = nullptr;
     p->act_slot0 = nullptr;
@@ -278,6 +279,7 @@
         if (rc == GS_OK) rc = dev_alloc(p, (size_t)2 * (lmax + 1), &p->act_slot0);
         if (rc == GS_OK) rc = dev_alloc(p, (size_t)p->d.nring, &p->act_red);
         if (rc == GS_OK && world <= 1) rc = dev_alloc(p, (size_t)p->d.nring, &p->ring_wconst);
+        if (rc == GS_OK && world <= 1) rc = dev_alloc(p, (size_t)2 * p->d.nring, &p->ring_sdir);
         if (rc == GS_OK) rc = dev_alloc(p, (size_t)p->npix_loc, &p->mapQ_tmp);
         if (rc == GS_OK) rc = dev_alloc(p, (size_t)p->npix_loc, &p->mapU_tmp);
         const size_t nre = (size_t)p->nreal_loc;
diff --git a/gibbssampler_b200/csrc/ringfft.cu b/gibbssampler_b200/csrc/ringfft.cu
--- a/gibbssampler_b200/csrc/ringfft.cu
+++ b/gibbssampler_b200/csrc/ringfft.cu
@@ -243,15 +243,6 @@
     (void)nbs;
 }
 
-__device__ __forceinline__ double2 ring_phase(const PlanDev& P, int ring, int m)
-{
-    const int q = P.ring_phq[ring], den = P.ring_phden[ring];
-    const unsigned r = ((unsigned)m * (unsigned)q) % (2u * (unsigned)den);
-    double s, c;
-    sincospi((double)r / (double)den, &s, &c);
-    return make_double2(c, s);
-}
-
 template <bool SH>
 __device__ __forceinline__ int64_t fm_ring_index(const PlanDev& P, int comp, int ring, int m)
 {
@@ -293,10 +284,34 @@
     }
     return all;
 }
-__global__ void __launch_bounds__(1024) ring_order_kernel(const RingJob* __restrict__ jobs, const int2* __restrict__ groups, int ngroups,
-                                                          const unsigned char* __restrict__ ract, const double* __restrict__ wconst,
-                                                          int2* __restrict__ groups_out)
-{
+__device__ __forceinline__ bool group_direct(const double* __restrict__ sdir, const RingJob* __restrict__ jobs, const int2* __restrict__ groups)
+{
+    if (!sdir) return false;
+    const double s = sdir[jobs[groups[blockIdx.x].x].ringA];
+    return s == s;
+}
+__global__ void __launch_bounds__(1024) ring_order_kernel(PlanDev P, int spin2, const RingJob* __restrict__ jobs, const int2* __restrict__ groups,
+                                                          int ngroups, const unsigned char* __restrict__ ract, const double* __restrict__ wconst,
+                                                          int2* __restrict__ groups_out, double* __restrict__ sdir)
+{
+    for (int gi = threadIdx.x; gi < ngroups; gi += blockDim.x) {
+        const int2 g = groups[gi];
+        bool any = false, direct = true;
+        for (int s = 0; s < g.y; ++s) {
+            const RingJob jb = jobs[g.x + s];
+            any = any || ract[jb.ringA] || (jb.ringB >= 0 && ract[jb.ringB]);
+            const double a = wconst[jb.ringA], b = jb.ringB >= 0 ? wconst[jb.ringB] : 0.0;
+            direct = direct && a == a && b == b && 2 * ring_mtop(P, jb.ringA, spin2) <= P.ring_nphi[jb.ringA];
+        }
+        direct = direct && any;
+        const double nan = __longlong_as_double(0x7ff8000000000000LL);
+        for (int s = 0; s < g.y; ++s) {
+            const RingJob jb = jobs[g.x + s];
+            sdir[jb.ringA] = direct ? (double)P.ring_nphi[jb.ringA] * wconst[jb.ringA] : nan;
+            if (jb.ringB >= 0) sdir[jb.ringB] = direct ? (double)P.ring_nphi[jb.ringA] * wconst[jb.ringB] : nan;
+        }
+    }
+
     __shared__ int wcount[32][3];
     __shared__ int base[3], total[3];
     const int tid = threadIdx.x, lane = tid & 31, w = tid >> 5;
@@ -673,10 +688,11 @@
 __global__ void __launch_bounds__(RF_NT, 2)
 ring_apply_kernel(PlanDev P, const RingJob* __restrict__ jobs, const int2* __restrict__ groups, double2* __restrict__ Fm,
                   const double* __restrict__ pixw, const int* __restrict__ skip, const unsigned char* __restrict__ ract, int spin2,
-                  int64_t f_stride, const double* __restrict__ wconst)
+                  int64_t f_stride, const double* __restrict__ wconst, const double* __restrict__ sdir)
 {
     if (skip && *skip) return;
     if (group_idle(ract, jobs, groups)) return;
+    if (group_direct(sdir, jobs, groups)) return;
     extern __shared__ double2 smem[];
     Fm += blockIdx.y * f_stride;
     double2* twq = smem;
@@ -684,33 +700,6 @@
         const RingSub S = ring_sub(P, jobs, groups, twq + (P.tw_n >> 2) + 1);
         const int mtop = ring_mtop(P, S.job.ringA, spin2);
         const double wA = wconst[S.job.ringA], wB = wconst[S.job.ringB >= 0 ? S.job.ringB : S.job.ringA];
-        bool direct = true;
-        {
-            const int2 g = groups[blockIdx.x];
-            for (int s = 0; s < g.y; ++s) {
-                const int ra = jobs[g.x + s].ringA;
-                direct = direct && 2 * ring_mtop(P, ra, spin2) <= P.ring_nphi[ra];
-            }
-        }
-        if (direct) {
-            const RingJob& job = S.job;
-            const double sa = (double)S.n * wA, sb = (double)S.n * wB;
-            for (int m = S.tid; m <= mtop; m += S.nt) {
-                const int64_t ia = fm_ring_index<SH>(P, job.compA, job.ringA, m);
-                const int64_t ib = job.ringB >= 0 ? fm_ring_index<SH>(P, job.compB, job.ringB, m) : ia;
-                double2 a = Fm[ia], b = job.ringB >= 0 ? Fm[ib] : make_double2(0.0, 0.0);
-                if (m == 0) { a.y = 0.0; b.y = 0.0; }
-                else if (2 * m == S.n) {
-                    const double2 e2 = ring_phase(P, job.ringA, 2 * m);
-                    const double2 ta = cmul(a, e2), tb = cmul(b, e2);
-                    a = make_double2(a.x + ta.x, a.y - ta.y);
-                    b = make_double2(b.x + tb.x, b.y - tb.y);
-                }
-                Fm[ia] = make_double2(sa * a.x, sa * a.y);
-                if (job.ringB >= 0) Fm[ib] = make_double2(sb * b.x, sb * b.y);
-            }
-            return;
-        }
         ring_build_Z<SH>(P, S, Fm, mtop, S.scratch, false, true);
         __syncthreads();
         const double half_n = 0.5 * (double)S.n;
@@ -1171,18 +1160,28 @@
     const int2* grp = spin == 0 ? p->groups0 : p->groups2;
     const double* wconst = (p->use_act && g_gs_ring_const) ? p->ring_wconst : nullptr;
     if (wconst) grp = spin == 0 ? p->groups0_dyn : p->groups2_dyn;
-    if (p->world > 1) ring_apply_kernel<true><<<nj, RF_NT, p->ring_smem, st>>>(p->d, jobs, grp, p->Fx, pixw, skip, p->use_act ? p->act_ring : nullptr, spin ? 1 : 0, 0, nullptr);
-    else ring_apply_kernel<false><<<dim3(nj, nc), RF_NT, p->ring_smem, st>>>(p->d, jobs, grp, p->Fm, pixw, skip, p->use_act ? p->act_ring : nullptr, spin ? 1 : 0, nc > 1 ? gs_fm_stride(p) : 0, wconst);
+    if (p->world > 1) ring_apply_kernel<true><<<nj, RF_NT, p->ring_smem, st>>>(p->d, jobs, grp, p->Fx, pixw, skip, p->use_act ? p->act_ring : nullptr, spin ? 1 : 0, 0, nullptr, nullptr);
+    else ring_apply_kernel<false><<<dim3(nj, nc), RF_NT, p->ring_smem, st>>>(p->d, jobs, grp, p->Fm, pixw, skip, p->use_act ? p->act_ring : nullptr, spin ? 1 : 0, nc > 1 ? gs_fm_stride(p) : 0, wconst,
+                                                                             gs_ring_direct_scale(p, spin, pixw));
     GS_CHECK_LAUNCH();
     g_gs_launches += 1;
     return GS_OK;
 }
 
+const double* gs_ring_direct_scale(const gs_plan* p, int spin, const double* pixw)
+{
+    const int nj = spin == 0 ? p->ngroups0 : p->ngroups2, ns = spin == 0 ? p->nsjobs0 : p->nsjobs2;
+    if (p->world > 1 || !pixw || ns > 0 || nj <= 0 || !p->use_act || !g_gs_ring_const || !p->ring_wconst) return nullptr;
+    return p->ring_sdir + (spin ? p->d.nring : 0);
+}
+
 int gs_ring_order_build(gs_plan* p, cudaStream_t st)
 {
     if (p->world > 1 || !p->ring_wconst) return GS_OK;
-    if (p->ngroups2 > 0) ring_order_kernel<<<1, 1024, 0, st>>>(p->jobs2, p->groups2, p->ngroups2, p->act_ring, p->ring_wconst, p->groups2_dyn);
-    if (p->ngroups0 > 0) ring_order_kernel<<<1, 1024, 0, st>>>(p->jobs0, p->groups0, p->ngroups0, p->act_ring, p->ring_wconst, p->groups0_dyn);
+    if (p->ngroups2 > 0)
+        ring_order_kernel<<<1, 1024, 0, st>>>(p->d, 1, p->jobs2, p->groups2, p->ngroups2, p->act_ring, p->ring_wconst, p->groups2_dyn, p->ring_sdir + p->d.nring);
+    if (p->ngroups0 > 0)
+        ring_order_kernel<<<1, 1024, 0, st>>>(p->d, 0, p->jobs0, p->groups0, p->ngroups0, p->act_ring, p->ring_wconst, p->groups0_dyn, p->ring_sdir);
     GS_CHECK_LAUNCH();
     g_gs_launches += 2;
     return GS_OK;
diff --git a/gibbssampler_b200/csrc/rng.cuh b/gibbssampler_b200/csrc/rng.cuh
--- a/gibbssampler_b200/csrc/rng.cuh
+++ b/gibbssampler_b200/csrc/rng.cuh
@@ -60,9 +60,9 @@
     return boost * d;
 }
 
-__device__ __forceinline__ int l_of_real(int64_t i, int L)
+__device__ __forceinline__ int m_of_real(int64_t i, int L)
 {
-    if (i <= L) return (int)i;
+    if (i <= L) return 0;
     const int64_t id = (i + L + 1) >> 1;
     const double b = 2.0 * L + 3.0;
     int mm = (int)floor((b - sqrt(b * b - 8.0 * (double)id)) * 0.5);
@@ -70,5 +70,12 @@
     if (mm > L) mm = L;
     while (mm > 0 && (int64_t)mm * (2 * L + 1 - mm) / 2 + mm > id) --mm;
     while (mm < L && (int64_t)(mm + 1) * (2 * L + 1 - (mm + 1)) / 2 + (mm + 1) <= id) ++mm;
+    return mm;
+}
+__device__ __forceinline__ int l_of_real(int64_t i, int L)
+{
+    if (i <= L) return (int)i;
+    const int64_t id = (i + L + 1) >> 1;
+    const int mm = m_of_real(i, L);
     return (int)(id - (int64_t)mm * (2 * L + 1 - mm) / 2);
 }
diff --git a/gibbssampler_b200/csrc/solver.cu b/gibbssampler_b200/csrc/solver.cu
--- a/gibbssampler_b200/csrc/solver.cu
+++ b/gibbssampler_b200/csrc/solver.cu
@@ -1,5 +1,7 @@
 #include <math.h>
 #include <string.h>
+
+#include <cooperative_groups.h>
 
 #include <algorithm>
 
@@ -18,19 +20,19 @@
 struct gs_pcg_ws {
     double *r[2], *p[2], *q[2];
     const unsigned short* lof;
+    const unsigned short* mof;
     double* ic_l[2];
     double* pre_l[2];
     double* partials;
+    bool tail;
     double* red;
     PcgState* state;
     PcgState* host_state;
 };
 
 template <int NR>
-__device__ bool grid_reduce(double (&v)[NR], double* partials, unsigned* counter, double (&tot)[NR])
-{
-    __shared__ double sm[NR][SV_NT / 32];
-    __shared__ bool last;
+__device__ __forceinline__ void block_partial(const double (&v)[NR], double* partials, double (&sm)[NR][SV_NT / 32])
+{
     const int lane = threadIdx.x & 31, w = threadIdx.x >> 5;
 #pragma unroll
     for (int k = 0; k < NR; ++k) {
@@ -46,13 +48,12 @@
             for (int i = 0; i < SV_NT / 32; ++i) s += sm[k][i];
             partials[blockIdx.x * NR + k] = s;
         }
-        __threadfence();
-        const unsigned t = atomicInc(counter, gridDim.x - 1);
-        last = (t == gridDim.x - 1);
-    }
-    __syncthreads();
-    if (!last) return false;
-    __threadfence();
+    }
+}
+template <int NR>
+__device__ __forceinline__ void sum_partials(const double* partials, double (&sm)[NR][SV_NT / 32], double (&tot)[NR])
+{
+    const int lane = threadIdx.x & 31, w = threadIdx.x >> 5;
 #pragma unroll
     for (int k = 0; k < NR; ++k) {
         double s = 0.0;
@@ -65,6 +66,23 @@
         for (int i = 0; i < SV_NT / 32; ++i) t += sm[k][i];
         tot[k] = t;
     }
+}
+
+template <int NR>
+__device__ bool grid_reduce(double (&v)[NR], double* partials, unsigned* counter, double (&tot)[NR])
+{
+    __shared__ double sm[NR][SV_NT / 32];
+    __shared__ bool last;
+    block_partial<NR>(v, partials, sm);
+    if (threadIdx.x == 0) {
+        __threadfence();
+        const unsigned t = atomicInc(counter, gridDim.x - 1);
+        last = (t == gridDim.x - 1);
+    }
+    __syncthreads();
+    if (!last) return false;
+    __threadfence();
+    sum_partials<NR>(partials, sm, tot);
     return true;
 }
 
@@ -92,18 +110,21 @@
     s->rr = rr; s->d0 = rr; s->delta = rz; s->iter = 0;
     s->done = (rr <= 0.0 || s->itermax <= 0) ? 1 : 0;
 }
+__device__ __forceinline__ double alpha_of(double delta, double pq) { return pq != 0.0 ? delta / pq : 0.0; }
+__device__ __forceinline__ double beta_of(double delta, double rz) { return delta != 0.0 ? rz / delta : 0.0; }
+__device__ __forceinline__ bool stops(const PcgState& s, double rr, int iter) { return rr <= s.eps2 * s.d0 || iter >= s.itermax; }
 __device__ __forceinline__ void fin_apq(PcgState* s, double pq)
 {
     s->pq = pq;
-    s->alpha = pq != 0.0 ? s->delta / pq : 0.0;
+    s->alpha = alpha_of(s->delta, pq);
 }
 __device__ __forceinline__ void fin_update(PcgState* s, double rr, double rz)
 {
     s->rr = rr; s->rz = rz;
-    s->beta = s->delta != 0.0 ? rz / s->delta : 0.0;
+    s->beta = beta_of(s->delta, rz);
     s->delta = rz;
     s->iter += 1;
-    if (rr <= s->eps2 * s->d0 || s->iter >= s->itermax) s->done = 1;
+    if (stops(*s, rr, s->iter)) s->done = 1;
 }
 __global__ void pcg_scalar_kernel(gs_pcg_ws W, int stage)
 {
@@ -138,10 +159,10 @@
 
 #define SV_U 4
 
-__global__ void __launch_bounds__(SV_NT) pcg_apq_kernel(gs_pcg_ws W, int64_t n, int nc)
-{
-    if (W.state->done) return;
-    double v[1] = {0.0};
+template <class QLoad>
+__device__ __forceinline__ double apq_pass(const gs_pcg_ws& W, int64_t n, int nc, QLoad qload)
+{
+    double v = 0.0;
     const int64_t stride = (int64_t)gridDim.x * blockDim.x, total = nc * n;
     for (int64_t i0 = blockIdx.x * (int64_t)blockDim.x + threadIdx.x; i0 < total; i0 += SV_U * stride) {
         double p[SV_U], q[SV_U], ic[SV_U];
@@ -151,7 +172,15 @@
             int c; int64_t j;
             pick(i, n, c, j);
             const bool ok = i < total;
-            p[k] = ok ? (c ? W.p[1] : W.p[0])[j] : 0.0; q[k] = ok ? (c ? W.q[1] : W.q[0])[j] : 0.0;
+            q[k] = ok ? qload(c, j) : 0.0;
+        }
+#pragma unroll
+        for (int k = 0; k < SV_U; ++k) {
+            const int64_t i = i0 + k * stride;
+            int c; int64_t j;
+            pick(i, n, c, j);
+            const bool ok = i < total;
+            p[k] = ok ? (c ? W.p[1] : W.p[0])[j] : 0.0;
             ic[k] = ok ? __ldg((c ? W.ic_l[1] : W.ic_l[0]) + W.lof[j]) : 0.0;
         }
 #pragma unroll
@@ -162,21 +191,14 @@
             pick(i, n, c, j);
             const double qq = fma(ic[k], p[k], q[k]);
             (c ? W.q[1] : W.q[0])[j] = qq;
-            v[0] += p[k] * qq;
-        }
-    }
-    double tot[1];
-    if (grid_reduce<1>(v, W.partials, &W.state->counter, tot) && threadIdx.x == 0) {
-        if (W.red) W.red[0] = tot[0];
-        else fin_apq(W.state, tot[0]);
-    }
-}
-
-__global__ void __launch_bounds__(SV_NT) pcg_update_kernel(gs_pcg_ws W, double* xE, double* xB, int64_t n, int nc)
-{
-    if (W.state->done) return;
-    const double alpha = W.state->alpha;
-    double v[2] = {0.0, 0.0};
+            v += p[k] * qq;
+        }
+    }
+    return v;
+}
+
+__device__ __forceinline__ void update_pass(const gs_pcg_ws& W, double* xE, double* xB, int64_t n, int nc, double alpha, double (&v)[2])
+{
     const int64_t stride = (int64_t)gridDim.x * blockDim.x, total = nc * n;
     for (int64_t i0 = blockIdx.x * (int64_t)blockDim.x + threadIdx.x; i0 < total; i0 += SV_U * stride) {
         double x[SV_U], p[SV_U], q[SV_U], r[SV_U], pre[SV_U];
@@ -202,17 +224,10 @@
             v[1] += rr * rr * pre[k];
         }
     }
-    double tot[2];
-    if (grid_reduce<2>(v, W.partials, &W.state->counter, tot) && threadIdx.x == 0) {
-        if (W.red) { W.red[0] = tot[0]; W.red[1] = tot[1]; }
-        else fin_update(W.state, tot[0], tot[1]);
-    }
-}
-
-__global__ void __launch_bounds__(SV_NT) pcg_dir_kernel(gs_pcg_ws W, int64_t n, int nc)
-{
-    if (W.state->done) return;
-    const double beta = W.state->beta;
+}
+
+__device__ __forceinline__ void dir_pass(const gs_pcg_ws& W, int64_t n, int nc, double beta)
+{
     const int64_t stride = (int64_t)gridDim.x * blockDim.x, total = nc * n;
     for (int64_t i0 = blockIdx.x * (int64_t)blockDim.x + threadIdx.x; i0 < total; i0 += SV_U * stride) {
         double p[SV_U], r[SV_U], pre[SV_U];
@@ -236,6 +251,105 @@
     }
 }
 
+__global__ void __launch_bounds__(SV_NT) pcg_apq_kernel(gs_pcg_ws W, int64_t n, int nc)
+{
+    if (W.state->done) return;
+    double v[1] = {apq_pass(W, n, nc, [&](int c, int64_t j) { return (c ? W.q[1] : W.q[0])[j]; })};
+    double tot[1];
+    if (grid_reduce<1>(v, W.partials, &W.state->counter, tot) && threadIdx.x == 0) {
+        if (W.red) W.red[0] = tot[0];
+        else fin_apq(W.state, tot[0]);
+    }
+}
+
+__global__ void __launch_bounds__(SV_NT) pcg_update_kernel(gs_pcg_ws W, double* xE, double* xB, int64_t n, int nc)
+{
+    if (W.state->done) return;
+    double v[2] = {0.0, 0.0};
+    update_pass(W, xE, xB, n, nc, W.state->alpha, v);
+    double tot[2];
+    if (grid_reduce<2>(v, W.partials, &W.state->counter, tot) && threadIdx.x == 0) {
+        if (W.red) { W.red[0] = tot[0]; W.red[1] = tot[1]; }
+        else fin_update(W.state, tot[0], tot[1]);
+    }
+}
+
+__global__ void __launch_bounds__(SV_NT) pcg_dir_kernel(gs_pcg_ws W, int64_t n, int nc)
+{
+    if (W.state->done) return;
+    dir_pass(W, n, nc, W.state->beta);
+}
+
+template <int SPIN>
+__global__ void __launch_bounds__(SV_NT, 4)
+pcg_tail_kernel(PlanDev P, gs_pcg_ws W, LegFinishArgs F, const double* __restrict__ fl, double* xE, double* xB, int64_t n, int nc)
+{
+    const PcgState s = *W.state;
+    if (s.done) return;
+    __shared__ double sm1[1][SV_NT / 32], sm2[2][SV_NT / 32];
+    cooperative_groups::grid_group grid = cooperative_groups::this_grid();
+    const int L = P.lmax;
+    auto finish = [&](int c, int64_t j) {
+        const int l = W.lof[j], m = W.mof[j];
+        if (l < SPIN) return 0.0;
+        const int64_t base = (int64_t)m * (2 * L + 1 - m) / 2, id = base + l;
+        const int im = m ? (int)(j - (2 * base - (L + 1)) - 2 * l) : 0;
+        return leg_finish_one<SPIN>(F.partial, leg_finish_chunks(P, F.pcount, F.slot0, m, F.cp), P.nalm, id,
+                                    leg_finish_post<SPIN>(P, id, l, m, fl, 1.0, GS_ALM_REAL), (SPIN ? 2 * c : 0) + im);
+    };
+    double* part1 = W.partials + 2 * SV_GRID;
+    const double v1[1] = {apq_pass(W, n, nc, finish)};
+    block_partial<1>(v1, part1, sm1);
+    grid.sync();
+    double pq[1];
+    sum_partials<1>(part1, sm1, pq);
+    const double alpha = alpha_of(s.delta, pq[0]);
+
+    double v2[2] = {0.0, 0.0};
+    update_pass(W, xE, xB, n, nc, alpha, v2);
+    block_partial<2>(v2, W.partials, sm2);
+    grid.sync();
+    double tot[2];
+    sum_partials<2>(W.partials, sm2, tot);
+    if (blockIdx.x == 0 && threadIdx.x == 0) {
+        fin_apq(W.state, pq[0]);
+        fin_update(W.state, tot[0], tot[1]);
+    }
+    if (stops(s, tot[0], s.iter + 1)) return;
+    dir_pass(W, n, nc, beta_of(s.delta, tot[1]));
+}
+
+static int launch_tail(gs_plan* p, int spin, const gs_pcg_ws& w, const LegFinishArgs& F, const double* bl, double* xE, double* xB,
+                       int64_t n, int nc, cudaStream_t st)
+{
+    cudaLaunchConfig_t cfg = {};
+    cfg.gridDim = dim3(SV_GRID);
+    cfg.blockDim = dim3(SV_NT);
+    cfg.stream = st;
+    cudaLaunchAttribute attr[1];
+    attr[0].id = cudaLaunchAttributeCooperative;
+    attr[0].val.cooperative = 1;
+    cfg.attrs = attr;
+    cfg.numAttrs = 1;
+    if (spin) GS_CHECK_CUDA(cudaLaunchKernelEx(&cfg, pcg_tail_kernel<2>, p->d, w, F, bl, xE, xB, n, nc));
+    else GS_CHECK_CUDA(cudaLaunchKernelEx(&cfg, pcg_tail_kernel<0>, p->d, w, F, bl, xE, xB, n, nc));
+    g_gs_launches += 1;
+    return GS_OK;
+}
+
+static bool tail_fits(int device)
+{
+    int coop = 0, sms = 0, b0 = 0, b2 = 0;
+    if (cudaDeviceGetAttribute(&coop, cudaDevAttrCooperativeLaunch, device) != cudaSuccess ||
+        cudaDeviceGetAttribute(&sms, cudaDevAttrMultiProcessorCount, device) != cudaSuccess ||
+        cudaOccupancyMaxActiveBlocksPerMultiprocessor(&b0, pcg_tail_kernel<0>, SV_NT, 0) != cudaSuccess ||
+        cudaOccupancyMaxActiveBlocksPerMultiprocessor(&b2, pcg_tail_kernel<2>, SV_NT, 0) != cudaSuccess) {
+        cudaGetLastError();
+        return false;
+    }
+    return coop && (int64_t)std::min(b0, b2) * sms >= SV_GRID;
+}
+
 __global__ void zero2_kernel(double* a, double* b, int64_t n)
 {
     for (int64_t i = blockIdx.x * (int64_t)blockDim.x + threadIdx.x; i < n; i += (int64_t)gridDim.x * blockDim.x) {
@@ -262,20 +376,27 @@
         rhs[i] = fma(resc, rhs[i], fma(sic[i], xi[i], bdata[i]));
 }
 
-__global__ void lof_build_kernel(unsigned short* __restrict__ lof, const int* __restrict__ l_of_loc, int L, int64_t n)
-{
-    for (int64_t i = blockIdx.x * (int64_t)blockDim.x + threadIdx.x; i < n; i += (int64_t)gridDim.x * blockDim.x)
+__global__ void lof_build_kernel(unsigned short* __restrict__ lof, unsigned short* __restrict__ mof, const int* __restrict__ l_of_loc, int L, int64_t n)
+{
+    for (int64_t i = blockIdx.x * (int64_t)blockDim.x + threadIdx.x; i < n; i += (int64_t)gridDim.x * blockDim.x) {
         lof[i] = (unsigned short)(l_of_loc ? l_of_loc[i] : l_of_real(i, L));
-}
-static bool build_lof(gs_plan* p, const unsigned short** out)
-{
-    void* d = nullptr;
+        if (mof) mof[i] = (unsigned short)m_of_real(i, L);
+    }
+}
+static bool build_lof(gs_plan* p, const unsigned short** out, const unsigned short** mout)
+{
+    void *d = nullptr, *dm = nullptr;
     const int64_t n = p->nreal_loc;
     if (cudaMalloc(&d, (size_t)n * sizeof(unsigned short)) != cudaSuccess) return false;
     p->owned.push_back(d);
-    lof_build_kernel<<<SV_GRID, SV_NT>>>((unsigned short*)d, p->world > 1 ? p->d.sh.l_of_loc : nullptr, p->d.lmax, n);
+    if (p->world == 1) {
+        if (cudaMalloc(&dm, (size_t)n * sizeof(unsigned short)) != cudaSuccess) return false;
+        p->owned.push_back(dm);
+    }
+    lof_build_kernel<<<SV_GRID, SV_NT>>>((unsigned short*)d, (unsigned short*)dm, p->world > 1 ? p->d.sh.l_of_loc : nullptr, p->d.lmax, n);
     if (cudaDeviceSynchronize() != cudaSuccess) return false;
     *out = (const unsigned short*)d;
+    *mout = (const unsigned short*)dm;
     return true;
 }
 
@@ -308,8 +429,9 @@
     for (int c = 0; c < 2 && ok; ++c)
         ok = alloc_owned(p, &w->r[c], n) && alloc_owned(p, &w->p[c], n) && alloc_owned(p, &w->q[c], n) && alloc_owned(p, &w->ic_l[c], L1) &&
              alloc_owned(p, &w->pre_l[c], L1);
-    ok = ok && alloc_owned(p, &w->partials, SV_GRID * 2) && build_lof(p, &w->lof);
+    ok = ok && alloc_owned(p, &w->partials, SV_GRID * 3) && build_lof(p, &w->lof, &w->mof);
     ok = ok && alloc_state(p, &w->state, &w->host_state);
+    w->tail = p->world == 1 && tail_fits(p->device);
     if (!ok) { gs_set_error("PCG workspace allocation failed: %s", cudaGetErrorString(cudaGetLastError())); delete w; return nullptr; }
     p->pcg_ws = w;
     return w;
@@ -329,9 +451,10 @@
             w[k].q[c] = Q + (2 * k + c) * n;
             ok = alloc_owned(p, &w[k].r[c], n) && alloc_owned(p, &w[k].ic_l[c], L1) && alloc_owned(p, &w[k].pre_l[c], L1);
         }
-        ok = ok && alloc_owned(p, &w[k].partials, SV_GRID * 2);
-        if (ok) { if (k == 0) ok = build_lof(p, &w[0].lof); else w[1].lof = w[0].lof; }
+        ok = ok && alloc_owned(p, &w[k].partials, SV_GRID * 3);
+        if (ok) { if (k == 0) ok = build_lof(p, &w[0].lof, &w[0].mof); else { w[1].lof = w[0].lof; w[1].mof = w[0].mof; } }
         ok = ok && alloc_state(p, &w[k].state, &w[k].host_state);
+        w[k].tail = tail_fits(p->device);
     }
     void* d = nullptr;
     ok = ok && cudaMalloc(&d, sizeof(int)) == cudaSuccess;
@@ -361,6 +484,8 @@
 
 int g_gs_pcg_graph = 1;
 extern "C" int gs_set_pcg_graph(int on) { const int old = g_gs_pcg_graph; g_gs_pcg_graph = on ? 1 : 0; return old; }
+int g_gs_pcg_tail = 1;
+extern "C" int gs_set_pcg_tail(int on) { const int old = g_gs_pcg_tail; g_gs_pcg_tail = on ? 1 : 0; return old; }
 int g_gs_ring_fused = 1;
 extern "C" int gs_set_ring_fused(int fused) { const int old = g_gs_ring_fused; g_gs_ring_fused = fused ? 1 : 0; return old; }
 
@@ -384,17 +509,20 @@
 };
 
 static int apply_noise_op(gs_plan* p, const double* vE, const double* vB, const double* bl, const double* inv_noise,
-                          double* qE, double* qB, cudaStream_t st, const int* skip, int spin = 2, int nc = 1, int64_t stride = 0)
+                          double* qE, double* qB, cudaStream_t st, const int* skip, int spin = 2, int nc = 1, int64_t stride = 0,
+                          bool finish = true)
 {
     int rc;
-    if ((rc = gs_leg_synth(p, spin, vE, vB, GS_ALM_REAL, bl, st, skip, nullptr, nc, stride))) return rc;
-    if (g_gs_ring_fused || nc > 1) {
+    const bool fused = g_gs_ring_fused || nc > 1;
+    const double* rscale = fused ? gs_ring_direct_scale(p, spin, inv_noise) : nullptr;
+    if ((rc = gs_leg_synth(p, spin, vE, vB, GS_ALM_REAL, bl, st, skip, nullptr, nc, stride, rscale))) return rc;
+    if (fused) {
         if ((rc = gs_ring_apply(p, spin, inv_noise, st, skip, nc))) return rc;
     } else {
         if ((rc = gs_ring_synth(p, spin, p->mapQ_tmp, p->mapU_tmp, st, skip))) return rc;
         if ((rc = gs_ring_anal(p, spin, p->mapQ_tmp, p->mapU_tmp, inv_noise, st, skip))) return rc;
     }
-    return gs_leg_anal(p, spin, qE, qB, GS_ALM_REAL, bl, 1.0, 0, st, skip, nc, stride);
+    return gs_leg_anal(p, spin, qE, qB, GS_ALM_REAL, bl, 1.0, 0, st, skip, nc, stride, finish ? 1 : 0);
 }
 
 template <class Iteration>
@@ -532,9 +660,11 @@
     }
 
     const int* done = &w->state->done;
+    const bool tail = g_gs_pcg_tail && w->tail && !dist;
     auto iteration = [&](cudaStream_t s) -> int {
         int r;
-        if ((r = apply_noise_op(p, w->p[0], w->p[1], bl, inv_noise, w->q[0], w->q[1], s, done, spin))) return r;
+        if ((r = apply_noise_op(p, w->p[0], w->p[1], bl, inv_noise, w->q[0], w->q[1], s, done, spin, 1, 0, !tail))) return r;
+        if (tail) return launch_tail(p, spin, *w, gs_leg_finish_args(p, spin, 1), bl, x_E, x_B, n, nc, s);
         pcg_apq_kernel<<<SV_GRID, SV_NT, 0, s>>>(*w, n, nc);
         if (dist) {
             if ((r = gs_shard_allreduce(p, w->red, 1, s))) return r;
@@ -608,18 +738,26 @@
     }
     pcg_alldone_kernel<<<1, 1, 0, st>>>(W[0].state, W[1].state, p->pcg_alldone);
     const int64_t bstride = 2 * n;
+    const bool tail = g_gs_pcg_tail && W[0].tail;
     bool done[2] = {false, false};
     int launched = 0;
     while (!(done[0] && done[1]) && launched < itermax) {
         for (int it = 0; it < check_every && launched < itermax; ++it, ++launched) {
-            if (!done[0] && !done[1]) {
-                if ((rc = apply_noise_op(p, W[0].p[0], W[0].p[1], bl, inv_noise, W[0].q[0], W[0].q[1], st, p->pcg_alldone, 2, 2, bstride))) return rc;
+            const bool both = !done[0] && !done[1];
+            if (both) {
+                if ((rc = apply_noise_op(p, W[0].p[0], W[0].p[1], bl, inv_noise, W[0].q[0], W[0].q[1], st, p->pcg_alldone, 2, 2, bstride, !tail))) return rc;
             } else {
                 gs_pcg_ws* w = &W[done[0] ? 1 : 0];
-                if ((rc = apply_noise_op(p, w->p[0], w->p[1], bl, inv_noise, w->q[0], w->q[1], st, &w->state->done, 2))) return rc;
+                if ((rc = apply_noise_op(p, w->p[0], w->p[1], bl, inv_noise, w->q[0], w->q[1], st, &w->state->done, 2, 1, 0, !tail))) return rc;
             }
             for (int k = 0; k < 2; ++k) {
                 if (done[k]) continue;
+                if (tail) {
+                    LegFinishArgs F = gs_leg_finish_args(p, 2, both ? 2 : 1);
+                    if (both) F.partial += k * F.part_stride;
+                    if ((rc = launch_tail(p, 2, W[k], F, bl, x_E + k * stride, x_B + k * stride, n, 2, st))) return rc;
+                    continue;
+                }
                 pcg_apq_kernel<<<SV_GRID, SV_NT, 0, st>>>(W[k], n, 2);
                 pcg_update_kernel<<<SV_GRID, SV_NT, 0, st>>>(W[k], x_E + k * stride, x_B + k * stride, n, 2);
                 pcg_dir_kernel<<<SV_GRID, SV_NT, 0, st>>>(W[k], n, 2);
@@ -1020,6 +1158,7 @@
     std::swap(p->act_count, f.act_count);
     std::swap(p->act_slot0, f.act_slot0);
     std::swap(p->ring_wconst, f.ring_wconst);
+    std::swap(p->ring_sdir, f.ring_sdir);
     std::swap(p->groups0_dyn, f.groups0_dyn);
     std::swap(p->groups2_dyn, f.groups2_dyn);
 }
@@ -1032,7 +1171,7 @@
     auto alloc = [&](void** q, size_t bytes) { void* d = nullptr; if (cudaMalloc(&d, std::max<size_t>(16, bytes)) != cudaSuccess) return false; p->owned.push_back(d); *q = d; return true; };
     bool ok = alloc((void**)&f.act_ring, (size_t)p->d.nring) && alloc((void**)&f.act_pairs, (size_t)p->d.npair * sizeof(int)) &&
               alloc((void**)&f.act_count, sizeof(int)) && alloc((void**)&f.act_slot0, (size_t)2 * L1 * sizeof(int)) &&
-              alloc((void**)&f.ring_wconst, (size_t)p->d.nring * sizeof(double)) &&
+              alloc((void**)&f.ring_wconst, (size_t)p->d.nring * sizeof(double)) && alloc((void**)&f.ring_sdir, (size_t)2 * p->d.nring * sizeof(double)) &&
               alloc((void**)&f.groups0_dyn, (size_t)p->ngroups0 * sizeof(int2)) && alloc((void**)&f.groups2_dyn, (size_t)p->ngroups2 * sizeof(int2));
     if (!ok) { memset(&f, 0, sizeof(f)); gs_set_error("ring flag allocation failed: %s", cudaGetErrorString(cudaGetLastError())); return GS_E_NOMEM; }
     return GS_OK;
@@ -1269,7 +1408,7 @@
     if ((rc = act.begin(inv_noise, st))) { for (int i = 0; i < 5; ++i) cudaEventDestroy(ev[i]); return rc; }
     for (int r = 0; r < nrep && rc == GS_OK; ++r) {
         cudaEventRecord(ev[0], st);
-        rc = gs_leg_synth(p, 2, x_E, x_B, GS_ALM_REAL, bl, st);
+        rc = gs_leg_synth(p, 2, x_E, x_B, GS_ALM_REAL, bl, st, nullptr, nullptr, 1, 0, g_gs_ring_fused ? gs_ring_direct_scale(p, 2, inv_noise) : nullptr);
         cudaEventRecord(ev[1], st);
         if (!rc) rc = g_gs_ring_fused ? gs_ring_apply(p, 2, inv_noise, st) : gs_ring_synth(p, 2, p->mapQ_tmp, p->mapU_tmp, st);
         cudaEventRecord(ev[2], st);
@@ -1305,7 +1444,7 @@
         rc = act.begin(inv_noise, st);
         for (int r = 0; r < nrep && rc == GS_OK; ++r) {
             cudaEventRecord(ev[0], st);
-            rc = gs_leg_synth(p, 2, x_E, x_B, GS_ALM_REAL, bl, st, nullptr, nullptr, n_chain, stride);
+            rc = gs_leg_synth(p, 2, x_E, x_B, GS_ALM_REAL, bl, st, nullptr, nullptr, n_chain, stride, gs_ring_direct_scale(p, 2, inv_noise));
             cudaEventRecord(ev[1], st);
             if (!rc) rc = gs_ring_apply(p, 2, inv_noise, st, nullptr, n_chain);
             cudaEventRecord(ev[2], st);
diff --git a/include/gibbs_b200.h b/include/gibbs_b200.h
--- a/include/gibbs_b200.h
+++ b/include/gibbs_b200.h
@@ -81,6 +81,8 @@
                         int check_every, int* n_iter_out, double* resid_out, void* stream);
 
 int gs_set_pcg_graph(int on);
+
+int gs_set_pcg_tail(int on);
 
 int gs_cr_apply_q_pol(gs_plan* plan, const double* dl_EE, const double* dl_BB, const double* bl,
                       const double* inv_noise, const double* x_E, const double* x_B, double* y_E,
```
